# KhaoulaAguech/pl-fem-vectoriel

Hardware: AMD Instinct MI355X
Metric: eigenmodes/sec (assembly+solve), 7-core P2 mesh, 10 modes; |Δn_eff| vs ref (higher is better)
Workload: dtype f64

## Files before the change

### include/plfem.h

```cpp
#ifndef PLFEM_H
#define PLFEM_H

#include <stdint.h>

#ifdef __cplusplus
extern "C" {
#endif

#define PLFEM_OK 0
#define PLFEM_EINVAL (-1)
#define PLFEM_EMESH (-2)
#define PLFEM_EHIP (-3)
#define PLFEM_ENOCONV (-4)
#define PLFEM_ESTATE (-5)
#define PLFEM_ESINGULAR (-6)
#define PLFEM_ERESIDUAL (-7)
#define PLFEM_EHOST (-8)

typedef struct plfem_symbolic plfem_symbolic;
typedef struct plfem_ctx plfem_ctx;

int plfem_symbolic_create(int32_t nv, int32_t ne, const double* p_host, const int32_t* t_host,
                          int32_t leaf_elems, int32_t nthreads, plfem_symbolic** out,
                          char* err, int32_t errlen);
// ... 15 lines not shown
int plfem_symbolic_get(const plfem_symbolic* sym, const char* name, void* out_host, int64_t nbytes);

int plfem_mesh_edge_count(int32_t nv, int32_t ne, const double* p_host, const int32_t* t_host,
                          int32_t* nedges, char* err, int32_t errlen);
int plfem_mesh_refine(int32_t nv, int32_t ne, const double* p_host, const int32_t* t_host,
                      double* p_out, int32_t* t_out, char* err, int32_t errlen);

int plfem_mesh_refine_marked_count(int32_t nv, int32_t ne, const double* p_host, const int32_t* t_host,
                                   const uint8_t* marked_host, int32_t* nv_out, int32_t* ne_out, char* err, int32_t errlen);
int plfem_mesh_refine_marked(int32_t nv, int32_t ne, const double* p_host, const int32_t* t_host,
                             const uint8_t* marked_host, double* p_out, int32_t* t_out, int32_t* parent_out,
                             char* err, int32_t errlen);

#define PLFEM_MAX_NCV 320
int plfem_workspace_bytes(const plfem_symbolic* sym, int32_t max_ncv, int64_t* bytes);
int plfem_create(const plfem_symbolic* sym, int32_t device, void* hip_stream, int32_t max_ncv,
                 void* workspace_dev, int64_t workspace_bytes, plfem_ctx** out, char* err, int32_t errlen);
void plfem_destroy(plfem_ctx* ctx);
const char* plfem_last_error(const plfem_ctx* ctx);
int plfem_synchronize(plfem_ctx* ctx);

int plfem_assemble_hfield(plfem_ctx* ctx, const double* cores_host, int32_t ncore, double eps_core,
                          double eps_clad, double k0, double alpha_p);

int plfem_assemble_scalar(plfem_ctx* ctx, const double* cores_host, int32_t ncore, double eps_core,
                          double eps_clad, double k0);

int plfem_set_index_profile(plfem_ctx* ctx, const double* layers_host, int32_t nlayer, double eps_bg);

int plfem_set_index_map(plfem_ctx* ctx, const double* eps_host, int32_t nx, int32_t ny, double x0, double y0, double dx,
                        double dy);

int plfem_cmt_coupling(plfem_ctx* ctx, int32_t n, const double* fields_i_dev, const double* fields_j_dev,
                       const double* cores_host, int32_t ncore, double eps_core, double eps_clad,
                       double* raw_host, double* pi_host, double* pj_host, double* eps_mean_host);

enum { PLFEM_BLK_AXX = 0, PLFEM_BLK_AXY, PLFEM_BLK_AYX, PLFEM_BLK_AYY, PLFEM_BLK_MINV,
       PLFEM_BLK_DXX, PLFEM_BLK_DXY, PLFEM_BLK_DYY, PLFEM_BLK_COUNT };
int plfem_block_values_dev(plfem_ctx* ctx, int32_t block, const double** values_dev);
int plfem_block_values_host(plfem_ctx* ctx, int32_t block, double* values_host);

int plfem_spmv(plfem_ctx* ctx, int32_t which, const double* x_dev, double* y_dev);

int plfem_factor(plfem_ctx* ctx, double sigma);
int plfem_solve(plfem_ctx* ctx, const double* rhs_dev, double* x_dev, int32_t refine_steps);

int plfem_lanczos_shift_invert(plfem_ctx* ctx, int32_t k, int32_t ncv, double tol, int32_t maxiter,
                               double sigma, double* evals_host, double* evecs_dev, double* stats_host);

enum { PLFEM_POST_NORM = 0, PLFEM_POST_DIV_ENERGY, PLFEM_POST_CORE_X, PLFEM_POST_CORE_Y,
       PLFEM_POST_ALL_X, PLFEM_POST_ALL_Y, PLFEM_POST_COUNT };
int plfem_postprocess(plfem_ctx* ctx, int32_t k, double* evecs_dev, const double* cores_host,
                      int32_t ncore, double* out_host, double* frac_core_host, double* modes_int_dev);

int plfem_residuals(plfem_ctx* ctx, int32_t k, const double* evals_host, const double* evecs_dev, double* out_host);

enum { PLFEM_SOLVE_NCONV = 0, PLFEM_SOLVE_NOPINV, PLFEM_SOLVE_RESTARTS, PLFEM_SOLVE_MAX_REL_RES, PLFEM_SOLVE_BLOCK_SOLVES,
       PLFEM_SOLVE_RESIDUAL_FIRST, PLFEM_SOLVE_RESIDUAL, PLFEM_SOLVE_REFINED, PLFEM_SOLVE_PERTURBED,
       PLFEM_SOLVE_T_ASSEMBLE_US, PLFEM_SOLVE_T_FACTOR_US, PLFEM_SOLVE_T_LANCZOS_US, PLFEM_SOLVE_T_POST_US,
       PLFEM_SOLVE_T_UPLOAD_US, PLFEM_SOLVE_T_RESIDUAL_US, PLFEM_SOLVE_T_CALL_US, PLFEM_SOLVE_STATS };
int plfem_solve_modes(plfem_ctx* ctx, const double* cores_host, int32_t ncore, double eps_core, double eps_clad,
                      double k0, double alpha_p, double sigma, int32_t k, int32_t ncv, double tol, int32_t maxiter,
                      double residual_tol, double tol_refined, double* evals_host, double* post_host,
                      double* frac_core_host, double* resid_host, double* modes_int_host, double* stats_host);
int plfem_modes_dev(plfem_ctx* ctx, const double** evecs_dev, int32_t* k);

int plfem_set_option(plfem_ctx* ctx, const char* name, double value);

int plfem_timings(plfem_ctx* ctx, double* out_host );

enum { PLFEM_PROF_KFWD = 0, PLFEM_PROF_FWD_SWEEP, PLFEM_PROF_BWD_SWEEP, PLFEM_PROF_SPMV_B, PLFEM_PROF_COUNT };
int plfem_profile_begin(plfem_ctx* ctx, int32_t max_ranges);
int plfem_profile_end(plfem_ctx* ctx, double* out_host );

#define PLFEM_LOC_TOL 1e-10
#define PLFEM_LOC_EPS4 8.881784197001252e-16
typedef struct plfem_locator plfem_locator;
int plfem_locator_bytes(const plfem_symbolic* sym, int64_t* bytes);
int plfem_locator_create(const plfem_symbolic* sym, int32_t device, void* hip_stream, void* mem_dev, int64_t mem_bytes,
                         plfem_locator** out, char* err, int32_t errlen);
void plfem_locator_destroy(plfem_locator* loc);
const char* plfem_locator_last_error(const plfem_locator* loc);
int plfem_stage_modes(plfem_locator* loc, int32_t ncomp, int32_t k, int32_t nrows, const double* src_dev, double* dst_dev);
int plfem_sample_fields(plfem_locator* loc, int32_t ncomp, int32_t k, const double* modes_dev, int32_t indexed,
                        const double* beta_dev, int32_t npts, const double* points_dev, double* out_dev, int32_t* elem_dev);
int plfem_overlap_work_bytes(int32_t ka, int32_t kb, int64_t* bytes);
int plfem_field_overlap(plfem_locator* loc_a, const double* modes_a_dev, int32_t ka, int32_t indexed_a,
                        plfem_locator* loc_b, const double* modes_b_dev, int32_t kb, int32_t indexed_b, int32_t ncomp,
                        const double* cores_host, int32_t ncore, double eps_core, double eps_clad,
                        void* work_dev, int64_t work_bytes, double* out_host);
int plfem_overlap_posed_work_bytes(const plfem_locator* loc_b, int32_t ka, int32_t kb, int32_t nposes, int64_t* bytes);
int plfem_field_overlap_posed(plfem_locator* loc_a, const double* modes_a_dev, int32_t ka, int32_t indexed_a,
                              plfem_locator* loc_b, const double* modes_b_dev, int32_t kb, int32_t indexed_b, int32_t ncomp,
                              const double* cores_host, int32_t ncore, double eps_core, double eps_clad,
                              int32_t nposes, const double* poses_host ,
                              void* work_dev, int64_t work_bytes, double* out_host );
int plfem_gram_work_bytes(int32_t ncomp, int32_t k, int64_t* bytes);
int plfem_mode_grams(plfem_locator* loc, int32_t ncomp, int32_t k, const double* modes_dev, int32_t indexed,
                     const double* cores_host, int32_t ncore, void* work_dev, int64_t work_bytes, double* out_host);

int plfem_profile_gram_work_bytes(int32_t ncomp, int32_t k, int64_t* bytes);
int plfem_profile_grams(plfem_locator* loc, int32_t ncomp, int32_t k, const double* modes_dev, int32_t indexed,
                        const double* layers_host, int32_t nlayer, double eps_bg, void* work_dev, int64_t work_bytes,
                        double* out_host);

int plfem_locator_set_index_map(plfem_locator* loc, const double* eps_host, int32_t nx, int32_t ny, double x0, double y0,
                                double dx, double dy);

int plfem_core_gram_work_bytes(const plfem_locator* loc, int32_t ncomp, int32_t k, int32_t ncore, int64_t* bytes);
int plfem_core_grams(plfem_locator* loc, int32_t ncomp, int32_t k, const double* modes_dev, int32_t indexed,
                     const double* cores_host, int32_t ncore, void* work_dev, int64_t work_bytes,
                     double* out_host   ,
                     int64_t* count_host );

int plfem_moment_gram_work_bytes(int32_t ncomp, int32_t k, int64_t* bytes);
int plfem_moment_grams(plfem_locator* loc, int32_t ncomp, int32_t k, const double* modes_dev, int32_t indexed,
                       const double* cores_host, int32_t ncore, const double origin_host[2], void* work_dev,
                       int64_t work_bytes, double* out_host);

int plfem_quartic_work_bytes(int32_t ncomp, int32_t k, int64_t* bytes);
int plfem_mode_quartic(plfem_locator* loc, int32_t ncomp, int32_t k, const double* modes_dev, int32_t indexed,
                       const double* cores_host, int32_t ncore, double w_core, double w_clad,
                       void* work_dev, int64_t work_bytes, double* out_host);

int plfem_project_work_bytes(int32_t ncomp, int32_t k, int32_t la, int32_t lb, int64_t* bytes);
int plfem_mode_project(plfem_locator* loc, int32_t ncomp, int32_t k, const double* modes_dev, int32_t indexed,
                       int32_t la, const double* xfac_host ,
                       int32_t lb, const double* yfac_host ,
                       void* work_dev, int64_t work_bytes, double* out_host );

int plfem_project_sampled_work_bytes(int32_t ncomp, int32_t k, int32_t nf, int64_t* bytes);
int plfem_mode_project_sampled(plfem_locator* loc, int32_t ncomp, int32_t k, const double* modes_dev, int32_t indexed,
                               int32_t nx, int32_t ny, double x0, double y0, double dx, double dy,
                               int32_t nf, const double* frames_dev ,
                               void* work_dev, int64_t work_bytes, double* out_host );

int plfem_indicator_work_bytes(const plfem_locator* loc, int32_t ncomp, int32_t k, int64_t* bytes);
int plfem_mode_indicators(plfem_locator* loc, int32_t ncomp, int32_t k, const double* modes_dev, int32_t indexed,
                          const double* lambda_host , double k0, double alpha_p,
                          const double* cores_host, int32_t ncore, double eps_core, double eps_clad,
                          const double* layers_host, int32_t nlayer, double eps_bg,
                          void* work_dev, int64_t work_bytes, double* out_host );

#ifdef PLFEM_TEST_HOOKS
int plfem_debug_factor_until(plfem_ctx* ctx, double sigma, int32_t level, int32_t step, int32_t stage);
int plfem_debug_copy(plfem_ctx* ctx, const char* name, int64_t offset, int64_t count, double* out_host);
int plfem_debug_symeig(int32_t n, const double* a_host, int32_t last_rows, double* w_out, double* v_out);
int plfem_debug_symeig_band(int32_t n, int32_t b, const double* a_host, int32_t nsel, double* w_out, double* v_out);
int plfem_debug_set_perturb(plfem_ctx* ctx, double value);
int plfem_debug_set_elements(plfem_ctx* ctx, const double* elem_host );
#define PLFEM_DEBUG_PLAN_FIELDS 10
int plfem_debug_solve_block(plfem_ctx* ctx, const double* rhs_dev, int64_t ldx, double* x_dev, int32_t refine_steps);
int plfem_debug_level_plan(plfem_ctx* ctx, int64_t* out, int64_t cap);
enum { PLFEM_DEBUG_PANEL_DOT = 0, PLFEM_DEBUG_PANEL_AXPY, PLFEM_DEBUG_PANEL_DOT_BLOCK, PLFEM_DEBUG_PANEL_AXPY_BLOCK };
enum { PLFEM_DEBUG_SPMV_B_BLOCK = 0, PLFEM_DEBUG_SPMV_B_BLOCK_IL, PLFEM_DEBUG_SPMV_B_BLOCK_IL_GRAM, PLFEM_DEBUG_SPMV_A_BLOCK };
int plfem_debug_panel(plfem_ctx* ctx, int32_t form, int32_t ncols, const double* Pm, double* W, int64_t ldw, double* H,
                      int32_t ldh, double* hacc, int32_t ldacc, double* wil);
int plfem_debug_scale_store(plfem_ctx* ctx, const double* w, const double* bw, const double* beta2, double* v, double* bv,
                            double* beta_out);
int plfem_debug_first_pass(plfem_ctx* ctx, const double* xl_front, const double* BVm, const double* Vm, int32_t ncols,
                           double* W, int64_t ldw, double* Hout, int32_t ldh);
int plfem_debug_spmv_block(plfem_ctx* ctx, int32_t form, const double* x, double* y, int64_t ld, double* gram_out,
                           int32_t* nparts);
int plfem_debug_chol(plfem_ctx* ctx, const double* G, int32_t ldg, int32_t use_partials, int32_t nchunks, double* Tblk,
                     int32_t ldT, double* Rinv, int32_t* rank_flag);
int plfem_debug_block_scale(plfem_ctx* ctx, const double* W, const double* BW, int64_t ldw, const double* Rinv, double* Vn,
                            double* BVn, int64_t ldv, const double* exp_src, int32_t exp_n, double* exp_dst, int32_t* cnt_dst,
                            int32_t want_front);
int plfem_debug_rotate(plfem_ctx* ctx, const double* V, int32_t m, const double* S, int32_t ldS, int32_t p, double* out);
int plfem_debug_start_field(plfem_ctx* ctx, int32_t nvec, double* out);
#endif

#ifdef __cplusplus
}
#endif
#endif
```

### pl_fem_vectoriel_amd/_native.py

```python
from __future__ import annotations

import ctypes
import time
import os
from typing import Optional

import numpy as np

_HERE = os.path.dirname(os.path.abspath(__file__))
LIB_PATH = os.path.join(_HERE, "libplfem_hip.so")
HOOKS_PATH = os.path.join(_HERE, "libplfem_testhooks.so")

PLFEM_OK = 0
PLFEM_EINVAL, PLFEM_EMESH, PLFEM_EHIP, PLFEM_ENOCONV, PLFEM_ESTATE, PLFEM_ESINGULAR, PLFEM_ERESIDUAL = -1, -2, -3, -4, -5, -6, -7
PLFEM_EHOST = -8
BLOCKS = ("Axx", "Axy", "Ayx", "Ayy", "Minv", "Dxx", "Dxy", "Dyy")
INFO_NAMES = ("nv", "ne", "nedges", "N", "nsolve", "nnz", "levels", "nfronts", "front_doubles", "max_front",
              "solve_entries", "factor_flops", "t_numbering_us", "t_pattern_us", "t_tree_us", "t_fronts_us", "dofs_per_node",
              "arena_doubles")
POST_NAMES = ("norm", "div_energy", "core_x", "core_y", "all_x", "all_y")

EXPORTS = (
    "plfem_symbolic_create", "plfem_symbolic_destroy", "plfem_symbolic_info", "plfem_symbolic_array_bytes",
    "plfem_symbolic_get", "plfem_workspace_bytes", "plfem_create", "plfem_destroy", "plfem_last_error", "plfem_synchronize",
    "plfem_assemble_hfield", "plfem_block_values_dev", "plfem_block_values_host", "plfem_spmv", "plfem_factor",
    "plfem_solve", "plfem_lanczos_shift_invert", "plfem_postprocess", "plfem_timings",
    "plfem_profile_begin", "plfem_profile_end",
    "plfem_mesh_edge_count", "plfem_mesh_refine",
    "plfem_residuals", "plfem_set_option", "plfem_symbolic_create_ex", "plfem_assemble_scalar", "plfem_cmt_coupling",
    "plfem_solve_modes", "plfem_modes_dev",
    "plfem_locator_bytes", "plfem_locator_create", "plfem_locator_destroy", "plfem_locator_last_error", "plfem_stage_modes",
    "plfem_sample_fields", "plfem_overlap_work_bytes", "plfem_field_overlap", "plfem_gram_work_bytes", "plfem_mode_grams",
    "plfem_overlap_posed_work_bytes", "plfem_field_overlap_posed",
    "plfem_quartic_work_bytes", "plfem_mode_quartic", "plfem_project_work_bytes", "plfem_mode_project",
    "plfem_core_gram_work_bytes", "plfem_core_grams", "plfem_moment_gram_work_bytes", "plfem_moment_grams",
    "plfem_set_index_profile", "plfem_profile_gram_work_bytes", "plfem_profile_grams",
    "plfem_project_sampled_work_bytes", "plfem_mode_project_sampled",
    "plfem_indicator_work_bytes", "plfem_mode_indicators", "plfem_mesh_refine_marked_count", "plfem_mesh_refine_marked",
    "plfem_set_index_map", "plfem_locator_set_index_map",
)
SOLVE_STATS = ("nconv", "n_opinv", "restarts", "max_rel_res", "n_block_solves", "true_residual_first", "true_residual", "refined",
               "pivot_perturbations", "assemble_us", "factor_us", "lanczos_us", "post_us", "upload_us", "residual_us", "call_us")
TEST_HOOK_EXPORTS = ("plfem_debug_factor_until", "plfem_debug_copy", "plfem_debug_symeig", "plfem_debug_symeig_band",
                     "plfem_debug_set_perturb", "plfem_debug_solve_block", "plfem_debug_level_plan", "plfem_debug_panel",
                     "plfem_debug_scale_store", "plfem_debug_first_pass", "plfem_debug_spmv_block", "plfem_debug_chol",
                     "plfem_debug_block_scale", "plfem_debug_rotate", "plfem_debug_start_field", "plfem_debug_set_elements")
PANEL_FORMS = ("dot", "axpy", "dot_block", "axpy_block")
SPMV_BLOCK_FORMS = ("b_block", "b_block_il", "b_block_il_gram", "a_block")
BLOCK_P = 4
PLAN_FIELDS = ("count", "fwd_rows", "bwd_rows", "fwd_mixed", "max_s2", "max_m", "fwd_n", "bwd_n", "steps", "max_block_p")
MAX_NCV = 320
PROF_SLOTS = ("k_fwd", "fwd_sweep", "bwd_sweep", "spmv_b")

_ARRAY_DTYPES = {
    "edof": np.int32, "tsorted": np.int32, "edges": np.int32, "doflocs": np.float64, "bmask": np.uint8,
    "interior": np.int32, "int_index": np.int32, "rowptr": np.int32, "colind": np.int32, "slot_row": np.int32,
    "nptr": np.int32, "nadj": np.int32, "nloc": np.uint8, "leaf_of_elem": np.int32, "leaf_elem_ptr": np.int32, "leaf_elems": np.int32, "epos": np.int32, "epos_leaf": np.int32,
    "owner": np.int32, "fs": np.int32, "fb": np.int32, "fs_true": np.int32, "fb_true": np.int32,
    "fnode_ptr": np.int64, "fnodes": np.int32, "cinv0": np.int32, "cinv1": np.int32, "foff": np.int64, "soff": np.int64, "prow": np.int32, "npos": np.int32,
    "loc_grid": np.float64, "loc_cell_ptr": np.int32, "loc_cell_elems": np.int32, "loc_stats": np.float64,
    "elem_nbr": np.int32,
}


from scipy.sparse.linalg import ArpackNoConvergence as _ArpackNoConvergence


def set_index_map_call(entry, handle, index_map):
    if index_map is None:
        return entry(handle, None, 0, 0, 0.0, 0.0, 0.0, 0.0)
    eps, x0, y0, dx, dy = index_map
    eps = np.ascontiguousarray(eps, dtype=np.float64)
    if eps.ndim != 2:
        raise ValueError("the index map must be a (ny, nx) array")
    return entry(handle, eps.ctypes.data_as(ctypes.c_void_p), eps.shape[1], eps.shape[0], float(x0), float(y0), float(dx),
                 float(dy))


class ArpackLikeNoConvergence(_ArpackNoConvergence, RuntimeError):

    def __init__(self, msg, eigenvalues=None, eigenvectors=None, stats=None):
        _ArpackNoConvergence.__init__(self, msg, eigenvalues, eigenvectors)
        self.stats = stats


_lib = None
_hooks = None

SCRATCH_FILL = None


def device_scratch(nbytes: int, tdev):
    import torch
    if SCRATCH_FILL is None:
        return torch.empty(int(nbytes), dtype=torch.uint8, device=tdev)
    buf = torch.empty((int(nbytes) + 7) & ~7, dtype=torch.uint8, device=tdev)
    buf.view(torch.float64).fill_(float(SCRATCH_FILL))
    torch.cuda.current_stream(tdev).synchronize()
    return buf


def device_output(shape, dtype, tdev):
    import torch
    if SCRATCH_FILL is None:
        return torch.empty(shape, dtype=dtype, device=tdev)
    shape = tuple(int(v) for v in (shape if isinstance(shape, (tuple, list)) else (shape,)))
    nbytes = int(np.prod(shape, dtype=np.int64)) * torch.empty((), dtype=dtype).element_size()
    return device_scratch(nbytes, tdev)[:nbytes].view(dtype).view(shape)


def _tune_host_allocator(_force: bool = False) -> None:
    if os.environ.get("PLFEM_MALLOC_TUNE", "0") != "1" and not _force:
        return
    try:
        libc = ctypes.CDLL("libc.so.6")
        libc.mallopt(-3, 32 << 20)
        libc.mallopt(-1, 512 << 20)
    except (OSError, AttributeError):
        pass


def load_library() -> ctypes.CDLL:
    global _lib
    if _lib is not None:
        return _lib
    if not os.path.exists(LIB_PATH):
        raise RuntimeError(
            f"libplfem_hip.so requis: {LIB_PATH} not found — build it with "
            "`python -c 'import __graft_entry__ as g; g.build()'` (hipcc --offload-arch=gfx950). "
            "There is no CPU fallback for the eigenmode path.")
    import torch
    lib = ctypes.CDLL(LIB_PATH)
    _tune_host_allocator()
    c_void_pp = ctypes.POINTER(ctypes.c_void_p)
    lib.plfem_symbolic_create.argtypes = [ctypes.c_int32, ctypes.c_int32, ctypes.c_void_p, ctypes.c_void_p,
                                          ctypes.c_int32, ctypes.c_int32, c_void_pp, ctypes.c_char_p, ctypes.c_int32]
    lib.plfem_symbolic_create_ex.argtypes = [ctypes.c_int32, ctypes.c_int32, ctypes.c_void_p, ctypes.c_void_p, ctypes.c_int32,
                                             ctypes.c_int32, ctypes.c_int32, ctypes.c_int32, c_void_pp, ctypes.c_char_p, ctypes.c_int32]
    lib.plfem_symbolic_destroy.argtypes = [ctypes.c_void_p]
    lib.plfem_symbolic_destroy.restype = None
    lib.plfem_symbolic_info.argtypes = [ctypes.c_void_p, ctypes.c_void_p]
    lib.plfem_symbolic_array_bytes.argtypes = [ctypes.c_void_p, ctypes.c_char_p]
    lib.plfem_symbolic_array_bytes.restype = ctypes.c_int64
    lib.plfem_symbolic_get.argtypes = [ctypes.c_void_p, ctypes.c_char_p, ctypes.c_void_p, ctypes.c_int64]
    lib.plfem_workspace_bytes.argtypes = [ctypes.c_void_p, ctypes.c_int32, ctypes.POINTER(ctypes.c_int64)]
    lib.plfem_create.argtypes = [ctypes.c_void_p, ctypes.c_int32, ctypes.c_void_p, ctypes.c_int32, ctypes.c_void_p,
                                 ctypes.c_int64, c_void_pp, ctypes.c_char_p, ctypes.c_int32]
    lib.plfem_destroy.argtypes = [ctypes.c_void_p]
    lib.plfem_destroy.restype = None
    lib.plfem_last_error.argtypes = [ctypes.c_void_p]
    lib.plfem_last_error.restype = ctypes.c_char_p
    lib.plfem_synchronize.argtypes = [ctypes.c_void_p]
    lib.plfem_assemble_hfield.argtypes = [ctypes.c_void_p, ctypes.c_void_p, ctypes.c_int32, ctypes.c_double,
                                          ctypes.c_double, ctypes.c_double, ctypes.c_double]
    lib.plfem_assemble_scalar.argtypes = [ctypes.c_void_p, ctypes.c_void_p, ctypes.c_int32, ctypes.c_double,
                                          ctypes.c_double, ctypes.c_double]
    lib.plfem_cmt_coupling.argtypes = [ctypes.c_void_p, ctypes.c_int32, ctypes.c_void_p, ctypes.c_void_p, ctypes.c_void_p,
                                       ctypes.c_int32, ctypes.c_double, ctypes.c_double, ctypes.c_void_p, ctypes.c_void_p,
                                       ctypes.c_void_p, ctypes.POINTER(ctypes.c_double)]
    lib.plfem_block_values_dev.argtypes = [ctypes.c_void_p, ctypes.c_int32, c_void_pp]
    lib.plfem_block_values_host.argtypes = [ctypes.c_void_p, ctypes.c_int32, ctypes.c_void_p]
    lib.plfem_spmv.argtypes = [ctypes.c_void_p, ctypes.c_int32, ctypes.c_void_p, ctypes.c_void_p]
    lib.plfem_factor.argtypes = [ctypes.c_void_p, ctypes.c_double]
    lib.plfem_solve.argtypes = [ctypes.c_void_p, ctypes.c_void_p, ctypes.c_void_p, ctypes.c_int32]
    lib.plfem_lanczos_shift_invert.argtypes = [ctypes.c_void_p, ctypes.c_int32, ctypes.c_int32, ctypes.c_double,
                                               ctypes.c_int32, ctypes.c_double, ctypes.c_void_p, ctypes.c_void_p,
                                               ctypes.c_void_p]
    lib.plfem_postprocess.argtypes = [ctypes.c_void_p, ctypes.c_int32, ctypes.c_void_p, ctypes.c_void_p,
                                      ctypes.c_int32, ctypes.c_void_p, ctypes.c_void_p, ctypes.c_void_p]
    lib.plfem_timings.argtypes = [ctypes.c_void_p, ctypes.c_void_p]
    lib.plfem_mesh_edge_count.argtypes = [ctypes.c_int32, ctypes.c_int32, ctypes.c_void_p, ctypes.c_void_p,
                                          ctypes.POINTER(ctypes.c_int32), ctypes.c_char_p, ctypes.c_int32]
    lib.plfem_mesh_refine.argtypes = [ctypes.c_int32, ctypes.c_int32, ctypes.c_void_p, ctypes.c_void_p,
                                      ctypes.c_void_p, ctypes.c_void_p, ctypes.c_char_p, ctypes.c_int32]
    lib.plfem_profile_begin.argtypes = [ctypes.c_void_p, ctypes.c_int32]
    lib.plfem_profile_end.argtypes = [ctypes.c_void_p, ctypes.c_void_p]
    lib.plfem_residuals.argtypes = [ctypes.c_void_p, ctypes.c_int32, ctypes.c_void_p, ctypes.c_void_p, ctypes.c_void_p]
    lib.plfem_set_option.argtypes = [ctypes.c_void_p, ctypes.c_char_p, ctypes.c_double]
    lib.plfem_solve_modes.argtypes = ([ctypes.c_void_p, ctypes.c_void_p, ctypes.c_int32] + [ctypes.c_double] * 5 +
                                      [ctypes.c_int32, ctypes.c_int32, ctypes.c_double, ctypes.c_int32, ctypes.c_double,
                                       ctypes.c_double] + [ctypes.c_void_p] * 6)
    lib.plfem_modes_dev.argtypes = [ctypes.c_void_p, c_void_pp, ctypes.POINTER(ctypes.c_int32)]
    lib.plfem_locator_bytes.argtypes = [ctypes.c_void_p, ctypes.POINTER(ctypes.c_int64)]
    lib.plfem_locator_create.argtypes = [ctypes.c_void_p, ctypes.c_int32, ctypes.c_void_p, ctypes.c_void_p, ctypes.c_int64,
                                         c_void_pp, ctypes.c_char_p, ctypes.c_int32]
    lib.plfem_locator_destroy.argtypes = [ctypes.c_void_p]
    lib.plfem_locator_destroy.restype = None
    lib.plfem_locator_last_error.argtypes = [ctypes.c_void_p]
    lib.plfem_locator_last_error.restype = ctypes.c_char_p
    lib.plfem_stage_modes.argtypes = [ctypes.c_void_p, ctypes.c_int32, ctypes.c_int32, ctypes.c_int32, ctypes.c_void_p,
                                      ctypes.c_void_p]
    lib.plfem_sample_fields.argtypes = [ctypes.c_void_p, ctypes.c_int32, ctypes.c_int32, ctypes.c_void_p, ctypes.c_int32,
                                        ctypes.c_void_p, ctypes.c_int32, ctypes.c_void_p, ctypes.c_void_p, ctypes.c_void_p]
    lib.plfem_overlap_work_bytes.argtypes = [ctypes.c_int32, ctypes.c_int32, ctypes.POINTER(ctypes.c_int64)]
    lib.plfem_field_overlap.argtypes = ([ctypes.c_void_p, ctypes.c_void_p, ctypes.c_int32, ctypes.c_int32] * 2 +
                                        [ctypes.c_int32, ctypes.c_void_p, ctypes.c_int32, ctypes.c_double, ctypes.c_double,
                                         ctypes.c_void_p, ctypes.c_int64, ctypes.c_void_p])
    lib.plfem_overlap_posed_work_bytes.argtypes = [ctypes.c_void_p, ctypes.c_int32, ctypes.c_int32, ctypes.c_int32,
                                                   ctypes.POINTER(ctypes.c_int64)]
    lib.plfem_field_overlap_posed.argtypes = ([ctypes.c_void_p, ctypes.c_void_p, ctypes.c_int32, ctypes.c_int32] * 2 +
                                              [ctypes.c_int32, ctypes.c_void_p, ctypes.c_int32, ctypes.c_double, ctypes.c_double,
                                               ctypes.c_int32, ctypes.c_void_p, ctypes.c_void_p, ctypes.c_int64, ctypes.c_void_p])
    lib.plfem_gram_work_bytes.argtypes = [ctypes.c_int32, ctypes.c_int32, ctypes.POINTER(ctypes.c_int64)]
    lib.plfem_mode_grams.argtypes = [ctypes.c_void_p, ctypes.c_int32, ctypes.c_int32, ctypes.c_void_p, ctypes.c_int32,
                                     ctypes.c_void_p, ctypes.c_int32, ctypes.c_void_p, ctypes.c_int64, ctypes.c_void_p]
    lib.plfem_core_gram_work_bytes.argtypes = [ctypes.c_void_p, ctypes.c_int32, ctypes.c_int32, ctypes.c_int32,
                                               ctypes.POINTER(ctypes.c_int64)]
    lib.plfem_core_grams.argtypes = [ctypes.c_void_p, ctypes.c_int32, ctypes.c_int32, ctypes.c_void_p, ctypes.c_int32,
                                     ctypes.c_void_p, ctypes.c_int32, ctypes.c_void_p, ctypes.c_int64, ctypes.c_void_p,
                                     ctypes.c_void_p]
    lib.plfem_moment_gram_work_bytes.argtypes = [ctypes.c_int32, ctypes.c_int32, ctypes.POINTER(ctypes.c_int64)]
    lib.plfem_moment_grams.argtypes = [ctypes.c_void_p, ctypes.c_int32, ctypes.c_int32, ctypes.c_void_p, ctypes.c_int32,
                                       ctypes.c_void_p, ctypes.c_int32, ctypes.c_void_p, ctypes.c_void_p, ctypes.c_int64,
                                       ctypes.c_void_p]
    lib.plfem_set_index_profile.argtypes = [ctypes.c_void_p, ctypes.c_void_p, ctypes.c_int32, ctypes.c_double]
    lib.plfem_set_index_map.argtypes = [ctypes.c_void_p, ctypes.c_void_p, ctypes.c_int32, ctypes.c_int32] + [ctypes.c_double] * 4
    lib.plfem_locator_set_index_map.argtypes = lib.plfem_set_index_map.argtypes
    lib.plfem_profile_gram_work_bytes.argtypes = [ctypes.c_int32, ctypes.c_int32, ctypes.POINTER(ctypes.c_int64)]
    lib.plfem_profile_grams.argtypes = [ctypes.c_void_p, ctypes.c_int32, ctypes.c_int32, ctypes.c_void_p, ctypes.c_int32,
                                        ctypes.c_void_p, ctypes.c_int32, ctypes.c_double, ctypes.c_void_p, ctypes.c_int64,
                                        ctypes.c_void_p]
    lib.plfem_quartic_work_bytes.argtypes = [ctypes.c_int32, ctypes.c_int32, ctypes.POINTER(ctypes.c_int64)]
    lib.plfem_mode_quartic.argtypes = [ctypes.c_void_p, ctypes.c_int32, ctypes.c_int32, ctypes.c_void_p, ctypes.c_int32,
                                       ctypes.c_void_p, ctypes.c_int32, ctypes.c_double, ctypes.c_double, ctypes.c_void_p,
                                       ctypes.c_int64, ctypes.c_void_p]
    lib.plfem_project_work_bytes.argtypes = [ctypes.c_int32] * 4 + [ctypes.POINTER(ctypes.c_int64)]
    lib.plfem_mode_project.argtypes = [ctypes.c_void_p, ctypes.c_int32, ctypes.c_int32, ctypes.c_void_p, ctypes.c_int32,
                                       ctypes.c_int32, ctypes.c_void_p, ctypes.c_int32, ctypes.c_void_p, ctypes.c_void_p,
                                       ctypes.c_int64, ctypes.c_void_p]
    lib.plfem_project_sampled_work_bytes.argtypes = [ctypes.c_int32] * 3 + [ctypes.POINTER(ctypes.c_int64)]
    lib.plfem_mode_project_sampled.argtypes = [ctypes.c_void_p, ctypes.c_int32, ctypes.c_int32, ctypes.c_void_p, ctypes.c_int32,
                                               ctypes.c_int32, ctypes.c_int32, ctypes.c_double, ctypes.c_double, ctypes.c_double,
                                               ctypes.c_double, ctypes.c_int32, ctypes.c_void_p, ctypes.c_void_p, ctypes.c_int64,
                                               ctypes.c_void_p]
    lib.plfem_indicator_work_bytes.argtypes = [ctypes.c_void_p, ctypes.c_int32, ctypes.c_int32, ctypes.POINTER(ctypes.c_int64)]
    lib.plfem_mode_indicators.argtypes = [ctypes.c_void_p, ctypes.c_int32, ctypes.c_int32, ctypes.c_void_p, ctypes.c_int32,
                                          ctypes.c_void_p, ctypes.c_double, ctypes.c_double, ctypes.c_void_p, ctypes.c_int32,
                                          ctypes.c_double, ctypes.c_double, ctypes.c_void_p, ctypes.c_int32, ctypes.c_double,
                                          ctypes.c_void_p, ctypes.c_int64, ctypes.c_void_p]
    lib.plfem_mesh_refine_marked_count.argtypes = [ctypes.c_int32, ctypes.c_int32, ctypes.c_void_p, ctypes.c_void_p,
                                                   ctypes.c_void_p, ctypes.POINTER(ctypes.c_int32),
                                                   ctypes.POINTER(ctypes.c_int32), ctypes.c_char_p, ctypes.c_int32]
    lib.plfem_mesh_refine_marked.argtypes = [ctypes.c_int32, ctypes.c_int32, ctypes.c_void_p, ctypes.c_void_p, ctypes.c_void_p,
                                             ctypes.c_void_p, ctypes.c_void_p, ctypes.c_void_p, ctypes.c_char_p, ctypes.c_int32]
    _lib = lib
    return lib


def _ptr(a: np.ndarray):
    return a.ctypes.data_as(ctypes.c_void_p)


def mesh_refine(p, t):
    lib = load_library()
    p = np.ascontiguousarray(np.asarray(p, dtype=np.float64))
    t = np.ascontiguousarray(np.asarray(t, dtype=np.int32))
    if p.ndim != 2 or p.shape[0] != 2 or t.ndim != 2 or t.shape[0] != 3:
        raise ValueError("mesh.p must be (2, nv) and mesh.t (3, ne)")
    err = ctypes.create_string_buffer(512)
    nedges = ctypes.c_int32(0)
    rc = lib.plfem_mesh_edge_count(p.shape[1], t.shape[1], _ptr(p), _ptr(t), ctypes.byref(nedges), err, 512)
    if rc != PLFEM_OK:
        raise ValueError(f"plfem_mesh_edge_count failed ({rc}): {err.value.decode()}")
    p2 = np.empty((2, p.shape[1] + nedges.value), dtype=np.float64)
    t2 = np.empty((3, 4 * t.shape[1]), dtype=np.int32)
    rc = lib.plfem_mesh_refine(p.shape[1], t.shape[1], _ptr(p), _ptr(t), _ptr(p2), _ptr(t2), err, 512)
    if rc != PLFEM_OK:
        raise ValueError(f"plfem_mesh_refine failed ({rc}): {err.value.decode()}")
    return p2, t2


def mesh_refine_marked(p, t, marked):
    lib = load_library()
    p = np.ascontiguousarray(np.asarray(p, dtype=np.float64))
    t = np.ascontiguousarray(np.asarray(t, dtype=np.int32))
    if p.ndim != 2 or p.shape[0] != 2 or t.ndim != 2 or t.shape[0] != 3:
        raise ValueError("mesh.p must be (2, nv) and mesh.t (3, ne)")
    try:
        mk = np.asarray(marked)
        if mk.dtype.kind not in "biu":
            raise TypeError
    except (TypeError, ValueError):
        raise ValueError("marked must be an array of one flag (bool or integer) per element") from None
    if mk.shape != (t.shape[1],):
        raise ValueError(f"marked must have one flag per element ({t.shape[1]}), got shape {mk.shape}")
    mk = np.ascontiguousarray(mk != 0, dtype=np.uint8)
    err = ctypes.create_string_buffer(512)
    nv2, ne2 = ctypes.c_int32(0), ctypes.c_int32(0)
    rc = lib.plfem_mesh_refine_marked_count(p.shape[1], t.shape[1], _ptr(p), _ptr(t), _ptr(mk), ctypes.byref(nv2),
                                            ctypes.byref(ne2), err, 512)
    if rc != PLFEM_OK:
        raise ValueError(f"plfem_mesh_refine_marked_count failed ({rc}): {err.value.decode()}")
    p2 = np.empty((2, nv2.value), dtype=np.float64)
    t2 = np.empty((3, ne2.value), dtype=np.int32)
    parent = np.empty(ne2.value, dtype=np.int32)
    rc = lib.plfem_mesh_refine_marked(p.shape[1], t.shape[1], _ptr(p), _ptr(t), _ptr(mk), _ptr(p2), _ptr(t2), _ptr(parent),
                                      err, 512)
    if rc != PLFEM_OK:
        raise ValueError(f"plfem_mesh_refine_marked failed ({rc}): {err.value.decode()}")
    return p2, t2, parent


def load_test_hooks() -> ctypes.CDLL:
    global _hooks
    if _hooks is not None:
        return _hooks
    load_library()
    if not os.path.exists(HOOKS_PATH):
        raise RuntimeError(f"{HOOKS_PATH} not found -- build it with `python -c 'import __graft_entry__ as g; g.build()'`")
    h = ctypes.CDLL(HOOKS_PATH)
    h.plfem_debug_factor_until.argtypes = [ctypes.c_void_p, ctypes.c_double, ctypes.c_int32, ctypes.c_int32, ctypes.c_int32]
    h.plfem_debug_copy.argtypes = [ctypes.c_void_p, ctypes.c_char_p, ctypes.c_int64, ctypes.c_int64, ctypes.c_void_p]
    h.plfem_debug_set_perturb.argtypes = [ctypes.c_void_p, ctypes.c_double]
    h.plfem_debug_set_elements.argtypes = [ctypes.c_void_p, ctypes.c_void_p]
    h.plfem_debug_solve_block.argtypes = [ctypes.c_void_p, ctypes.c_void_p, ctypes.c_int64, ctypes.c_void_p, ctypes.c_int32]
    h.plfem_debug_level_plan.argtypes = [ctypes.c_void_p, ctypes.c_void_p, ctypes.c_int64]
    h.plfem_debug_symeig.argtypes = [ctypes.c_int32, ctypes.c_void_p, ctypes.c_int32, ctypes.c_void_p, ctypes.c_void_p]
    h.plfem_debug_symeig_band.argtypes = [ctypes.c_int32, ctypes.c_int32, ctypes.c_void_p, ctypes.c_int32,
                                          ctypes.c_void_p, ctypes.c_void_p]
    vp, i32, i64 = ctypes.c_void_p, ctypes.c_int32, ctypes.c_int64
    h.plfem_debug_panel.argtypes = [vp, i32, i32, vp, vp, i64, vp, i32, vp, i32, vp]
    h.plfem_debug_scale_store.argtypes = [vp, vp, vp, vp, vp, vp, vp]
    h.plfem_debug_first_pass.argtypes = [vp, vp, vp, vp, i32, vp, i64, vp, i32]
    h.plfem_debug_spmv_block.argtypes = [vp, i32, vp, vp, i64, vp, vp]
    h.plfem_debug_chol.argtypes = [vp, vp, i32, i32, i32, vp, i32, vp, vp]
    h.plfem_debug_block_scale.argtypes = [vp, vp, vp, i64, vp, vp, vp, i64, vp, i32, vp, vp, i32]
    h.plfem_debug_rotate.argtypes = [vp, vp, i32, vp, i32, i32, vp]
    h.plfem_debug_start_field.argtypes = [vp, i32, vp]
    _hooks = h
    return h


def debug_symeig(a, last_rows: int = -1):
    lib = load_test_hooks()
    a = np.ascontiguousarray(np.asarray(a, dtype=np.float64))
    n = a.shape[0]
    if a.shape != (n, n):
        raise ValueError("square matrix expected")
    w = np.empty(n, dtype=np.float64)
    v = np.empty((n, n if last_rows < 0 else last_rows), dtype=np.float64)
    rc = lib.plfem_debug_symeig(n, _ptr(a), int(last_rows), _ptr(w), _ptr(v))
    if rc != PLFEM_OK:
        raise ValueError(f"plfem_debug_symeig failed ({rc})")
    return w, v


def debug_symeig_band(a, b: int, nsel: int):
    lib = load_test_hooks()
    a = np.ascontiguousarray(np.asarray(a, dtype=np.float64))
    n = a.shape[0]
    if a.shape != (n, n):
        raise ValueError("square matrix expected")
    w = np.empty(n, dtype=np.float64)
    v = np.empty((n, n), dtype=np.float64)
    rc = lib.plfem_debug_symeig_band(n, int(b), _ptr(a), int(nsel), _ptr(w), _ptr(v))
    if rc != PLFEM_OK:
        raise ValueError(f"plfem_debug_symeig_band failed ({rc})")
    return w, v


def default_host_threads() -> int:
    ncpu = os.cpu_count() or 1
    if ncpu < 64:
        return max(1, min(ncpu, 8))
    try:
        local_world = max(1, int(os.environ.get("LOCAL_WORLD_SIZE", "1")))
    except ValueError:
        local_world = 1
    return max(2, min(24, (ncpu // 2) // local_world))


class Symbolic:

    def __init__(self, p, t, leaf_elems: int = 0, nthreads: int = 0, dofs_per_node: int = 2, dirichlet: bool = True):
        lib = load_library()
        p = np.ascontiguousarray(np.asarray(p, dtype=np.float64))
        t = np.ascontiguousarray(np.asarray(t, dtype=np.int32))
        if p.ndim != 2 or p.shape[0] != 2 or t.ndim != 2 or t.shape[0] != 3:
            raise ValueError("mesh.p must be (2, nv) and mesh.t (3, ne)")
        h = ctypes.c_void_p()
        err = ctypes.create_string_buffer(512)
        if nthreads <= 0:
            nthreads = int(os.environ.get("PLFEM_HOST_THREADS", default_host_threads()))
        if leaf_elems <= 0:
            leaf_elems = int(os.environ.get("PLFEM_LEAF_ELEMS", 0))
        rc = lib.plfem_symbolic_create_ex(p.shape[1], t.shape[1], _ptr(p), _ptr(t), int(leaf_elems), int(nthreads),
                                          int(dofs_per_node), 1 if dirichlet else 0, ctypes.byref(h), err, 512)
        if rc != PLFEM_OK:
            raise ValueError(f"plfem_symbolic_create failed ({rc}): {err.value.decode()}")
        self._h = h
        self._lib = lib
        info = np.zeros(32, dtype=np.int64)
        lib.plfem_symbolic_info(h, _ptr(info))
        self.info = {k: int(info[i]) for i, k in enumerate(INFO_NAMES)}
        for k in ("nv", "ne", "nedges", "N", "nsolve", "nnz"):
            setattr(self, k, self.info[k])
        self.dofs_per_node = self.info["dofs_per_node"]

    def array(self, name: str) -> np.ndarray:
        nb = self._lib.plfem_symbolic_array_bytes(self._h, name.encode())
        if nb < 0:
            raise KeyError(name)
        out = np.empty(nb // np.dtype(_ARRAY_DTYPES[name]).itemsize, dtype=_ARRAY_DTYPES[name])
        rc = self._lib.plfem_symbolic_get(self._h, name.encode(), _ptr(out), ctypes.c_int64(nb))
        if rc != PLFEM_OK:
            raise RuntimeError(f"plfem_symbolic_get({name}) failed: {rc}")
        return out

    def close(self):
        if getattr(self, "_h", None):
            self._lib.plfem_symbolic_destroy(self._h)
            self._h = None

    def __del__(self):
        try:
            self.close()
        except Exception:
            pass


class Context:

    def __init__(self, sym: Symbolic, device: Optional[int] = None, max_ncv: int = 65, use_torch_stream: bool = True):
        import torch

        lib = load_library()
        if not torch.cuda.is_available():
            raise RuntimeError("no HIP device visible: the eigenmode path has no CPU fallback")
        if device is None:
            device = torch.cuda.current_device()
        self.torch = torch
        self.device = int(device)
        self.tdev = torch.device("cuda", self.device)
        self.sym = sym
        self._lib = lib
        stream = torch.cuda.current_stream(self.tdev).cuda_stream if use_torch_stream else 0
        h = ctypes.c_void_p()
        err = ctypes.create_string_buffer(512)
        need = ctypes.c_int64(0)
        rc = lib.plfem_workspace_bytes(sym._h, int(max_ncv), ctypes.byref(need))
        if rc != PLFEM_OK:
            raise ValueError(f"plfem_workspace_bytes failed ({rc})")
        t0 = time.perf_counter()
        self.workspace = device_scratch(int(need.value) + 256, self.tdev)
        self.t_workspace = time.perf_counter() - t0
        base = self.workspace.data_ptr()
        aligned = (base + 255) & ~255
        rc = lib.plfem_create(sym._h, self.device, ctypes.c_void_p(stream), int(max_ncv), ctypes.c_void_p(aligned),
                              ctypes.c_int64(int(need.value)), ctypes.byref(h), err, 512)
        if rc in (PLFEM_EINVAL, PLFEM_EMESH):
            raise ValueError(f"plfem_create: {err.value.decode()}")
        if rc != PLFEM_OK:
            raise RuntimeError(f"plfem_create failed ({rc}): {err.value.decode()}")
        self._h = h
        self.max_ncv = int(max_ncv)
        self.N = sym.N
        self.dpn = sym.dofs_per_node
        self.n2 = self.dpn * sym.N

    def _check(self, rc, what):
        if rc == PLFEM_OK:
            return
        msg = self._lib.plfem_last_error(self._h).decode()
        if rc in (PLFEM_EINVAL, PLFEM_EMESH):
            raise ValueError(f"{what}: {msg}")
        raise RuntimeError(f"{what} failed ({rc}): {msg}")

    def _cores(self, cores):
        c = np.ascontiguousarray(np.asarray(cores, dtype=np.float64).reshape(-1, 3))
        return c, c.shape[0]

    def empty(self, *shape):
        return device_output(shape, self.torch.float64, self.tdev)

    def set_index_profile(self, profile=None):
        if profile is None:
            self._check(self._lib.plfem_set_index_profile(self._h, None, 0, 0.0), "plfem_set_index_profile")
            self.set_index_map(None)
            return
        t = np.ascontiguousarray(np.asarray(profile.table(), dtype=np.float64).reshape(-1, 8))
        index_map = getattr(profile, "index_map", None)
        if t.shape[0] == 0 and index_map is None:
            raise ValueError("plfem_set_index_profile: the profile has no layers")
# ... 41 lines not shown
    def factor(self, sigma: float):
        self._check(self._lib.plfem_factor(self._h, float(sigma)), "plfem_factor")

    def solve(self, rhs, refine_steps: int = 0):
        x = self.empty(self.n2)
        self._check(self._lib.plfem_solve(self._h, ctypes.c_void_p(rhs.data_ptr()), ctypes.c_void_p(x.data_ptr()),
                                          int(refine_steps)), "plfem_solve")
        return x

    def lanczos(self, k, ncv, tol, maxiter, sigma):
        evals = np.empty(k, dtype=np.float64)
        evecs = self.empty(k, self.n2)
        stats = np.zeros(8, dtype=np.float64)
        rc = self._lib.plfem_lanczos_shift_invert(self._h, int(k), int(ncv), float(tol), int(maxiter), float(sigma),
                                                  _ptr(evals), ctypes.c_void_p(evecs.data_ptr()), _ptr(stats))
        st = {"nconv": int(stats[0]), "n_opinv": int(stats[1]), "restarts": int(stats[2]), "max_rel_res": float(stats[3]),
              "n_block_solves": int(stats[4])}
        if rc == PLFEM_ENOCONV:
            raise ArpackLikeNoConvergence(self._lib.plfem_last_error(self._h).decode(), evals, evecs, st)
        self._check(rc, "plfem_lanczos_shift_invert")
        return evals, evecs, st

    def solve_modes(self, cores, eps_core, eps_clad, k0, alpha_p, sigma, k, ncv, tol, maxiter, residual_tol, tol_refined,
                    modes_host=None):
        c, n = self._cores(cores)
        evals = np.empty(k, dtype=np.float64)
        post = np.zeros((k, len(POST_NAMES)), dtype=np.float64)
        resid = np.zeros(k, dtype=np.float64)
        stats = np.zeros(len(SOLVE_STATS), dtype=np.float64)
        frac = ctypes.c_double(0.0)
        if modes_host is not None and (tuple(modes_host.shape) != (k, self.dpn * self.sym.nsolve) or not modes_host.is_contiguous()
                                       or modes_host.dtype != self.torch.float64 or modes_host.device.type != "cpu"):
            raise ValueError("modes_host must be a contiguous float64 CPU tensor of shape (k, dofs_per_node * nsolve)")
        rc = self._lib.plfem_solve_modes(self._h, _ptr(c), n, float(eps_core), float(eps_clad), float(k0), float(alpha_p),
                                         float(sigma), int(k), int(ncv), float(tol), int(maxiter), float(residual_tol),
                                         float(tol_refined), _ptr(evals), _ptr(post), ctypes.cast(ctypes.byref(frac), ctypes.c_void_p),
                                         _ptr(resid), ctypes.c_void_p(modes_host.data_ptr()) if modes_host is not None else None,
                                         _ptr(stats))
        st = {name: (float(stats[i]) if name.endswith("_us") or "res" in name else int(stats[i])) for i, name in enumerate(SOLVE_STATS)}
        st["refined"] = bool(st["refined"])
        if rc == PLFEM_ENOCONV:
            raise ArpackLikeNoConvergence(self._lib.plfem_last_error(self._h).decode(), evals, self.modes_dev(), st)
        self._check(rc, "plfem_solve_modes")
        return evals, post, float(frac.value), resid, st

    def modes_dev(self):
        ptr = ctypes.c_void_p()
        k = ctypes.c_int32(0)
        self._check(self._lib.plfem_modes_dev(self._h, ctypes.byref(ptr), ctypes.byref(k)), "plfem_modes_dev")

        class _View:
            __cuda_array_interface__ = {"shape": (int(k.value), int(self.n2)), "typestr": "<f8", "data": (int(ptr.value), False),
                                        "version": 2, "strides": None}
        return self.torch.as_tensor(_View(), device=self.tdev).clone()

    def postprocess(self, evecs, cores, want_interior: bool = True):
        k = evecs.shape[0]
        c, n = self._cores(cores)
        out = np.zeros((k, len(POST_NAMES)), dtype=np.float64)
        frac = ctypes.c_double(0.0)
        modes_int = self.empty(k, self.dpn * self.sym.nsolve) if want_interior else None
        self._check(self._lib.plfem_postprocess(self._h, int(k), ctypes.c_void_p(evecs.data_ptr()), _ptr(c), n,
                                                _ptr(out), ctypes.byref(frac),
                                                ctypes.c_void_p(modes_int.data_ptr()) if want_interior else None),
                    "plfem_postprocess")
        return out, float(frac.value), modes_int

    def timings(self):
        t = np.zeros(8, dtype=np.float64)
        self._check(self._lib.plfem_timings(self._h, _ptr(t)), "plfem_timings")
        return {"assemble_us": t[0], "factor_us": t[1], "lanczos_us": t[2], "post_us": t[3], "upload_us": t[4],
                "pivot_perturbations": int(t[5])}

    def debug_factor_until(self, sigma, level, step, stage):
        self._check(load_test_hooks().plfem_debug_factor_until(self._h, float(sigma), int(level), int(step), int(stage)),
                    "plfem_debug_factor_until")

    def debug_copy(self, name: str, offset: int, count: int) -> np.ndarray:
        out = np.empty(int(count), dtype=np.float64)
        self._check(load_test_hooks().plfem_debug_copy(self._h, name.encode(), ctypes.c_int64(int(offset)),
                                                       ctypes.c_int64(int(count)), _ptr(out)), "plfem_debug_copy")
        return out

    def debug_set_perturb(self, value: float):
        self._check(load_test_hooks().plfem_debug_set_perturb(self._h, float(value)), "plfem_debug_set_perturb")

    def debug_set_elements(self, elem: np.ndarray):
        elem = np.ascontiguousarray(elem, dtype=np.float64)
        if elem.size != self.sym.ne * 8 * 36:
            raise ValueError("debug_set_elements: need ne x 8 x 36 doubles")
        self._check(load_test_hooks().plfem_debug_set_elements(self._h, _ptr(elem)), "plfem_debug_set_elements")

    def debug_solve_block(self, rhs, x, ldx: int, refine_steps: int = 0):
        self._check(load_test_hooks().plfem_debug_solve_block(self._h, ctypes.c_void_p(rhs.data_ptr()), ctypes.c_int64(int(ldx)),
                                                              ctypes.c_void_p(x.data_ptr()), int(refine_steps)),
                    "plfem_debug_solve_block")

    @staticmethod
    def _dev(t, offset: int = 0):
        return None if t is None else ctypes.c_void_p(t.data_ptr() + 8 * int(offset))

    def debug_panel(self, form: str, ncols: int, Pm, W, ldw: int, H, ldh: int, hacc=None, ldacc: int = 0, wil=None):
        d = self._dev
        self._check(load_test_hooks().plfem_debug_panel(self._h, PANEL_FORMS.index(form), int(ncols), d(Pm), d(W), int(ldw), d(H),
                                                        int(ldh), d(hacc), int(ldacc), d(wil)), "plfem_debug_panel")

    def debug_scale_store(self, w, bw, beta2, v, bv, beta_out=None):
        d = self._dev
        self._check(load_test_hooks().plfem_debug_scale_store(self._h, d(w), d(bw), d(beta2), d(v), d(bv), d(beta_out)),
                    "plfem_debug_scale_store")

    def debug_first_pass(self, xl_front, BVm, Vm, ncols: int, W, ldw: int, Hout, ldh: int):
        d = self._dev
        self._check(load_test_hooks().plfem_debug_first_pass(self._h, d(xl_front), d(BVm), d(Vm), int(ncols), d(W), int(ldw),
                                                             d(Hout), int(ldh)), "plfem_debug_first_pass")

    def debug_spmv_block(self, form: str, x, y, ld: int, gram_out=None) -> int:
        nparts = ctypes.c_int32(0)
        d = self._dev
        self._check(load_test_hooks().plfem_debug_spmv_block(self._h, SPMV_BLOCK_FORMS.index(form), d(x), d(y), int(ld),
                                                             d(gram_out), ctypes.byref(nparts)), "plfem_debug_spmv_block")
        return int(nparts.value)

    def debug_chol(self, G, ldg: int, use_partials: bool, nchunks: int, Tblk, ldT: int, Rinv, Tblk_offset: int = 0) -> int:
        flag = ctypes.c_int32(0)
        d = self._dev
        self._check(load_test_hooks().plfem_debug_chol(self._h, d(G), int(ldg), 1 if use_partials else 0, int(nchunks),
                                                       d(Tblk, Tblk_offset), int(ldT), d(Rinv), ctypes.byref(flag)),
                    "plfem_debug_chol")
        return int(flag.value)

    def debug_block_scale(self, W, BW, ldw: int, Rinv, Vn, BVn, ldv: int, exp_src=None, exp_n: int = 0, exp_dst=None,
                          cnt_dst=None, want_front: bool = False):
        d = self._dev
        self._check(load_test_hooks().plfem_debug_block_scale(self._h, d(W), d(BW), int(ldw), d(Rinv), d(Vn), d(BVn), int(ldv),
                                                              d(exp_src), int(exp_n), d(exp_dst), d(cnt_dst),
                                                              1 if want_front else 0), "plfem_debug_block_scale")

    def debug_rotate(self, V, m: int, S, ldS: int, p: int, out):
        d = self._dev
        self._check(load_test_hooks().plfem_debug_rotate(self._h, d(V), int(m), d(S), int(ldS), int(p), d(out)),
                    "plfem_debug_rotate")

    def debug_start_field(self, nvec: int, out):
        self._check(load_test_hooks().plfem_debug_start_field(self._h, int(nvec), self._dev(out)), "plfem_debug_start_field")

    def debug_level_plan(self):
        nl = self.sym.info["levels"] + 1
        out = np.zeros(len(PLAN_FIELDS) * nl, dtype=np.int64)
        self._check(load_test_hooks().plfem_debug_level_plan(self._h, _ptr(out), ctypes.c_int64(out.size)),
                    "plfem_debug_level_plan")
        return [dict(zip(PLAN_FIELDS, (int(v) for v in row))) for row in out.reshape(nl, len(PLAN_FIELDS))]

    def profile_begin(self, max_launches: int = 4096):
        self._check(self._lib.plfem_profile_begin(self._h, int(max_launches)), "plfem_profile_begin")

    def profile_end(self):
        out = np.zeros((len(PROF_SLOTS), 3), dtype=np.float64)
        self._check(self._lib.plfem_profile_end(self._h, _ptr(out)), "plfem_profile_end")
        res = {"launches": int(out[0, 0]), "total_us": float(out[0, 1]), "bytes": float(out[0, 2])}
        res["slots"] = {name: {"ranges": int(out[i, 0]), "total_us": float(out[i, 1]), "bytes": float(out[i, 2])}
                        for i, name in enumerate(PROF_SLOTS)}
        return res

    def residuals(self, evals, evecs) -> np.ndarray:
        lam = np.ascontiguousarray(np.asarray(evals, dtype=np.float64))
        out = np.zeros(len(lam), dtype=np.float64)
        self._check(self._lib.plfem_residuals(self._h, len(lam), _ptr(lam), ctypes.c_void_p(evecs.data_ptr()), _ptr(out)),
                    "plfem_residuals")
        return out

    def set_option(self, name: str, value: float):
        self._check(self._lib.plfem_set_option(self._h, name.encode(), float(value)), "plfem_set_option")

    def synchronize(self):
        self._check(self._lib.plfem_synchronize(self._h), "plfem_synchronize")

    def close(self):
        if getattr(self, "_h", None):
            self._lib.plfem_destroy(self._h)
            self._h = None
            self.workspace = None

    def __del__(self):
        try:
            self.close()
        except Exception:
            pass
```

### pl_fem_vectoriel_amd/csrc/api_debug.hip

```cpp
#include <algorithm>
#include <cmath>
#include <cstring>
#include <numeric>
#include <string>
#include <vector>

#ifndef PLFEM_TEST_HOOKS
#define PLFEM_TEST_HOOKS 1
#endif
#include "device.h"

namespace {
void perturb_root_pivots(plfem_ctx* c) {
  if (c->test_perturb != 0.0)
    plfem::launch_axpby(c, (int64_t)2 * c->dpn * c->S->fs[0], 1.0 + c->test_perturb, c->d_delta, 0.0, c->d_delta,
                        c->d_delta);
}
}

extern "C" int plfem_debug_set_perturb(plfem_ctx* c, double value) try {
  if (!c) return PLFEM_EINVAL;
  c->test_perturb = value;
  c->test_post_factor = value != 0.0 ? perturb_root_pivots : nullptr;
  c->factored = false;
  return PLFEM_OK;
} catch (...) { return host_failure(c); }

extern "C" int plfem_debug_factor_until(plfem_ctx* c, double sigma, int32_t level, int32_t step, int32_t stage) try {
  if (!c) return PLFEM_EINVAL;
  if (!c->assembled) { c->err = "debug factor before assemble"; return PLFEM_ESTATE; }
  TRY(wait_for_upload(c));
  plfem::launch_factor(c, sigma, level, step, stage);
  HIP_TRY(c, hipStreamSynchronize(c->stream));
  return check_launch(c, "debug factor");
} catch (...) { return host_failure(c); }

extern "C" int plfem_debug_copy(plfem_ctx* c, const char* name, int64_t offset, int64_t count, double* out_host) try {
  if (!c || !name || !out_host || offset < 0 || count < 0) return PLFEM_EINVAL;
  std::string n(name);
  const double* src = nullptr;
  if (n == "front") src = c->d_front;
  else if (n == "schur") src = c->d_schur;
  else if (n == "fvec") src = c->d_fvec;
  else if (n == "wbuf") src = c->d_wbuf;
  else if (n == "rbuf") src = c->d_rbuf;
  else if (n == "dinv") src = c->d_dinv;
  else if (n == "delta") src = c->d_delta;
  else if (n == "fvec2") src = c->d_fvec2;
  else if (n == "xl") src = c->d_xl;
  else if (n == "elem") src = c->d_elem;
  else if (n == "V") src = c->d_V;
  else if (n == "BV") src = c->d_BV;
  else if (n == "Hcols") src = c->d_Hcols;
  else if (n == "counters") {
    if (offset + count > 4) return PLFEM_EINVAL;
    int32_t tmp[4];
    HIP_TRY(c, hipStreamSynchronize(c->stream));
    HIP_TRY(c, hipMemcpy(tmp, c->d_counters, sizeof(tmp), hipMemcpyDeviceToHost));
    for (int64_t q = 0; q < count; ++q) out_host[q] = (double)tmp[offset + q];
    return PLFEM_OK;
  }
  else if (n == "colind" || n == "slot_row") {
    if (offset + count > c->nnz) return PLFEM_EINVAL;
    std::vector<int32_t> tmp((size_t)count);
    HIP_TRY(c, hipStreamSynchronize(c->stream));
    HIP_TRY(c, hipMemcpy(tmp.data(), (n == "colind" ? c->d_colind : c->d_slot_row) + offset, sizeof(int32_t) * count, hipMemcpyDeviceToHost));
    for (int64_t q = 0; q < count; ++q) out_host[q] = (double)tmp[q];
    return PLFEM_OK;
  }
  else return PLFEM_EINVAL;
  HIP_TRY(c, hipStreamSynchronize(c->stream));
  HIP_TRY(c, hipMemcpy(out_host, src + offset, sizeof(double) * count, hipMemcpyDeviceToHost));
  return PLFEM_OK;
} catch (...) { return host_failure(c); }

extern "C" int plfem_debug_set_elements(plfem_ctx* c, const double* elem_host) try {
  if (!c || !elem_host) return PLFEM_EINVAL;
  HIP_TRY(c, hipSetDevice(c->device));
  TRY(wait_for_upload(c));
  HIP_TRY(c, hipStreamSynchronize(c->stream));
  HIP_TRY(c, hipMemcpy(c->d_elem, elem_host, sizeof(double) * (size_t)c->ne * plfem::ELEM_STRIDE, hipMemcpyHostToDevice));
  plfem::launch_csr_gather(c);
  HIP_TRY(c, hipStreamSynchronize(c->stream));
  TRY(check_launch(c, "debug set elements"));
  c->assembled = true;
  c->factored = false;
  return PLFEM_OK;
} catch (...) { return host_failure(c); }

extern "C" int plfem_debug_solve_block(plfem_ctx* c, const double* rhs_dev, int64_t ldx, double* x_dev, int32_t refine_steps) try {
  constexpr int P = plfem::BLOCK_P;
  if (!c || !rhs_dev || !x_dev || refine_steps < 0) return PLFEM_EINVAL;
  if (!c->factored) { c->err = "debug block solve before plfem_factor"; return PLFEM_ESTATE; }
  if (c->max_block_p < P) { c->err = "debug block solve: the LDS budget of this tree allows one right-hand side per sweep"; return PLFEM_EINVAL; }
  if (ldx < c->n2) { c->err = "debug block solve: ldx < n2"; return PLFEM_EINVAL; }
  const int64_t scratch = (int64_t)c->n2 * plfem::basis_cols(c->max_ncv);
  if (refine_steps > 0 && 3 * P * ldx > scratch) { c->err = "debug block solve: ldx too large for the refinement scratch"; return PLFEM_EINVAL; }
  HIP_TRY(c, hipSetDevice(c->device));
  plfem::solve_refined(c, P, rhs_dev, x_dev, ldx, false, refine_steps, c->d_V2, c->d_V2 + (size_t)P * ldx,
                       c->d_V2 + (size_t)2 * P * ldx);
  HIP_TRY(c, hipStreamSynchronize(c->stream));
  return check_launch(c, "debug block solve");
} catch (...) { return host_failure(c); }

extern "C" int plfem_debug_level_plan(plfem_ctx* c, int64_t* out, int64_t cap) try {
  if (!c || !out) return PLFEM_EINVAL;
  const plfem::LaunchPlan& plan = *c->plan;
  const int nl = (int)plan.levels.size();
  if (cap < (int64_t)PLFEM_DEBUG_PLAN_FIELDS * nl) { c->err = "debug level plan: cap too small"; return PLFEM_EINVAL; }
  for (int l = 0; l < nl; ++l) {
    const plfem::LevelInfo& li = plan.levels[l];
    const int next = l + 1 < nl ? plan.levels[l + 1].step0 : (int)plan.upd_n.size();
    const int64_t rec[PLFEM_DEBUG_PLAN_FIELDS] = {li.count, li.fwd_rows, li.bwd_rows, li.fwd_mixed ? 1 : 0, li.max_s2, li.max_m,
                                                  li.fwd_n, li.bwd_n, next - li.step0, c->max_block_p};
    std::copy(rec, rec + PLFEM_DEBUG_PLAN_FIELDS, out + (int64_t)PLFEM_DEBUG_PLAN_FIELDS * l);
  }
  return PLFEM_OK;
} catch (...) { return host_failure(c); }

namespace {
int lanczos_hook_done(plfem_ctx* c, const char* what) {
  HIP_TRY(c, hipStreamSynchronize(c->stream));
  return check_launch(c, what);
}
}

extern "C" int plfem_debug_panel(plfem_ctx* c, int32_t form, int32_t ncols, const double* Pm, double* W, int64_t ldw, double* H,
                                 int32_t ldh, double* hacc, int32_t ldacc, double* wil) try {
  constexpr int P = plfem::BLOCK_P;
  if (!c || !H || !Pm || !W || form < PLFEM_DEBUG_PANEL_DOT || form > PLFEM_DEBUG_PANEL_AXPY_BLOCK) return PLFEM_EINVAL;
  if (ncols < 1 || ncols > c->max_ncv + P) { c->err = "debug panel: need 1 <= ncols <= max_ncv + BLOCK_P"; return PLFEM_EINVAL; }
  const bool block = form == PLFEM_DEBUG_PANEL_DOT_BLOCK || form == PLFEM_DEBUG_PANEL_AXPY_BLOCK;
  if (block && (ldw < c->n2 || ldh < ncols || (hacc && ldacc < ncols))) { c->err = "debug panel: leading dimension too small"; return PLFEM_EINVAL; }
  HIP_TRY(c, hipSetDevice(c->device));
  switch (form) {
    case PLFEM_DEBUG_PANEL_DOT: plfem::launch_panel_dot(c, 1, Pm, ncols, W, ldw, H, ldh, hacc, ldacc); break;
    case PLFEM_DEBUG_PANEL_AXPY: plfem::launch_panel_axpy(c, 1, Pm, ncols, H, ldh, W, ldw); break;
    case PLFEM_DEBUG_PANEL_DOT_BLOCK: plfem::launch_panel_dot(c, P, Pm, ncols, W, ldw, H, ldh, hacc, ldacc); break;
    default: plfem::launch_panel_axpy(c, P, Pm, ncols, H, ldh, W, ldw, wil); break;
  }
  return lanczos_hook_done(c, "debug panel");
} catch (...) { return host_failure(c); }

extern "C" int plfem_debug_scale_store(plfem_ctx* c, const double* w, const double* bw, const double* beta2, double* v, double* bv,
                                       double* beta_out) try {
  if (!c || !w || !bw || !beta2 || !v || !bv) return PLFEM_EINVAL;
  HIP_TRY(c, hipSetDevice(c->device));
  plfem::launch_scale_store(c, w, bw, beta2, v, bv, beta_out);
  return lanczos_hook_done(c, "debug scale store");
} catch (...) { return host_failure(c); }

extern "C" int plfem_debug_first_pass(plfem_ctx* c, const double* xl_front, const double* BVm, const double* Vm, int32_t ncols,
                                      double* W, int64_t ldw, double* Hout, int32_t ldh) try {
  if (!c || !xl_front || !BVm || !Vm || !W || !Hout) return PLFEM_EINVAL;
  if (ncols < 1 || ncols > plfem::FIRST_COLS || ldw < c->n2 || ldh < ncols) { c->err = "debug first pass: need 1 <= ncols <= FIRST_COLS, ldw >= n2, ldh >= ncols"; return PLFEM_EINVAL; }
  HIP_TRY(c, hipSetDevice(c->device));
  HIP_TRY(c, hipMemcpyAsync(c->d_xl, xl_front, sizeof(double) * 2 * c->fnodes_total * plfem::BLOCK_P, hipMemcpyDeviceToDevice, c->stream));
  plfem::launch_first_pass_block(c, BVm, Vm, ncols, W, ldw, Hout, ldh);
  return lanczos_hook_done(c, "debug first pass");
} catch (...) { return host_failure(c); }

extern "C" int plfem_debug_spmv_block(plfem_ctx* c, int32_t form, const double* x, double* y, int64_t ld, double* gram_out,
                                      int32_t* nparts) try {
  constexpr int P = plfem::BLOCK_P;
  if (!c || !x || !y || form < PLFEM_DEBUG_SPMV_B_BLOCK || form > PLFEM_DEBUG_SPMV_A_BLOCK) return PLFEM_EINVAL;
  if (!c->assembled) { c->err = "debug block spmv before assemble"; return PLFEM_ESTATE; }
  if (ld < c->n2) { c->err = "debug block spmv: ld < n2"; return PLFEM_EINVAL; }
  HIP_TRY(c, hipSetDevice(c->device));
  int np = 0;
  switch (form) {
    case PLFEM_DEBUG_SPMV_B_BLOCK: plfem::launch_spmv(c, 1, P, x, y, ld); break;
    case PLFEM_DEBUG_SPMV_B_BLOCK_IL: plfem::launch_spmv_b_block_il(c, x, y, ld); break;
    case PLFEM_DEBUG_SPMV_B_BLOCK_IL_GRAM:
      np = plfem::launch_spmv_b_block_il(c, x, y, ld, c->d_partial);
      if (gram_out) HIP_TRY(c, hipMemcpyAsync(gram_out, c->d_partial, sizeof(double) * P * P * np, hipMemcpyDeviceToDevice, c->stream));
      break;
    default: plfem::launch_spmv(c, 0, P, x, y, ld); break;
  }
  if (nparts) *nparts = np;
  return lanczos_hook_done(c, "debug block spmv");
} catch (...) { return host_failure(c); }

extern "C" int plfem_debug_chol(plfem_ctx* c, const double* G, int32_t ldg, int32_t use_partials, int32_t nchunks, double* Tblk,
                                int32_t ldT, double* Rinv, int32_t* rank_flag) try {
  constexpr int P = plfem::BLOCK_P;
  if (!c || !Tblk || !Rinv || ldT < P) return PLFEM_EINVAL;
  HIP_TRY(c, hipSetDevice(c->device));
  if (use_partials) {
    if (nchunks < 1 || (size_t)P * P * nchunks > c->partial_doubles) { c->err = "debug chol: nchunks out of range"; return PLFEM_EINVAL; }
    if (G) HIP_TRY(c, hipMemcpyAsync(c->d_partial, G, sizeof(double) * P * P * nchunks, hipMemcpyDeviceToDevice, c->stream));
  } else if (!G || ldg < P) {
    return PLFEM_EINVAL;
  }
  HIP_TRY(c, hipMemsetAsync(c->d_counters + 2, 0, sizeof(int32_t), c->stream));
  if (use_partials) plfem::launch_chol_from_partials(c, nchunks, Tblk, ldT, Rinv);
  else plfem::launch_chol_block(c, G, ldg, Tblk, ldT, Rinv);
  int32_t flag = 0;
  HIP_TRY(c, hipMemcpyAsync(&flag, c->d_counters + 2, sizeof(int32_t), hipMemcpyDeviceToHost, c->stream));
  HIP_TRY(c, hipMemsetAsync(c->d_counters + 2, 0, sizeof(int32_t), c->stream));
  TRY(lanczos_hook_done(c, "debug chol"));
  if (rank_flag) *rank_flag = flag;
  return PLFEM_OK;
} catch (...) { return host_failure(c); }

extern "C" int plfem_debug_block_scale(plfem_ctx* c, const double* W, const double* BW, int64_t ldw, const double* Rinv, double* Vn,
                                       double* BVn, int64_t ldv, const double* exp_src, int32_t exp_n, double* exp_dst,
                                       int32_t* cnt_dst, int32_t want_front) try {
  if (!c || !W || !BW || !Rinv || !Vn || !BVn || exp_n < 0) return PLFEM_EINVAL;
  if (ldw < c->n2 || ldv < c->n2) { c->err = "debug block scale: leading dimension < n2"; return PLFEM_EINVAL; }
  if (exp_dst && (!exp_src || !cnt_dst)) { c->err = "debug block scale: an export needs exp_src and cnt_dst"; return PLFEM_EINVAL; }
  HIP_TRY(c, hipSetDevice(c->device));
  plfem::launch_block_scale(c, W, BW, ldw, Rinv, Vn, BVn, ldv, exp_src, exp_dst ? exp_n : 0, exp_dst, cnt_dst,
                            want_front ? c->d_fvec : nullptr);
  return lanczos_hook_done(c, "debug block scale");
} catch (...) { return host_failure(c); }

extern "C" int plfem_debug_rotate(plfem_ctx* c, const double* V, int32_t m, const double* S, int32_t ldS, int32_t p, double* out) try {
  if (!c || !V || !S || !out) return PLFEM_EINVAL;
  if (m < 1 || m > PLFEM_MAX_NCV + plfem::BLOCK_P || p < 1 || ldS < m) { c->err = "debug rotate: need 1 <= m <= PLFEM_MAX_NCV + BLOCK_P, p >= 1, ldS >= m"; return PLFEM_EINVAL; }
  HIP_TRY(c, hipSetDevice(c->device));
  plfem::launch_rotate(c, V, m, S, ldS, p, out);
  return lanczos_hook_done(c, "debug rotate");
} catch (...) { return host_failure(c); }

extern "C" int plfem_debug_start_field(plfem_ctx* c, int32_t nvec, double* out) try {
  if (!c || !out || nvec < 1 || nvec > plfem::BLOCK_P) return PLFEM_EINVAL;
  HIP_TRY(c, hipSetDevice(c->device));
  plfem::launch_start_field(c, nvec, out);
  return lanczos_hook_done(c, "debug start field");
} catch (...) { return host_failure(c); }
```

### pl_fem_vectoriel_amd/csrc/api_debug_host.cpp

```cpp
#include <algorithm>
#include <cmath>
#include <numeric>
#include <vector>

#define PLFEM_TEST_HOOKS 1
#include "../../include/plfem.h"
#include "host_eig.h"
#include "internal.h"

extern "C" int plfem_debug_symeig(int32_t n, const double* a_host, int32_t last_rows, double* w_out, double* v_out) try {
  if (n < 1 || n > 4096 || !a_host || !w_out || !v_out || last_rows > n) return PLFEM_EINVAL;
  std::vector<double> A(a_host, a_host + (size_t)n * n), V, w;
  const bool ok = last_rows < 0 ? plfem::sym_eig(n, A, V, w) : plfem::sym_eig_last_rows(n, last_rows, A, V, w);
  std::copy(w.begin(), w.end(), w_out);
  std::copy(V.begin(), V.end(), v_out);
  return ok ? PLFEM_OK : PLFEM_ENOCONV;
} catch (...) { return host_failure(nullptr, 0); }

extern "C" int plfem_debug_symeig_band(int32_t n, int32_t b, const double* a_host, int32_t nsel, double* w_out, double* v_out) try {
  if (n < 1 || n > 4096 || b < 0 || !a_host || !w_out || !v_out || nsel < 0 || nsel > n) return PLFEM_EINVAL;
  std::vector<double> w;
  bool ok = plfem::sym_band_eigenvalues(n, b, a_host, n, w);
  std::vector<int> order(n);
  std::iota(order.begin(), order.end(), 0);
  std::sort(order.begin(), order.end(), [&](int x, int y) { return std::fabs(w[x]) > std::fabs(w[y]); });
  order.resize(nsel);
  std::fill(v_out, v_out + (size_t)n * n, 0.0);
  ok = plfem::sym_band_eigenvectors(n, b, a_host, n, w, order, v_out, n) && ok;
  std::copy(w.begin(), w.end(), w_out);
  return ok ? PLFEM_OK : PLFEM_ENOCONV;
} catch (...) { return host_failure(nullptr, 0); }
```

### pl_fem_vectoriel_amd/csrc/api_device.hip

```cpp
#include <algorithm>
#include <atomic>
#include <memory>
#include <cmath>
#include <cstdio>
#include <cstdlib>
#include <cstring>
#include <chrono>
#include <mutex>
#include <numeric>
#include <thread>
#include <vector>

#include "device.h"
#include "host_eig.h"
#include "p2_element.h"

using plfem::Symbolic;

namespace {
template <class T>
T& process_wide() {
  static T* t = new T();
  return *t;
}
// ... 64 lines not shown
    auto& cache = pc.blocks;
    int best = -1;
    for (int i = 0; i < (int)cache.size(); ++i)
      if (cache[i].bytes >= bytes && (best < 0 || cache[i].bytes < cache[best].bytes)) best = i;
    if (best >= 0) {
      *out = cache[best].p;
      *got = cache[best].bytes;
      cache.erase(cache.begin() + best);
      return hipSuccess;
    }
  }
  *got = bytes;
  return hipHostMalloc((void**)out, bytes, hipHostMallocMapped | hipHostMallocCoherent | hipHostMallocPortable);
}

void pinned_release(double* p, size_t bytes) noexcept {
  try {
    auto& pc = process_wide<PinnedCache>();
    std::lock_guard<std::mutex> lk(pc.m);
    if (pc.blocks.size() < 8) { pc.blocks.push_back({p, bytes}); return; }
  } catch (const std::exception&) {
  }
  (void)hipHostFree(p);
}
}

namespace {

inline size_t align_up(size_t x) { return (x + 255) & ~(size_t)255; }

template <class T>
int dalloc(plfem_ctx* c, T** dst, size_t count) {
  size_t bytes = align_up(std::max<size_t>(count, 1) * sizeof(T));
  if (c->slab) {
    if (c->slab_off + bytes > c->slab_bytes) { c->err = "workspace too small"; return PLFEM_EINVAL; }
    *dst = reinterpret_cast<T*>(c->slab + c->slab_off);
  }
  c->slab_off += bytes;
  return PLFEM_OK;
}

struct UploadItem { size_t off; const void* src; size_t bytes; };

template <class T, class A>
int upload(plfem_ctx* c, std::vector<UploadItem>& items, T** dst, const std::vector<T, A>& src) {
  const size_t off = c->slab_off;
  int rc = dalloc(c, dst, src.size());
  if (rc != PLFEM_OK) return rc;
  if (c->slab && !src.empty()) items.push_back({off, src.data(), src.size() * sizeof(T)});
  return PLFEM_OK;
}

int flush_uploads(plfem_ctx* c, const std::vector<UploadItem>& items, size_t span, char* staging, size_t mesh_items) {
  size_t total = 0;
  for (const auto& it : items) total += it.bytes;
  const int nthreads = total > (4u << 20) ? 8 : 1;
  const int npieces = total > (2u << 20) ? 4 : 1;
  std::vector<size_t> first(1, 0);
  if (mesh_items > 0 && mesh_items < items.size()) first.push_back(mesh_items);
  {
    size_t acc = 0, rest = 0;
    for (size_t q = first.back(); q < items.size(); ++q) rest += items[q].bytes;
    const size_t q0 = first.back(), base = first.size();
    for (size_t q = q0; q < items.size(); ++q) {
      if ((int)first.size() < npieces && acc >= rest * (first.size() - base + 1) / (npieces - base + 1) && q > first.back()) first.push_back(q);
      acc += items[q].bytes;
    }
    first.push_back(items.size());
  }
  const bool split = c->copy_stream != nullptr && mesh_items > 0 && mesh_items < items.size();
  const size_t npc = first.size() - 1;
  std::unique_ptr<std::atomic<int>[]> done(new std::atomic<int>[npc]);
  for (size_t pc = 0; pc < npc; ++pc) done[pc].store(0, std::memory_order_relaxed);
  hipError_t herr = hipSuccess;
  plfem::host_parallel(nthreads, [&](int t, int nt) {
    for (size_t pc = 0; pc < npc; ++pc) {
      size_t bytes = 0;
      for (size_t q = first[pc]; q < first[pc + 1]; ++q) bytes += items[q].bytes;
      const size_t lo = bytes * t / nt, hi = bytes * (t + 1) / nt;
      size_t pos = 0;
      for (size_t q = first[pc]; q < first[pc + 1] && pos < hi; ++q) {
        const size_t b0 = std::max(lo, pos), b1 = std::min(hi, pos + items[q].bytes);
        if (b0 < b1) std::memcpy(staging + items[q].off + (b0 - pos), (const char*)items[q].src + (b0 - pos), b1 - b0);
        pos += items[q].bytes;
      }
      done[pc].fetch_add(1, std::memory_order_release);
      if (t != 0) continue;
      for (int spins = 0; done[pc].load(std::memory_order_acquire) < nt; ++spins) plfem::cpu_relax(spins);
      const size_t q0 = first[pc], q1 = first[pc + 1];
      if (q0 == q1 || herr != hipSuccess) continue;
      const size_t plo = items[q0].off, phi = q1 < items.size() ? items[q1].off : span;
      herr = hipMemcpyAsync(c->slab + plo, staging + plo, phi - plo, hipMemcpyHostToDevice, (split && pc > 0) ? c->copy_stream : c->stream);
    }
  });
  if (herr == hipSuccess && split) {
    herr = hipEventRecord(c->ev_upload, c->copy_stream);
    c->upload_pending = true;
  }
  if (herr != hipSuccess) {
    c->err = std::string("hipMemcpyAsync (index upload): ") + hipGetErrorString(herr);
    return PLFEM_EHIP;
  }
  return PLFEM_OK;
}

void free_all(plfem_ctx* c) {
  if (c->copy_stream) (void)hipStreamSynchronize(c->copy_stream);
  if (c->own_slab && c->slab) (void)hipFree(c->slab);
  plfem::free_index_map(c->map);
  if (c->h_pinned) pinned_release(c->h_pinned, c->h_pinned_bytes);
  if (c->h_staging) {
    (void)hipStreamSynchronize(c->stream);
    pinned_release(c->h_staging, c->h_staging_bytes);
  }
  for (auto& pr : c->ev)
    for (auto& e : pr) ctx_event_release(c->device, EV_TIMING, e);
  for (auto& e : c->ev_step) ctx_event_release(c->device, EV_NO_TIMING, e);
  process_wide<EventPool>().give_all(c->device, EV_PROFILE, c->prof_ev);
  if (c->copy_stream) {
    (void)hipStreamSynchronize(c->copy_stream);
    process_wide<StreamPool>().give(c->device, 0, c->copy_stream, SIZE_MAX);
    c->copy_stream = nullptr;
  }
  ctx_event_release(c->device, EV_NO_TIMING, c->ev_copy);
  ctx_event_release(c->device, EV_NO_TIMING, c->ev_upload);
}

static double now_ms() { return std::chrono::duration<double, std::milli>(std::chrono::steady_clock::now().time_since_epoch()).count(); }

struct Placement {
  std::vector<UploadItem> items;
  size_t upload_span = 0, mesh_items = 0;
};

int place_buffers(plfem_ctx* c, int max_ncv, Placement& pl) {
  const Symbolic& S = *c->S;
  const plfem::LaunchPlan& P = *c->plan;
  auto& items = pl.items;
  c->slab_off = 0;
  items.clear();
  TRY(upload(c, items, &c->d_edof, S.edof));
  c->d_tsorted = c->d_edof;
  TRY(upload(c, items, &c->d_rowptr, S.rowptr));
  TRY(upload(c, items, &c->d_nptr, S.nptr));
  TRY(upload(c, items, &c->d_nadj, S.nadj));
  TRY(upload(c, items, &c->d_nloc, S.nloc));
  TRY(upload(c, items, &c->d_interior, S.interior));
  TRY(upload(c, items, &c->d_bmask, S.bmask));
  TRY(upload(c, items, &c->d_doflocs, S.doflocs));
  pl.mesh_items = items.size();
  TRY(upload(c, items, &c->d_blk, P.jobs));
  TRY(upload(c, items, reinterpret_cast<plfem::Tile**>(&c->d_tiles), P.tiles));
  TRY(upload(c, items, &c->d_forder, P.forder));
  TRY(upload(c, items, &c->d_frec, P.frec));
  TRY(upload(c, items, &c->d_fs2, P.fs2));
  TRY(upload(c, items, &c->d_fm, P.fm));
  TRY(upload(c, items, &c->d_fnode_ptr, S.fnode_ptr));
  TRY(upload(c, items, &c->d_foff, S.foff));
  TRY(upload(c, items, &c->d_soff, S.soff));
  TRY(upload(c, items, &c->d_fnodes, S.fnodes));
  TRY(upload(c, items, &c->d_cinv0, S.cinv0));
  TRY(upload(c, items, &c->d_cinv1, S.cinv1));
  TRY(upload(c, items, &c->d_epos, S.epos));
  TRY(upload(c, items, &c->d_leaf_elem_ptr, S.leaf_elem_ptr));
  TRY(upload(c, items, &c->d_leaf_elems, S.leaf_elems));
  TRY(upload(c, items, &c->d_npos, S.npos));
  TRY(upload(c, items, &c->d_prow, S.prow));
  pl.upload_span = c->slab_off;
  TRY(dalloc(c, &c->d_colind, (size_t)c->nnz));
  TRY(dalloc(c, &c->d_slot_row, (size_t)c->nnz));
  TRY(dalloc(c, &c->d_cores, plfem::MAX_CORES * 3));
  TRY(dalloc(c, &c->d_elem, (size_t)S.ne * plfem::ELEM_STRIDE));
  for (auto& p : c->d_vals) TRY(dalloc(c, &p, (size_t)c->nnz));
  TRY(dalloc(c, &c->d_front, (size_t)S.foff[S.nfronts]));
  c->arena_doubles = (S.arena_doubles + 31) & ~(int64_t)31;
  const int64_t fnodes_total = c->fnodes_total = S.fnode_ptr[S.nfronts];
  TRY(dalloc(c, &c->d_fvec, (size_t)2 * fnodes_total * plfem::BLOCK_P));
  const size_t union_start = c->slab_off;
  TRY(dalloc(c, &c->d_schur, (size_t)2 * c->arena_doubles));
  TRY(dalloc(c, &c->d_wbuf, (size_t)6 * P.level_nodes_max * plfem::NB));
  TRY(dalloc(c, &c->d_rbuf, (size_t)6 * P.level_nodes_max * plfem::NB));
  const size_t factor_end = c->slab_off;
  const size_t n2 = (size_t)c->n2, nc1 = (size_t)plfem::basis_cols(max_ncv), ncp = (size_t)plfem::proj_cols(max_ncv);
  c->slab_off = union_start;
  TRY(dalloc(c, &c->d_V, n2 * nc1));
  TRY(dalloc(c, &c->d_BV, n2 * nc1));
  TRY(dalloc(c, &c->d_V2, n2 * nc1));
  TRY(dalloc(c, &c->d_BV2, n2 * nc1));
  c->slab_off = std::max(c->slab_off, factor_end);
  TRY(dalloc(c, &c->d_dinv, (size_t)2 * S.nfronts * plfem::NB * plfem::NB));
  TRY(dalloc(c, &c->d_delta, (size_t)4 * fnodes_total));
  TRY(dalloc(c, &c->d_fvec2, (size_t)2 * fnodes_total * plfem::BLOCK_P));
  TRY(dalloc(c, &c->d_u0, (size_t)2 * fnodes_total * plfem::BLOCK_P));
  TRY(dalloc(c, &c->d_u1, (size_t)2 * fnodes_total * plfem::BLOCK_P));
  TRY(dalloc(c, &c->d_xl, (size_t)2 * fnodes_total * plfem::BLOCK_P));
  TRY(dalloc(c, &c->d_counters, 4));
  TRY(dalloc(c, &c->d_w, n2 * plfem::BLOCK_P));
  TRY(dalloc(c, &c->d_bw, n2 * plfem::BLOCK_P));
  TRY(dalloc(c, &c->d_hblk, ncp * plfem::BLOCK_P));
  TRY(dalloc(c, &c->d_G, 64));
  TRY(dalloc(c, &c->d_Rinv, 64));
  TRY(dalloc(c, &c->d_t1, n2 * plfem::BLOCK_P));
  TRY(dalloc(c, &c->d_t2, n2 * plfem::BLOCK_P));
  TRY(dalloc(c, &c->d_h, ncp));
  TRY(dalloc(c, &c->d_hacc, ncp));
  c->partial_doubles = std::max({plfem::panel_dot_partial_doubles(c->n2, (int)ncp), plfem::gram_partial_doubles(S.N),
                                 plfem::first_pass_partial_doubles(c->n2)});
  TRY(dalloc(c, &c->d_partial, c->partial_doubles));
  TRY(dalloc(c, &c->d_scal, 16));
  TRY(dalloc(c, &c->d_S, nc1 * nc1));
  TRY(dalloc(c, &c->d_Hcols, (nc1 + 1) * (nc1 + 1)));
  TRY(dalloc(c, &c->d_coremask, (size_t)S.N));
  c->post_doubles = std::max(plfem::post_sum_doubles(S.N, (int)nc1), plfem::resid_sum_doubles(S.N, (int)nc1)) + 16;
  TRY(dalloc(c, &c->d_post, 2 * c->post_doubles));
  TRY(dalloc(c, &c->d_layers, (size_t)plfem::MAX_LAYERS * plfem::LAYER_DOUBLES));
  return PLFEM_OK;
}

int create_impl(plfem_ctx* c, const plfem_symbolic* sym, int device, void* stream, int max_ncv, void* workspace,
                int64_t workspace_bytes, bool size_only) {
  const Symbolic& S = sym->S;
  c->S = &S;
  c->device = device;
  c->stream = (hipStream_t)stream;
  if (!size_only) {
    HIP_TRY(c, hipSetDevice(device));
    for (auto& pr : c->ev)
      for (auto& e : pr) HIP_TRY(c, ctx_event_acquire(device, EV_TIMING, &e));
    for (auto& e : c->ev_step) HIP_TRY(c, ctx_event_acquire(device, EV_NO_TIMING, &e));
    HIP_TRY(c, ctx_event_acquire(device, EV_NO_TIMING, &c->ev_upload));
    HIP_TRY(c, copy_stream_acquire(device, &c->copy_stream));
    HIP_TRY(c, phase_begin(c, plfem::PH_UPLOAD));
  }
  c->nv = S.nv; c->ne = S.ne; c->N = S.N; c->nnz = S.rowptr.empty() ? 0 : (int)S.rowptr[S.N]; c->nsolve = S.nsolve;
  c->L = S.L; c->nfronts = S.nfronts; c->dpn = S.dpn; c->sh = S.dpn - 1; c->n2 = S.dpn * (int64_t)S.N; c->max_ncv = max_ncv;
  if (!S.plan.built) { c->err = "plfem_create: the analysis carries no launch plan"; return PLFEM_ESTATE; }
  c->plan = &S.plan;
  if (!size_only) {
    int lim = 0;
    HIP_TRY(c, hipDeviceGetAttribute(&lim, hipDeviceAttributeMaxSharedMemoryPerBlock, device));
    const int worst = c->plan->worst_m;
    if (plfem::sweep_lds(plfem::BLOCK_P, worst) <= (size_t)lim) c->max_block_p = plfem::BLOCK_P;
    else if (plfem::sweep_lds(1, worst) <= (size_t)lim) c->max_block_p = 1;
    else {
      c->err = "plfem_create: largest front has " + std::to_string(worst) + " DOFs; the solve sweeps stage 8 (m + 1) bytes of it in LDS, "
               "which exceeds this device's " + std::to_string(lim) + " bytes per workgroup (use a smaller leaf size / a coarser mesh)";
      return PLFEM_EINVAL;
    }
  }
  const bool ctx_trace = getenv("PLFEM_CTX_TRACE") != nullptr;
  const double tt1 = now_ms();
  Placement pl;
  TRY(place_buffers(c, max_ncv, pl));
  const size_t need = c->slab_off;
  c->workspace_need = (int64_t)need;
  if (size_only) return PLFEM_OK;
  if (workspace) {
    if (workspace_bytes < (int64_t)need) { c->err = "plfem_create: workspace smaller than plfem_workspace_bytes"; return PLFEM_EINVAL; }
    if ((uintptr_t)workspace & 255) { c->err = "plfem_create: workspace must be 256-byte aligned"; return PLFEM_EINVAL; }
    c->slab = reinterpret_cast<char*>(workspace);
  } else {
    HIP_TRY(c, hipMalloc((void**)&c->slab, need));
    c->own_slab = true;
  }
  c->slab_bytes = need;
  const double tt2 = now_ms();
  TRY(place_buffers(c, max_ncv, pl));
  double* staging = nullptr;
  size_t staging_bytes = 0;
  HIP_TRY(c, pinned_acquire(pl.upload_span, &staging, &staging_bytes));
  c->h_staging = staging;
  c->h_staging_bytes = staging_bytes;
  TRY(flush_uploads(c, pl.items, pl.upload_span, reinterpret_cast<char*>(staging), pl.mesh_items));
  const double tt3 = now_ms();
  HIP_TRY(c, hipMemsetAsync(c->d_counters, 0, 4 * sizeof(int32_t), c->stream));
  HIP_TRY(c, hipMemsetAsync(c->d_fvec, 0, sizeof(double) * 2 * c->fnodes_total * plfem::BLOCK_P, c->stream));
  plfem::launch_pattern_fill(c);
  TRY(check_launch(c, "pattern fill"));
  {
    const size_t nc1p = (size_t)max_ncv + 2 + plfem::BLOCK_P;
    HIP_TRY(c, pinned_acquire(sizeof(double) * (plfem::PIN_PROJ + nc1p * nc1p + 2 * nc1p * plfem::BLOCK_P), &c->h_pinned, &c->h_pinned_bytes));
    c->h_slots = c->h_pinned + plfem::PIN_PROJ + nc1p * nc1p;
  }
  HIP_TRY(c, phase_end(c, plfem::PH_UPLOAD));
  const double tt4 = now_ms();
  if (ctx_trace) fprintf(stderr, "[ctx] size pass %.3f  upload pass %.3f  pinned+launch %.3f  sync %.3f ms\n", tt2 - tt1, tt3 - tt2, tt4 - tt3, now_ms() - tt4);
  return PLFEM_OK;
}

int upload_cores(plfem_ctx* c, const double* cores_host, int ncore) {
  if (ncore < 0 || ncore > plfem::MAX_CORES || (ncore > 0 && !cores_host)) {
    c->err = "ncore must be in [0, 64]";
    return PLFEM_EINVAL;
  }
  if (ncore > 0) {
    std::memcpy(c->h_pinned + plfem::PIN_CORES, cores_host, sizeof(double) * 3 * ncore);
    HIP_TRY(c, hipMemcpyAsync(c->d_cores, c->h_pinned + plfem::PIN_CORES, sizeof(double) * 3 * ncore, hipMemcpyHostToDevice, c->stream));
  }
  return PLFEM_OK;
}

}

extern "C" int plfem_create(const plfem_symbolic* sym, int32_t device, void* hip_stream, int32_t max_ncv,
                            void* workspace_dev, int64_t workspace_bytes, plfem_ctx** out, char* err,
                            int32_t errlen) try {
  if (!out) return PLFEM_EINVAL;
  *out = nullptr;
  if (!sym) return write_err(err, errlen, "plfem_create: null symbolic handle", PLFEM_EINVAL);
  if (max_ncv < 3 || max_ncv > PLFEM_MAX_NCV)
    return write_err(err, errlen, "plfem_create: max_ncv must be in [3, " + std::to_string(PLFEM_MAX_NCV) + "]", PLFEM_EINVAL);
  int ndev = 0;
  if (hipGetDeviceCount(&ndev) != hipSuccess || ndev < 1)
    return write_err(err, errlen, "plfem_create: no HIP device available (this library has no CPU fallback)", PLFEM_EHIP);
  if (device < 0 || device >= ndev) return write_err(err, errlen, "plfem_create: device index out of range", PLFEM_EINVAL);
  struct FreeCtx {
    void operator()(plfem_ctx* c) const { free_all(c); delete c; }
  };
  std::unique_ptr<plfem_ctx, FreeCtx> c(new plfem_ctx());
  const int rc = create_impl(c.get(), sym, device, hip_stream, max_ncv, workspace_dev, workspace_bytes, false);
  if (rc != PLFEM_OK) return write_err(err, errlen, c->err, rc);
  *out = c.release();
  return PLFEM_OK;
} catch (...) { return host_failure(err, errlen); }

extern "C" int plfem_workspace_bytes(const plfem_symbolic* sym, int32_t max_ncv, int64_t* bytes) try {
  if (!sym || !bytes || max_ncv < 3 || max_ncv > PLFEM_MAX_NCV) return PLFEM_EINVAL;
  plfem_ctx tmp;
  int rc = create_impl(&tmp, sym, 0, nullptr, max_ncv, nullptr, 0, true);
  *bytes = tmp.workspace_need;
  return rc;
} catch (...) { return host_failure(nullptr, 0); }

extern "C" void plfem_destroy(plfem_ctx* ctx) {
  if (!ctx) return;
  (void)hipSetDevice(ctx->device);
  (void)hipStreamSynchronize(ctx->stream);
  free_all(ctx);
  delete ctx;
}

extern "C" const char* plfem_last_error(const plfem_ctx* ctx) { return ctx ? ctx->err.c_str() : "null context"; }

extern "C" int plfem_synchronize(plfem_ctx* ctx) try {
  if (!ctx) return PLFEM_EINVAL;
  HIP_TRY(ctx, hipStreamSynchronize(ctx->stream));
  return PLFEM_OK;
} catch (...) { return host_failure(ctx); }

namespace {
template <class ElementMatrices>
int assemble(plfem_ctx* c, const double* cores_host, int ncore, double eps_core, double eps_clad, const char* what,
             ElementMatrices element_matrices) {
  const bool profile = c->nlayer > 0 || c->map.set();
  if (!profile && (!(eps_core > 0) || !(eps_clad > 0))) { c->err = "permittivities must be positive"; return PLFEM_EINVAL; }
  if (profile && !(c->eps_bg > 0)) {
    c->err = std::string(what) + ": an index map is set without a background permittivity (plfem_set_index_profile(ctx, NULL, 0, eps_bg))";
    return PLFEM_EINVAL;
  }
  HIP_TRY(c, hipSetDevice(c->device));
  TRY(upload_cores(c, cores_host, ncore));
  HIP_TRY(c, phase_begin(c, plfem::PH_ASSEMBLE));
  element_matrices();
  plfem::launch_csr_gather(c);
  HIP_TRY(c, phase_end(c, plfem::PH_ASSEMBLE));
  TRY(check_launch(c, what));
  c->assembled = true;
  c->factored = false;
  return PLFEM_OK;
}
}

extern "C" int plfem_set_index_profile(plfem_ctx* c, const double* layers_host, int32_t nlayer, double eps_bg) try {
  if (!c) return PLFEM_EINVAL;
  if (nlayer == 0) {
    c->nlayer = 0;
    c->eps_bg = (std::isfinite(eps_bg) && eps_bg > 0.0) ? eps_bg : 0.0;
    return PLFEM_OK;
  }
  if (const char* bad = plfem::profile_table_error(layers_host, nlayer, eps_bg)) {
    c->err = std::string("plfem_set_index_profile: ") + bad;
    return PLFEM_EINVAL;
  }
  HIP_TRY(c, hipSetDevice(c->device));
  const size_t bytes = sizeof(double) * plfem::LAYER_DOUBLES * nlayer;
  double* pin = c->h_pinned + plfem::PIN_LAYERS;
  std::memcpy(pin, layers_host, bytes);
  HIP_TRY(c, hipMemcpyAsync(c->d_layers, pin, bytes, hipMemcpyHostToDevice, c->stream));
  HIP_TRY(c, hipStreamSynchronize(c->stream));
  c->nlayer = nlayer;
// ... 670 lines not shown
```

### pl_fem_vectoriel_amd/csrc/device.h

```cpp
#pragma once
#include <hip/hip_runtime.h>

#include <cmath>
#include <cstdint>
#include <functional>
#include <string>
#include <type_traits>
#include <vector>

#include "../../include/plfem.h"
#include "internal.h"
#include "plan.h"

namespace plfem {

constexpr size_t PIN_POST = 0;
constexpr size_t PIN_RESID = 2048;
constexpr size_t PIN_CORE_QP = 4000;
constexpr size_t PIN_COUNTERS = 4096;
constexpr int PIN_COUNTERS_N = 2 * 4;
constexpr size_t PIN_CORES = 6144;
constexpr size_t PIN_LAYERS = 6400;
constexpr size_t PIN_PROJ = 8192;
static_assert(PIN_POST + 5 * PLFEM_MAX_NCV <= PIN_RESID, "pinned layout: post-processing sums");
static_assert(PIN_RESID + 3 * PLFEM_MAX_NCV <= PIN_CORE_QP, "pinned layout: residual check");
static_assert(PIN_CORE_QP + 1 <= PIN_COUNTERS, "pinned layout: core-point counter");
static_assert(PIN_COUNTERS + PIN_COUNTERS_N * sizeof(int32_t) / sizeof(double) <= PIN_CORES, "pinned layout: counters");
static_assert(PIN_CORES + 3 * MAX_CORES <= PIN_LAYERS, "pinned layout: core table");
static_assert(PIN_LAYERS + LAYER_DOUBLES * MAX_LAYERS <= PIN_PROJ, "pinned layout: layer table");

enum Phase { PH_ASSEMBLE, PH_FACTOR, PH_LANCZOS, PH_POST, PH_UPLOAD, PH_RESIDUAL, PH_COUNT };
static_assert(PLFEM_SOLVE_T_ASSEMBLE_US + PH_RESIDUAL == PLFEM_SOLVE_T_RESIDUAL_US, "phases in PLFEM_SOLVE_T_* order");

}

#define HIP_TRY(owner, call)                                                                 \
  do {                                                                                       \
    hipError_t e__ = (call);                                                                 \
    if (e__ != hipSuccess) {                                                                 \
      (owner)->err = std::string(#call) + ": " + hipGetErrorString(e__);                     \
      return PLFEM_EHIP;                                                                     \
    }                                                                                        \
  } while (0)

#define TRY(x)                         \
  do {                                 \
    int rc__ = (x);                    \
    if (rc__ != PLFEM_OK) return rc__; \
  } while (0)

namespace plfem {
struct IndexMap {
  double* d = nullptr;
  size_t cap = 0;
  int nx = 0, ny = 0;
  double x0 = 0, y0 = 0, inv_dx = 0, inv_dy = 0;
  bool set() const { return nx > 0; }
};
struct IndexMapHeader {
  double x0, y0, inv_dx, inv_dy;
  int nx, ny;
};
static_assert(sizeof(IndexMapHeader) <= MAP_HEADER * sizeof(double), "the grid fits the map buffer's header");
}

struct plfem_ctx {
  const plfem::Symbolic* S = nullptr;
  const plfem::LaunchPlan* plan = nullptr;
  int device = 0;
  hipStream_t stream = nullptr;
  std::string err;
  int nv = 0, ne = 0, N = 0, nnz = 0, nsolve = 0, L = 0, nfronts = 0, max_ncv = 0;
  int dpn = 2, sh = 1;
  int64_t fnodes_total = 0;
  int64_t n2 = 0;
  int32_t* d_forder = nullptr;
  plfem::FrontRec* d_frec = nullptr;
  int2* d_tiles = nullptr;
  plfem::SweepJob* d_blk = nullptr;
  int32_t *d_tsorted = nullptr, *d_edof = nullptr, *d_rowptr = nullptr, *d_colind = nullptr;
  int32_t *d_slot_row = nullptr, *d_nptr = nullptr, *d_nadj = nullptr, *d_interior = nullptr;
  uint8_t* d_nloc = nullptr;
  uint8_t* d_bmask = nullptr;
  double* d_doflocs = nullptr;
  int32_t *d_fs2 = nullptr, *d_fm = nullptr;
  int64_t *d_fnode_ptr = nullptr, *d_foff = nullptr;
  int32_t *d_fnodes = nullptr, *d_cinv0 = nullptr, *d_cinv1 = nullptr;
  int32_t *d_epos = nullptr, *d_leaf_elem_ptr = nullptr, *d_leaf_elems = nullptr;
  double* d_cores = nullptr;
  double* d_layers = nullptr;
  int nlayer = 0;
  double eps_bg = 0.0;
  plfem::IndexMap map;
  double* d_elem = nullptr;
  double* d_vals[PLFEM_BLK_COUNT] = {nullptr};
  double* d_front = nullptr;
  double* d_schur = nullptr;
  int64_t arena_doubles = 0;
  int64_t* d_soff = nullptr;
  double* d_fvec = nullptr;
  double *d_u0 = nullptr, *d_u1 = nullptr;
  double* d_xl = nullptr;
  int32_t* d_npos = nullptr;
  int32_t* d_prow = nullptr;
  double *d_wbuf = nullptr, *d_rbuf = nullptr;
  double* d_dinv = nullptr;
  double* d_delta = nullptr;
  double* d_fvec2 = nullptr;
  int32_t* d_counters = nullptr;
  double *d_V = nullptr, *d_BV = nullptr, *d_V2 = nullptr, *d_BV2 = nullptr;
  double *d_w = nullptr, *d_bw = nullptr, *d_t1 = nullptr, *d_t2 = nullptr;
  double *d_hblk = nullptr, *d_G = nullptr, *d_Rinv = nullptr;
  double *d_h = nullptr, *d_hacc = nullptr, *d_partial = nullptr, *d_scal = nullptr, *d_S = nullptr;
  double* d_Hcols = nullptr;
  uint8_t* d_coremask = nullptr;
  double* d_post = nullptr;
  size_t post_doubles = 0;
  size_t partial_doubles = 0;
  double* h_pinned = nullptr;
  size_t h_pinned_bytes = 0;
  double* h_staging = nullptr;
  size_t h_staging_bytes = 0;
  double* h_slots = nullptr;
  char* slab = nullptr;
  size_t slab_off = 0, slab_bytes = 0;
  bool own_slab = false;
  int64_t workspace_need = 0;
  bool assembled = false, factored = false;
  hipEvent_t ev_step[2] = {nullptr, nullptr};
  bool defer_sync = false;
  hipStream_t copy_stream = nullptr;
  hipEvent_t ev_copy = nullptr;
  hipEvent_t ev_upload = nullptr;
  bool upload_pending = false;
  bool prof_on = false;
  unsigned prof_toggle = 0;
  int prof_n = 0, prof_max = 0;
  std::vector<hipEvent_t> prof_ev;
  std::vector<int> prof_slot;
  std::vector<double> prof_rbytes;
  int refine_steps = 0;
  void (*test_post_factor)(plfem_ctx*) = nullptr;
  double test_perturb = 0.0;
  int max_block_p = plfem::BLOCK_P;
  double sigma = 0.0;
  hipEvent_t ev[plfem::PH_COUNT][2] = {};
  bool ev_used[plfem::PH_COUNT] = {};
  double* modes_dev = nullptr;
  int modes_k = 0;
};

namespace {
template <class Owner>
int check_launch(Owner* owner, const char* what) {
  const hipError_t e = hipGetLastError();
  if (e == hipSuccess) return PLFEM_OK;
  owner->err = std::string(what) + ": " + hipGetErrorString(e);
  return PLFEM_EHIP;
}

int wait_for_upload(plfem_ctx* c) {
  if (!c->upload_pending) return PLFEM_OK;
  HIP_TRY(c, hipStreamWaitEvent(c->stream, c->ev_upload, 0));
  c->upload_pending = false;
  return PLFEM_OK;
}

hipError_t phase_begin(plfem_ctx* c, plfem::Phase ph) { return hipEventRecord(c->ev[ph][0], c->stream); }
hipError_t phase_end(plfem_ctx* c, plfem::Phase ph) {
  const hipError_t e = hipEventRecord(c->ev[ph][1], c->stream);
  if (e == hipSuccess) c->ev_used[ph] = true;
  return e;
}
double phase_us(const plfem_ctx* c, plfem::Phase ph) {
  float ms = 0;
  return (c->ev_used[ph] && hipEventElapsedTime(&ms, c->ev[ph][0], c->ev[ph][1]) == hipSuccess) ? ms * 1e3 : 0.0;
}
}

namespace plfem {

inline int prof_open(plfem_ctx* c, int slot, double bytes) {
  if (!c->prof_on || c->prof_n >= c->prof_max) return -1;
  while ((int)c->prof_ev.size() < 2 * (c->prof_n + 1)) {
    hipEvent_t e;
    if (hipEventCreate(&e) != hipSuccess) return -1;
    c->prof_ev.push_back(e);
  }
  const int id = c->prof_n++;
  c->prof_slot.push_back(slot);
  c->prof_rbytes.push_back(bytes);
  (void)hipEventRecord(c->prof_ev[2 * id], c->stream);
  return id;
}
inline void prof_close(plfem_ctx* c, int id) {
  if (id >= 0) (void)hipEventRecord(c->prof_ev[2 * id + 1], c->stream);
}

template <int V, int... Rest, class F>
inline void with_constant(int v, F&& f) {
  if constexpr (sizeof...(Rest) == 0) f(std::integral_constant<int, V>());
  else if (v == V) f(std::integral_constant<int, V>());
  else with_constant<Rest...>(v, f);
}

template <int V, bool DESC = false>
__device__ __forceinline__ int multi_reduce_index(int lane) {
  int idx = 0;
#pragma unroll
  for (int h = V / 2, s = 0; h >= 1; h >>= 1, ++s) idx += ((DESC ? lane >> (5 - s) : lane >> s) & 1) ? h : 0;
  return idx;
}

template <int H, int BIT, bool DESC, int V>
__device__ __forceinline__ void multi_reduce_step(double (&a)[V], int lane) {
  if constexpr (H >= 1) {
    const bool up = (lane & BIT) != 0;
#pragma unroll
    for (int k = 0; k < H; ++k) {
      const double send = up ? a[k] : a[k + H];
      const double keep = up ? a[k + H] : a[k];
      a[k] = keep + __shfl_xor(send, BIT);
    }
    multi_reduce_step<H / 2, DESC ? BIT / 2 : 2 * BIT, DESC>(a, lane);
  }
}

template <int V, bool DESC = false>
__device__ __forceinline__ void multi_reduce(double (&a)[V], int lane) {
  multi_reduce_step<V / 2, DESC ? 32 : 1, DESC>(a, lane);
  if constexpr (DESC) {
#pragma unroll
    for (int off = 32 / V; off >= 1; off >>= 1) a[0] += __shfl_xor(a[0], off);
  } else {
#pragma unroll
    for (int off = V; off < 64; off <<= 1) a[0] += __shfl_xor(a[0], off);
  }
}

inline int ceil_div(int64_t a, int64_t b) { return (int)((a + b - 1) / b); }
inline int basis_cols(int max_ncv) { return max_ncv + 1 + BLOCK_P; }
inline int proj_cols(int max_ncv) { return basis_cols(max_ncv) + 8; }

inline const char* profile_table_error(const double* layers, int nlayer, double eps_bg) {
  if (nlayer < 0 || nlayer > MAX_LAYERS) return "nlayer must be in [0, 64]";
  if (nlayer > 0 && !layers) return "null layer table";
  if (!std::isfinite(eps_bg) || !(eps_bg > 0.0)) return "the background permittivity must be finite and positive";
  for (int l = 0; l < nlayer; ++l) {
    const double* p = layers + LAYER_DOUBLES * l;
    for (int j = 0; j < LAYER_DOUBLES; ++j)
      if (!std::isfinite(p[j])) return "every layer entry must be finite";
    if (p[2] < 0.0) return "r_in must be >= 0";
    if (!(p[3] > p[2])) return "r_out must be > r_in";
    if (!(p[4] > 0.0) || !(p[5] > 0.0)) return "permittivities must be positive";
    if (p[6] < 0.0) return "g must be >= 0";
  }
  return nullptr;
}

inline const char* index_map_error(const double* eps, int nx, int ny, double x0, double y0, double dx, double dy) {
  if (nx < 2 || ny < 2 || nx > MAP_NMAX || ny > MAP_NMAX || (int64_t)nx * ny > MAP_SAMPLES)
    return "nx and ny must be in [2, 8192] with nx ny <= 2^24 (a null map with nx = ny = 0 clears)";
  if (!eps) return "null map";
  if (!std::isfinite(x0) || !std::isfinite(y0)) return "the origin must be finite";
  if (!std::isfinite(dx) || !std::isfinite(dy) || !(dx > 0.0) || !(dy > 0.0) || !std::isfinite(1.0 / dx) ||
      !std::isfinite(1.0 / dy))
    return "the steps must be finite and positive, with finite inverses";
  for (int64_t i = 0, n = (int64_t)nx * ny; i < n; ++i)
    if (!std::isfinite(eps[i]) || !(eps[i] > 0.0)) return "every permittivity must be finite and positive";
  return nullptr;
}

template <class Owner>
int set_index_map(Owner* o, const char* entry, const double* eps, int nx, int ny, double x0, double y0, double dx, double dy) {
  IndexMap& m = o->map;
  const bool clear = !eps && nx == 0 && ny == 0;
  if (!clear) {
    if (const char* bad = index_map_error(eps, nx, ny, x0, y0, dx, dy)) {
      o->err = std::string(entry) + ": " + bad;
      return PLFEM_EINVAL;
    }
  }
  if (clear && !m.d) return PLFEM_OK;
  HIP_TRY(o, hipSetDevice(o->device));
  const size_t n = clear ? 0 : (size_t)nx * ny;
  if (clear || m.cap < n) {
    HIP_TRY(o, hipStreamSynchronize(o->stream));
    double* old = m.d;
    m = IndexMap();
    if (old) HIP_TRY(o, hipFree(old));
    if (clear) return PLFEM_OK;
    HIP_TRY(o, hipMalloc((void**)&m.d, sizeof(double) * (MAP_HEADER + n)));
    m.cap = n;
  }
  m.nx = 0;
  const IndexMapHeader head{x0, y0, 1.0 / dx, 1.0 / dy, nx, ny};
// ... 60 lines not shown
```

### pl_fem_vectoriel_amd/csrc/kernels_front.hip

```cpp
#include <algorithm>

#include <type_traits>

#include "device.h"

namespace plfem {
namespace {

typedef double v4d __attribute__((ext_vector_type(4)));

__device__ __forceinline__ double* schur_of(int f, const int64_t* __restrict__ soff, double* __restrict__ schur, int64_t arena) {
  const int level = 31 - __clz(f + 1);
  return schur + (level & 1) * arena + soff[f];
}

template <int sh>
__global__ __launch_bounds__(256) void k_leaf_assemble(
    int first_front, int ne, double sigma, const int32_t* __restrict__ fs2, const int32_t* __restrict__ fm,
    const int64_t* __restrict__ foff, const int64_t* __restrict__ soff,
    const int64_t* __restrict__ fnode_ptr, const int32_t* __restrict__ fnodes,
    const int32_t* __restrict__ leaf_elem_ptr, const int32_t* __restrict__ leaf_elems,
    const int32_t* __restrict__ epos, const double* __restrict__ elem, double* __restrict__ front,
    double* __restrict__ schur, int64_t arena) {
  const int lf = blockIdx.x;
// ... 137 lines not shown
    const double r2 = fast_rcp(d2);
    const double l0 = past_first ? y0 * r1 : 0.0;
    const double l1 = past_second ? fma(-l0, b, y1) * r2 : 0.0;
#pragma unroll
    for (int cc = 0; cc < 4; ++cc) v[cc] = fma(-l1, fma(-g, ra[cc], rb[cc]), fma(-l0, ra[cc], v[cc]));
    d0 = r1;
    d1 = r2;
    od = 0.0;
    asm volatile("" ::: "memory");
  } else {
    double dt = det;
    if (__builtin_expect(!(fabs(dt) >= thr * s), 0)) {
      dt = (dt < 0.0) ? -rep * s : rep * s;
      nper += 1;
    }
    const double rd = fast_rcp(dt);
    const double x11 = c * rd, x12 = -b * rd, x22 = a * rd;
    const double l0 = past_second ? fma(y0, x11, y1 * x12) : 0.0;
    const double l1 = past_second ? fma(y0, x12, y1 * x22) : 0.0;
#pragma unroll
    for (int cc = 0; cc < 4; ++cc) v[cc] = fma(-l1, rb[cc], fma(-l0, ra[cc], v[cc]));
    d0 = x11;
    d1 = x22;
    od = x12;
    asm volatile("" ::: "memory");
  }
}

struct PivotLds {
  double row[2][2][NB];
  double col[2][2][NB];
  double rmax[NB];
};

__device__ __forceinline__ void ldl_pivot_block(const double* src, int64_t ld, int nbk, int tid,
                                                double (*tile)[NB + 1], double* __restrict__ sDd, double* __restrict__ sDo,
                                                PivotLds& S, int32_t* __restrict__ counters) {
  static_assert(NB == 32, "thread map of ldl_pivot_block");
  const int i = tid & 31, cg = tid >> 5;
  double v[4];
  double rmax = 0.0;
#pragma unroll
  for (int cc = 0; cc < 4; ++cc) {
    const int c = 4 * cg + cc;
    v[cc] = (i < nbk && c < nbk) ? src[(int64_t)c * ld + i] : (i == c ? 1.0 : 0.0);
    rmax = fmax(rmax, fabs(v[cc]));
  }
  __syncthreads();
  tile[cg][i] = rmax;
  __syncthreads();
  if (tid < NB) {
    double r = 0.0;
#pragma unroll
    for (int g = 0; g < 8; ++g) r = fmax(r, fmax(tile[g][tid], tile[g][tid ^ 1]));
    S.rmax[tid] = r;
  }
  double dd = 1.0, od = 0.0;
  int nper = 0;
#pragma unroll
  for (int q = 0; q < NB / 2; ++q) {
    const int k = 2 * q, cgk = k >> 2, pc = k & 3, buf = q & 1;
    if (k >= nbk) break;
    if (cg == cgk) {
      S.col[buf][0][i] = v[pc];
      S.col[buf][1][i] = v[pc + 1];
      v[pc] = (i == k) ? 1.0 : 0.0;
      v[pc + 1] = (i == k + 1) ? 1.0 : 0.0;
    }
    if ((i | 1) == k + 1) {
#pragma unroll
      for (int cc = 0; cc < 4; ++cc) S.row[buf][i & 1][4 * cg + cc] = v[cc];
    }
    __syncthreads();
    const double a = S.col[buf][0][k], b = S.col[buf][0][k + 1], c = S.col[buf][1][k + 1];
    const double thr = fmax(1e-13 * S.rmax[k], 1e-300), rep = fmax(1e-8 * S.rmax[k], 1e-300);
    const double y0 = (i > k) ? S.col[buf][0][i] : 0.0, y1 = (i > k + 1) ? S.col[buf][1][i] : 0.0;
    double ra[4], rb[4];
#pragma unroll
    for (int cc = 0; cc < 4; ++cc) {
      const int cidx = 4 * cg + cc;
      const bool behind = cidx > k + 1;
      ra[cc] = behind ? S.col[buf][0][cidx] : S.row[buf][0][cidx];
      rb[cc] = behind ? S.col[buf][1][cidx] : S.row[buf][1][cidx];
    }
    double d0, d1, o01;
    pair_step(a, b, c, thr, rep, i > k, i > k + 1, y0, y1, ra, rb, v, d0, d1, o01, nper);
    if ((i | 1) == k + 1) {
      dd = (i == k) ? d0 : d1;
      od = o01;
    }
  }
  __syncthreads();
#pragma unroll
  for (int cc = 0; cc < 4; ++cc) {
    const int c = 4 * cg + cc;
    tile[i][c] = (c <= i) ? v[cc] : 0.0;
  }
  if (tid < NB) {
    sDd[i] = dd;
    sDo[i] = od;
  }
  if (tid == 0 && nper > 0 && counters) atomicAdd(&counters[0], nper);
}

__device__ __forceinline__ void store_pivot_results(int f, int k0, int nbk, int64_t np,
                                                    double* __restrict__ dinv, double* __restrict__ delta,
                                                    double (*tile)[NB + 1], const double* __restrict__ sDd,
                                                    const double* __restrict__ sDo) {
  double* D = dinv + (int64_t)f * NB * NB;
  for (int e = threadIdx.x; e < NB * NB; e += 256) D[e] = tile[e & (NB - 1)][e >> 5];
  if ((int)threadIdx.x < nbk)
    reinterpret_cast<double2*>(delta)[2 * np + k0 + threadIdx.x] = make_double2(sDd[threadIdx.x], sDo[threadIdx.x]);
}

struct PanelOperands {
  double xa0[NB / 4], xa1[NB / 4], rdd[2][4], rdo[2][4];
  __device__ __forceinline__ void load(const double (*tile)[NB + 1], const double* sDd, const double* sDo, int nbk, int lr, int lk) {
#pragma unroll
    for (int kk = 0; kk < NB / 4; ++kk) {
      xa0[kk] = tile[lr][4 * kk + lk];
      xa1[kk] = tile[16 + lr][4 * kk + lk];
    }
#pragma unroll
    for (int tc = 0; tc < 2; ++tc)
#pragma unroll
      for (int r = 0; r < 4; ++r) {
        const int c = 16 * tc + lk + 4 * r;
        rdd[tc][r] = (c < nbk) ? sDd[c] : 0.0;
        rdo[tc][r] = (c < nbk) ? sDo[c] : 0.0;
      }
  }
  __device__ __forceinline__ void rows(const double (&b)[NB / 4], int nbk, int kcol, int64_t m, int i, int lk,
                                       double* __restrict__ W, double* __restrict__ Y, double* __restrict__ F) const {
    v4d y0 = (v4d){0.0, 0.0, 0.0, 0.0}, y1 = (v4d){0.0, 0.0, 0.0, 0.0};
#pragma unroll
    for (int kk = 0; kk < NB / 4; ++kk) {
      y0 = __builtin_amdgcn_mfma_f64_16x16x4f64(xa0[kk], b[kk], y0, 0, 0, 0);
      y1 = __builtin_amdgcn_mfma_f64_16x16x4f64(xa1[kk], b[kk], y1, 0, 0, 0);
    }
#pragma unroll
    for (int tc = 0; tc < 2; ++tc)
#pragma unroll
      for (int r = 0; r < 4; ++r) {
        const int c = 16 * tc + lk + 4 * r;
        const double y = tc == 0 ? y0[r] : y1[r];
        const double w = fma(y, rdd[tc][r], lane_xor16(y, lk & 1) * rdo[tc][r]);
        W[(int64_t)c * m + i] = w;
        Y[(int64_t)c * m + i] = y;
        if (c < nbk) F[(int64_t)(kcol + c) * m + i] = w;
      }
  }
};

__global__ __launch_bounds__(256) void k_ldl_first_panel(const FrontRec* __restrict__ frec, double* __restrict__ front,
                                                         double* __restrict__ dinv, double* __restrict__ delta,
                                                         double* __restrict__ wbuf, double* __restrict__ rbuf,
                                                         int32_t* __restrict__ counters) {
  const FrontRec R = frec[blockIdx.x];
  const int f = R.f;
  const int s2 = R.s2;
  const int nbk = min(NB, s2);
  const int m = R.m;
  double* F = front + R.foff;
  const int wave = threadIdx.x >> 6, lane = threadIdx.x & 63;
  const int bx = blockIdx.y;
  const int n_pan = gridDim.y;
  const int t0 = nbk;
  if (bx > 0 && t0 + bx * 64 >= m) return;
  __shared__ __attribute__((aligned(16))) PivotLds piv;
  __shared__ double tile[NB][NB + 1];
  __shared__ double sDd[NB], sDo[NB];
  const int lr = lane & 15, lk = lane >> 4;
  double b[NB / 4];
  {
    const int ibase = t0 + bx * 64 + 16 * wave;
#pragma unroll
    for (int kk = 0; kk < NB / 4; ++kk) {
      const int jx = 4 * kk + lk;
      b[kk] = (ibase < m && jx < nbk) ? F[(int64_t)jx * m + ibase + lr] : 0.0;
    }
  }
  ldl_pivot_block(F, m, nbk, threadIdx.x, tile, sDd, sDo, piv, bx == 0 ? counters : nullptr);
  __syncthreads();
  if (bx == 0) store_pivot_results(f, 0, nbk, R.np, dinv, delta, tile, sDd, sDo);
  double* W = wbuf + 2 * R.np * NB;
  double* Y = rbuf + 2 * R.np * NB;
  PanelOperands po;
  po.load(tile, sDd, sDo, nbk, lr, lk);
  for (int ch = bx; t0 + ch * 64 < m; ch += n_pan) {
    const int ibase = t0 + ch * 64 + 16 * wave;
    if (ibase >= m) break;
    const int i = ibase + lr;
    if (ch != bx) {
#pragma unroll
      for (int kk = 0; kk < NB / 4; ++kk) {
        const int jx = 4 * kk + lk;
        b[kk] = (jx < nbk) ? F[(int64_t)jx * m + i] : 0.0;
      }
    }
    po.rows(b, nbk, 0, m, i, lk, W, Y, F);
  }
}

__device__ __forceinline__ void ldl_invrow_block(int f, int bx, int kb, const int32_t* __restrict__ fs2,
                                                 const int32_t* __restrict__ fm, const int64_t* __restrict__ foff,
                                                 double* __restrict__ front, const double* __restrict__ dinv,
                                                 double* __restrict__ part ) {
  const int s2 = fs2[f];
  const int k0 = kb * NB;
  if (k0 >= s2 || k0 == 0) return;
  const int wave = threadIdx.x >> 6, lane = threadIdx.x & 63;
  const int c0 = bx * 16;
  if (c0 >= k0) return;
  const int nbk = min(NB, s2 - k0);
  const int m = fm[f];
  double* F = front + foff[f];
  const double* D = dinv + (int64_t)f * NB * NB;
  const int lr = lane & 15, lk = lane >> 4;
  const int c = c0 + lr;
  v4d t0 = (v4d){0.0, 0.0, 0.0, 0.0}, t1 = (v4d){0.0, 0.0, 0.0, 0.0};
  auto groups = [&](int j0, auto G_) {
    constexpr int G = decltype(G_)::value;
    double a0[4 * G], a1[4 * G], b[4 * G];
#pragma unroll
    for (int t = 0; t < 4 * G; ++t) {
      const int j = j0 + 4 * t + lk;
      a0[t] = F[(int64_t)j * m + k0 + lr];
      a1[t] = (nbk > 16) ? F[(int64_t)j * m + k0 + 16 + lr] : 0.0;
      b[t] = (j >= c) ? F[(int64_t)j * m + c] : 0.0;
    }
#pragma unroll
    for (int t = 0; t < 4 * G; ++t) {
      t0 = __builtin_amdgcn_mfma_f64_16x16x4f64(a0[t], b[t], t0, 0, 0, 0);
      t1 = __builtin_amdgcn_mfma_f64_16x16x4f64(a1[t], b[t], t1, 0, 0, 0);
    }
  };
  const int ngroups = (k0 - c0) / 16;
  int j0 = c0 + 16 * (wave * ngroups / 4);
  const int j_end = c0 + 16 * ((wave + 1) * ngroups / 4);
  for (; j0 + 16 < j_end; j0 += 32) groups(j0, std::integral_constant<int, 2>());
  if (j0 < j_end) groups(j0, std::integral_constant<int, 1>());
  if (wave > 0) {
#pragma unroll
    for (int r = 0; r < 4; ++r) {
      part[((wave - 1) * 8 + r) * 64 + lane] = t0[r];
      part[((wave - 1) * 8 + 4 + r) * 64 + lane] = t1[r];
    }
  }
  __syncthreads();
  if (wave > 0) return;
#pragma unroll
  for (int w = 0; w < 3; ++w)
#pragma unroll
    for (int r = 0; r < 4; ++r) {
      t0[r] += part[(w * 8 + r) * 64 + lane];
      t1[r] += part[(w * 8 + 4 + r) * 64 + lane];
    }
  v4d x0 = (v4d){0.0, 0.0, 0.0, 0.0}, x1 = (v4d){0.0, 0.0, 0.0, 0.0};
#pragma unroll
  for (int kk = 0; kk < 8; ++kk) {
    const int q = 4 * kk + lk;
    const double a0 = -D[(int64_t)q * NB + lr];
    const double a1 = -D[(int64_t)q * NB + 16 + lr];
    const double b = kk < 4 ? t0[kk & 3] : t1[kk & 3];
    x0 = __builtin_amdgcn_mfma_f64_16x16x4f64(a0, b, x0, 0, 0, 0);
    x1 = __builtin_amdgcn_mfma_f64_16x16x4f64(a1, b, x1, 0, 0, 0);
  }
#pragma unroll
  for (int r = 0; r < 4; ++r) {
    const int r0 = lk + 4 * r, r1 = 16 + lk + 4 * r;
    if (r0 < nbk) F[(int64_t)(k0 + r0) * m + c] = x0[r];
    if (r1 < nbk) F[(int64_t)(k0 + r1) * m + c] = x1[r];
  }
}

template <int MODE>
__device__ __forceinline__ void ldl_update_tile(const int2 job, int kb, const int32_t* __restrict__ fs2,
                                                const int32_t* __restrict__ fm, const int64_t* __restrict__ foff,
                                                const int64_t* __restrict__ soff, const int64_t* __restrict__ fnode_ptr,
                                                double* __restrict__ front, double* __restrict__ schur, int64_t arena,
                                                const double* __restrict__ wbuf, const double* __restrict__ rbuf,
                                                const double* __restrict__ wbuf_prev, const double* __restrict__ rbuf_prev) {
  const int f = job.x;
  const int s2 = fs2[f];
  const int k0 = kb * NB;
  if (k0 >= s2) return;
  const int m = fm[f];
  const int nbk = min(NB, s2 - k0);
  const int t0 = k0 + nbk;
  const int wave = threadIdx.x >> 6, lane = threadIdx.x & 63;
  const int i0 = t0 + ((job.y & 0xffff) * 2 + (wave & 1)) * 32;
  const int j0 = t0 + ((job.y >> 16) * 2 + (wave >> 1)) * 32;
  if (i0 >= m || j0 >= m) return;
  if (i0 < j0) return;
  const int ncol = (t0 < s2 && j0 == t0) ? min(NB, s2 - t0) : 0;
  if ((MODE == 0 && t0 < s2) || ncol == NB) return;
  double* F = front + foff[f];
  double* S = schur_of(f, soff, schur, arena);
  const int b2 = m - s2;
  const int lr = lane & 15, lk = lane >> 4;
  const bool iv1 = i0 + 16 < m, jv1 = j0 + 16 < m;
  auto quad_ok = [&](int tj, int ti) { return (tj == 0 || jv1) && (ti == 0 || iv1) && !(j0 + 16 * tj >= s2 && i0 + 16 * ti < s2); };
  auto addr = [&](int tj, int ti, int r) -> double* {
    const int j = j0 + 16 * tj + lk + 4 * r, i = i0 + 16 * ti + lr;
    return j0 + 16 * tj < s2 ? F + (int64_t)j * m + i : S + (int64_t)(j - s2) * b2 + (i - s2);
  };
  double fv[2][2][4];
#pragma unroll
  for (int tj = 0; tj < 2; ++tj)
#pragma unroll
    for (int ti = 0; ti < 2; ++ti)
#pragma unroll
      for (int r = 0; r < 4; ++r) fv[tj][ti][r] = quad_ok(tj, ti) ? *addr(tj, ti, r) : 0.0;
  v4d acc[2][2];
#pragma unroll
  for (int tj = 0; tj < 2; ++tj)
#pragma unroll
    for (int ti = 0; ti < 2; ++ti) acc[tj][ti] = (v4d){0.0, 0.0, 0.0, 0.0};
#pragma unroll
  for (int pass = 0; pass <= MODE; ++pass) {
    const double* W = (pass == 0 ? wbuf : wbuf_prev) + 2 * fnode_ptr[f] * NB;
    const double* Y = (pass == 0 ? rbuf : rbuf_prev) + 2 * fnode_ptr[f] * NB;
    double a0[NB / 4], a1[NB / 4], b0[NB / 4], b1[NB / 4];
#pragma unroll
    for (int it = 0; it < NB / 4; ++it) {
      const int64_t col = (int64_t)(4 * it + lk) * m;
      a0[it] = Y[col + j0 + lr];
      a1[it] = jv1 ? Y[col + j0 + 16 + lr] : 0.0;
      b0[it] = W[col + i0 + lr];
      b1[it] = iv1 ? W[col + i0 + 16 + lr] : 0.0;
    }
#pragma unroll
    for (int it = 0; it < NB / 4; ++it) {
      acc[0][0] = __builtin_amdgcn_mfma_f64_16x16x4f64(a0[it], b0[it], acc[0][0], 0, 0, 0);
      acc[0][1] = __builtin_amdgcn_mfma_f64_16x16x4f64(a0[it], b1[it], acc[0][1], 0, 0, 0);
      acc[1][0] = __builtin_amdgcn_mfma_f64_16x16x4f64(a1[it], b0[it], acc[1][0], 0, 0, 0);
      acc[1][1] = __builtin_amdgcn_mfma_f64_16x16x4f64(a1[it], b1[it], acc[1][1], 0, 0, 0);
    }
  }
#pragma unroll
  for (int tj = 0; tj < 2; ++tj) {
#pragma unroll
    for (int ti = 0; ti < 2; ++ti) {
      if (!quad_ok(tj, ti)) continue;
      if (16 * tj < ncol) continue;
#pragma unroll
      for (int r = 0; r < 4; ++r) *addr(tj, ti, r) = fv[tj][ti][r] - acc[tj][ti][r];
    }
  }
}

template <int MODE>
__device__ __forceinline__ void ldl_column_block(const FrontRec& R, int bx, int n_pan, int kb, double* __restrict__ front,
                                                 double* __restrict__ dinv_next, double* __restrict__ delta,
                                                 const double* __restrict__ wbuf, const double* __restrict__ rbuf,
                                                 const double* __restrict__ wbuf_prev, const double* __restrict__ rbuf_prev,
                                                 double* __restrict__ wbuf_next, double* __restrict__ rbuf_next,
                                                 int32_t* __restrict__ counters) {
  const int f = R.f, s2 = R.s2;
  const int k0 = kb * NB;
  const int t0 = k0 + NB;
  if (t0 >= s2) return;
  const int nbn = min(NB, s2 - t0);
  const int m = R.m;
  const int t1 = t0 + nbn;
  if (bx > 0 && t1 + bx * 64 >= m) return;
  double* F = front + R.foff;
  __shared__ __attribute__((aligned(16))) PivotLds piv;
  __shared__ double tile[NB][NB + 1];
  __shared__ double sDd[NB], sDo[NB];
  const int wave = threadIdx.x >> 6, lane = threadIdx.x & 63;
  const int lr = lane & 15, lk = lane >> 4;
  const int64_t pbase = 2 * R.np * NB;
  const bool full = nbn > 16;
  const int qi = wave & 1, qj = wave >> 1;
  const bool quad_on = 16 * qi < nbn && 16 * qj < nbn;
  auto strip = [&](int ibase, double (&bq)[NB / 4], auto QUAD_, int m, int64_t pbase) {
    constexpr bool QUAD = decltype(QUAD_)::value;
    const bool rows_on = ibase < m;
    const int i = (rows_on ? ibase : t0) + lr;
    double fv[2][4], qv[4];
#pragma unroll
    for (int tj = 0; tj < 2; ++tj)
#pragma unroll
      for (int r = 0; r < 4; ++r) fv[tj][r] = (tj == 0 || full) ? F[(int64_t)(t0 + 16 * tj + lk + 4 * r) * m + i] : 0.0;
    if (QUAD) {
#pragma unroll
      for (int r = 0; r < 4; ++r) qv[r] = quad_on ? F[(int64_t)(t0 + 16 * qj + lk + 4 * r) * m + (t0 + 16 * qi + lr)] : 0.0;
    }
    v4d acc[2] = {(v4d){0.0, 0.0, 0.0, 0.0}, (v4d){0.0, 0.0, 0.0, 0.0}};
    v4d qacc = (v4d){0.0, 0.0, 0.0, 0.0};
#pragma unroll
    for (int pass = 0; pass <= MODE; ++pass) {
      const double* W = (pass == 0 ? wbuf : wbuf_prev) + pbase;
      const double* Y = (pass == 0 ? rbuf : rbuf_prev) + pbase;
      double ya[2][NB / 4], b[NB / 4], qb[NB / 4];
#pragma unroll
      for (int it = 0; it < NB / 4; ++it) {
        const int64_t col = (int64_t)(4 * it + lk) * m;
        ya[0][it] = Y[col + t0 + lr];
        ya[1][it] = full ? Y[col + t0 + 16 + lr] : 0.0;
        b[it] = W[col + i];
        if (QUAD) qb[it] = W[col + t0 + 16 * qi + lr];
      }
#pragma unroll
      for (int it = 0; it < NB / 4; ++it) {
        acc[0] = __builtin_amdgcn_mfma_f64_16x16x4f64(ya[0][it], b[it], acc[0], 0, 0, 0);
        acc[1] = __builtin_amdgcn_mfma_f64_16x16x4f64(ya[1][it], b[it], acc[1], 0, 0, 0);
        if (QUAD) qacc = __builtin_amdgcn_mfma_f64_16x16x4f64(qj == 0 ? ya[0][it] : ya[1][it], qb[it], qacc, 0, 0, 0);
      }
    }
#pragma unroll
    for (int tj = 0; tj < 2; ++tj)
#pragma unroll
      for (int r = 0; r < 4; ++r) bq[r + 4 * tj] = (tj == 0 || full) ? fv[tj][r] - acc[tj][r] : 0.0;
    if (QUAD && quad_on) {
#pragma unroll
      for (int r = 0; r < 4; ++r) tile[16 * qj + lk + 4 * r][16 * qi + lr] = qv[r] - qacc[r];
    }
  };
  double bq[NB / 4];
  const int ibase0 = t1 + bx * 64 + 16 * wave;
  strip(ibase0, bq, std::true_type(), m, pbase);
  __syncthreads();
  ldl_pivot_block(&tile[0][0], NB + 1, nbn, threadIdx.x, tile, sDd, sDo, piv, bx == 0 ? counters : nullptr);
  __syncthreads();
  if (bx == 0) store_pivot_results(f, t0, nbn, R.np, dinv_next, delta, tile, sDd, sDo);
  double* Wn = wbuf_next + pbase;
  double* Yn = rbuf_next + pbase;
  if (ibase0 >= m) return;
  {
    PanelOperands po;
    po.load(tile, sDd, sDo, nbn, lr, lk);
    po.rows(bq, nbn, t0, m, ibase0 + lr, lk, Wn, Yn, F);
  }
  for (int ibase = ibase0 + n_pan * 64; ibase < m; ibase += n_pan * 64) {
    int ml = m;
    int64_t pl = pbase;
    asm volatile("" : "+s"(ml), "+s"(pl) : : "memory");
    strip(ibase, bq, std::false_type(), ml, pl);
    asm volatile("" ::: "memory");
    PanelOperands po;
    po.load(tile, sDd, sDo, nbn, lr, lk);
    po.rows(bq, nbn, t0, ml, ibase + lr, lk, wbuf_next + pl, rbuf_next + pl, F);
  }
}

template <int MODE>
__global__ __launch_bounds__(256) __attribute__((amdgpu_waves_per_eu(3, 3))) void k_ldl_update(
    int un, int n_inv, int n_look, int n_pan, const int2* __restrict__ tiles, const int32_t* __restrict__ forder,
    const FrontRec* __restrict__ frec, int kb,
    const int32_t* __restrict__ fs2, const int32_t* __restrict__ fm, const int64_t* __restrict__ foff,
    const int64_t* __restrict__ soff, const int64_t* __restrict__ fnode_ptr, double* __restrict__ front,
    double* __restrict__ schur, int64_t arena, const double* __restrict__ dinv, double* __restrict__ dinv_next,
    double* __restrict__ delta, const double* __restrict__ wbuf, const double* __restrict__ rbuf,
    const double* __restrict__ wbuf_prev, const double* __restrict__ rbuf_prev, double* __restrict__ wbuf_next,
    double* __restrict__ rbuf_next, int32_t* __restrict__ counters) {
  int bid = blockIdx.x;
  if (bid < n_look * n_pan) {
    const FrontRec R = frec[bid / n_pan];
    ldl_column_block<MODE>(R, bid % n_pan, n_pan, kb, front, dinv_next, delta, wbuf, rbuf, wbuf_prev, rbuf_prev, wbuf_next,
                           rbuf_next, counters);
    return;
  }
  bid -= n_look * n_pan;
  if (bid < un) {
    ldl_update_tile<MODE>(tiles[bid], kb, fs2, fm, foff, soff, fnode_ptr, front, schur, arena, wbuf, rbuf, wbuf_prev, rbuf_prev);
    return;
  }
  bid -= un;
  const int f = forder[bid / (n_inv + 1)];
  const int sub = bid % (n_inv + 1);
  if (sub < n_inv) {
    __shared__ double part[3 * 8 * 64];
    ldl_invrow_block(f, sub, kb, fs2, fm, foff, front, dinv, part);
    return;
  }
  const int s2 = fs2[f];
  const int k0 = kb * NB;
  if (k0 >= s2) return;
  const int nbk = min(NB, s2 - k0);
  const int m = fm[f];
  double* F = front + foff[f];
  const double* D = dinv + (int64_t)f * NB * NB;
  for (int q = threadIdx.x; q < NB * NB; q += 256) {
    const int i = q & (NB - 1), c = q >> 5;
    if (i < nbk && c < nbk) F[(int64_t)(k0 + c) * m + (k0 + i)] = (i >= c) ? D[i + c * NB] : D[c + i * NB];
  }
}

__device__ __forceinline__ void mirror_x_block(const int2 job, const int32_t* __restrict__ fs2, const int32_t* __restrict__ fm,
                                               const int64_t* __restrict__ foff, double* __restrict__ front,
                                               double (*tile)[33]) {
  const int f = job.x, k0 = job.y * NB;
  const int m = fm[f], s2 = fs2[f];
  const int nbk = min(NB, s2 - k0);
  double* F = front + foff[f];
  const int tx = threadIdx.x & 31, ty = threadIdx.x >> 5;
  for (int c0 = 0; c0 < k0; c0 += 32) {
    for (int yy = ty; yy < 32; yy += 8)
      tile[yy][tx] = (yy < nbk) ? F[(int64_t)(k0 + yy) * m + c0 + tx] : 0.0;
    __syncthreads();
    for (int yy = ty; yy < 32; yy += 8)
      if (tx < nbk) F[(int64_t)(c0 + yy) * m + k0 + tx] = tile[tx][yy];
    __syncthreads();
  }
}

__global__ __launch_bounds__(256) void k_form_z_mirror(const int2* __restrict__ jobs, int nz, const int32_t* __restrict__ fs2,
                                                       const int32_t* __restrict__ fm, const int64_t* __restrict__ foff,
                                                       double* __restrict__ front) {
  __shared__ double lds[4][32][33];
  const int2 job = jobs[blockIdx.x];
  if ((int)blockIdx.x >= nz) {
    mirror_x_block(job, fs2, fm, foff, front, lds[0]);
    return;
  }
  const int f = job.x;
  const int m = fm[f], s2 = fs2[f];
  const int b2 = m - s2;
  const int wave = threadIdx.x >> 6, lane = threadIdx.x & 63;
  const int b0 = (job.y * 2 + (wave & 1)) * 32;
  const bool rows_on = b0 < b2;
  double* F = front + foff[f];
  double* FZ = F + (int64_t)m * s2;
  const int lr = lane & 15, lk = lane >> 4;
  const bool bv1 = b0 + 16 < b2;
  double (*tile)[33] = lds[wave];
  for (int cstep = 0; cstep < s2; cstep += 64) {
    const int c0 = cstep + 32 * (wave >> 1);
    const bool on = rows_on && c0 < s2;
    const bool cv1 = c0 + 16 < s2;
    v4d acc[2][2];
    for (int tb = 0; tb < 2; ++tb)
      for (int tc = 0; tc < 2; ++tc) acc[tb][tc] = (v4d){0.0, 0.0, 0.0, 0.0};
    if (on) {
      const int cA = c0 + lr, cB = c0 + 16 + lr;
      for (int j0 = c0; j0 < s2; j0 += 16) {
        double a0[4], a1[4], x0[4], x1[4];
#pragma unroll
        for (int t = 0; t < 4; ++t) {
          const int j = j0 + 4 * t + lk;
          a0[t] = F[(int64_t)j * m + s2 + b0 + lr];
          a1[t] = bv1 ? F[(int64_t)j * m + s2 + b0 + 16 + lr] : 0.0;
          x0[t] = (j >= cA) ? F[(int64_t)j * m + cA] : 0.0;
          x1[t] = (cv1 && j >= cB) ? F[(int64_t)j * m + cB] : 0.0;
        }
#pragma unroll
        for (int t = 0; t < 4; ++t) {
          acc[0][0] = __builtin_amdgcn_mfma_f64_16x16x4f64(a0[t], x0[t], acc[0][0], 0, 0, 0);
          acc[0][1] = __builtin_amdgcn_mfma_f64_16x16x4f64(a0[t], x1[t], acc[0][1], 0, 0, 0);
          acc[1][0] = __builtin_amdgcn_mfma_f64_16x16x4f64(a1[t], x0[t], acc[1][0], 0, 0, 0);
          acc[1][1] = __builtin_amdgcn_mfma_f64_16x16x4f64(a1[t], x1[t], acc[1][1], 0, 0, 0);
        }
      }
      for (int tb = 0; tb < 2; ++tb)
        for (int tc = 0; tc < 2; ++tc)
#pragma unroll
          for (int r = 0; r < 4; ++r) {
            const int bb = 16 * tb + lk + 4 * r, cc = 16 * tc + lr;
            tile[cc][bb] = acc[tb][tc][r];
            if ((tb == 0 || bv1) && (tc == 0 || cv1)) FZ[(int64_t)(b0 + bb) * s2 + (c0 + cc)] = acc[tb][tc][r];
          }
    }
    __syncthreads();
    if (on) {
      const int bb = lane & 31;
#pragma unroll 4
      for (int cc = lane >> 5; cc < 32; cc += 2)
        if (b0 + bb < b2 && c0 + cc < s2) F[(int64_t)(c0 + cc) * m + s2 + b0 + bb] = tile[cc][bb];
    }
  }
}

}

void launch_factor(plfem_ctx* c, double sigma, int stop_level, int stop_step, int stop_stage) {
  hipStream_t st = c->stream;
  const LaunchPlan& plan = *c->plan;
  (void)hipMemsetAsync(c->d_counters, 0, 4 * sizeof(int32_t), st);
  for (int lev = c->L; lev >= 0; --lev) {
    const LevelInfo& li = plan.levels[lev];
    if (lev == c->L) {
      const int64_t lo = c->S->foff[li.first], hi = c->S->foff[li.first + li.count];
      (void)hipMemsetAsync(c->d_front + lo, 0, sizeof(double) * (size_t)(hi - lo), st);
      int64_t sch = 0;
      for (int f = li.first; f < li.first + li.count; ++f) {
        const int64_t b2 = (int64_t)c->dpn * c->S->fb[f];
        sch = std::max(sch, c->S->soff[f] + b2 * b2);
      }
      (void)hipMemsetAsync(c->d_schur + (size_t)(lev & 1) * c->arena_doubles, 0, sizeof(double) * (size_t)sch, st);
      with_constant<0, 1>(c->sh, [&](auto sh) {
        hipLaunchKernelGGL(k_leaf_assemble<decltype(sh)::value>, dim3(li.count), dim3(256), 0, st, li.first, c->ne, sigma, c->d_fs2,
                           c->d_fm, c->d_foff, c->d_soff, c->d_fnode_ptr, c->d_fnodes, c->d_leaf_elem_ptr, c->d_leaf_elems, c->d_epos,
                           c->d_elem, c->d_front, c->d_schur, c->arena_doubles);
      });
    } else if (li.gather_n > 0) {
      with_constant<0, 1>(c->sh, [&](auto sh) {
        hipLaunchKernelGGL(k_front_gather<decltype(sh)::value>, dim3(li.gather_n), dim3(256), 0, st, c->d_tiles + li.gather_off,
                           c->d_fs2, c->d_fm, c->d_foff, c->d_soff, c->d_fnode_ptr, c->d_fnodes, c->d_cinv0, c->d_cinv1, c->d_front,
                           c->d_schur, c->arena_doubles);
      });
    }
    if (lev == stop_level && stop_stage == 0) return;
    const int steps = (li.max_s2 + NB - 1) / NB;
    const int32_t* ford = c->d_forder + li.first;
    const FrontRec* frec = c->d_frec + li.first;
    const int* hs2 = plan.forder_s2.data() + li.first;
    const int* hpm = plan.forder_maxm.data() + li.first;
    for (int kb = 0; kb < steps; ++kb) {
      const bool stop_here = (lev == stop_level && kb == stop_step);
      const int k0 = kb * NB;
      int nact = 0;
      {
        int lo = 0, hi = li.count;
        while (lo < hi) { int mid = (lo + hi) / 2; if (hs2[mid] > k0) lo = mid + 1; else hi = mid; }
        nact = lo;
      }
      if (nact == 0) break;
      const size_t third = (size_t)2 * plan.level_nodes_max * NB;
      const int64_t base = 2 * c->S->fnode_ptr[li.first] * NB;
      double* wb0 = c->d_wbuf - base;
      double* rb0 = c->d_rbuf - base;
      double* wb = wb0 + (kb % 3) * third;
      double* rb = rb0 + (kb % 3) * third;
      double* wb_prev = wb0 + ((kb + 2) % 3) * third;
      double* rb_prev = rb0 + ((kb + 2) % 3) * third;
      double* wb_next = wb0 + ((kb + 1) % 3) * third;
      double* rb_next = rb0 + ((kb + 1) % 3) * third;
      double* dinv_cur = c->d_dinv + (size_t)(kb & 1) * c->nfronts * NB * NB;
      double* dinv_nxt = c->d_dinv + (size_t)((kb + 1) & 1) * c->nfronts * NB * NB;
      auto panel_wgs = [&](int rows_below, int cap) {
        int n = std::max(1, rows_below > 0 ? (rows_below + 63) / 64 : 0);
        return li.count > 64 ? std::min(n, cap) : n;
      };
      if (kb == 0) {
        const int n_pan0 = panel_wgs(hpm[nact - 1] - 16, 2);
        hipLaunchKernelGGL(k_ldl_first_panel, dim3(nact, n_pan0), dim3(256), 0, st, frec, c->d_front, dinv_cur, c->d_delta, wb, rb,
                           c->d_counters);
      }
      if (stop_here && stop_stage >= 1 && stop_stage <= 2) return;
      const int un = plan.upd_n[li.step0 + kb];
      const int n_inv = kb > 0 ? (k0 + 15) / 16 : 0;
      const int2* ut = c->d_tiles + plan.upd_off[li.step0 + kb];
      int n_look = 0;
      {
        int lo = 0, hi = nact;
        while (lo < hi) { int mid = (lo + hi) / 2; if (hs2[mid] > k0 + NB) lo = mid + 1; else hi = mid; }
        n_look = lo;
      }
      const int cap = li.count >= 1024 ? 1 : 4;
      const int n_pan = n_look > 0 ? panel_wgs(hpm[n_look - 1] - (k0 + NB) - 16, cap) : 1;
      const unsigned gridB = (unsigned)(n_look * n_pan + un + nact * (n_inv + 1));
      with_constant<0, 1>(kb & 1, [&](auto mode) {
        hipLaunchKernelGGL(k_ldl_update<decltype(mode)::value>, dim3(gridB), dim3(256), 0, st, un, n_inv, n_look, n_pan, ut, ford,
                           frec, kb, c->d_fs2, c->d_fm, c->d_foff, c->d_soff, c->d_fnode_ptr, c->d_front, c->d_schur, c->arena_doubles,
                           dinv_cur, dinv_nxt, c->d_delta, wb, rb, mode ? wb_prev : wb, mode ? rb_prev : rb, wb_next, rb_next,
                           c->d_counters);
      });
      if (stop_here && (stop_stage == 3 || stop_stage == 4)) return;
    }
    if (stop_level >= 0 && li.formz_n + li.mirrorx_n > 0)
      hipLaunchKernelGGL(k_form_z_mirror, dim3(li.formz_n + li.mirrorx_n), dim3(256), 0, st, c->d_tiles + li.formz_off, li.formz_n,
                         c->d_fs2, c->d_fm, c->d_foff, c->d_front);
    if (lev == stop_level && stop_stage == 5) return;
  }
  if (stop_level < 0 && plan.formz_all_n + plan.mirrorx_all_n > 0)
    hipLaunchKernelGGL(k_form_z_mirror, dim3(plan.formz_all_n + plan.mirrorx_all_n), dim3(256), 0, st, c->d_tiles + plan.formz_all_off,
                       plan.formz_all_n, c->d_fs2, c->d_fm, c->d_foff, c->d_front);
}

}
```

### pl_fem_vectoriel_amd/csrc/plan.cpp

```cpp
#include "plan.h"

#include <algorithm>
#include <functional>

#include "symbolic.h"

namespace plfem {

void build_launch_plan(const Symbolic& S, LaunchPlan& P, const PlanTasks& par) {
  auto run = [&](int ntasks, const std::function<void(int)>& f) {
    if (par) par(ntasks, f);
    else for (int q = 0; q < ntasks; ++q) f(q);
  };
  const int nf = S.nfronts, L = S.L, dpn = S.dpn;
  P.fs2.resize(nf);
  P.fm.resize(nf);
  std::vector<int32_t>& fs2 = P.fs2;
  std::vector<int32_t>& fm = P.fm;
  P.levels.assign(L + 1, LevelInfo());
  P.forder.resize(nf);
  std::vector<int32_t>& forder = P.forder;
  P.forder_s2.assign(nf, 0);
  P.forder_maxm.assign(nf, 0);
  auto cdiv = [](int a, int b) { return (a + b - 1) / b; };
  auto gen_jobs = [&](int lev, bool fwd, SweepJob* out) -> int64_t {
    const LevelInfo& li = P.levels[lev];
    const int32_t* o = forder.data() + li.first;
    int64_t n = 0;
    auto put = [&](int f, int rb) {
      if (out) out[n] = SweepJob{f, rb, fm[f], fs2[f], S.fnode_ptr[f], f > 0 ? S.fnode_ptr[(f - 1) >> 1] : 0, S.foff[f], 0};
      ++n;
    };
    for (int q = 0; q < li.count; ++q) {
      const int f = o[q];
      if (fwd) {
        if (li.fwd_rows == 64 && fs2[f] > MIX_BIG_S2)
          for (int t = 0; t * 16 < fm[f]; ++t) put(f, t | SWEEP_ROW_JOB_FLAG);
        else
          for (int t = 0; t * li.fwd_rows < fm[f]; ++t) put(f, t);
      } else {
        const int rows = std::max(fs2[f], lev < L ? 1 : 0);
        for (int t = 0; t * li.bwd_rows < rows; ++t) put(f, t);
      }
    }
    return n;
  };
  auto lower = [](int f, int nt, Tile* out, int64_t& pos) {
    if (out)
      for (int ty = 0; ty < nt; ++ty)
        for (int tx = ty; tx < nt; ++tx) out[pos++] = Tile{f, tx | (ty << 16)};
    else
      pos += (int64_t)nt * (nt + 1) / 2;
  };
  auto gen_gather = [&](int lev, Tile* out) -> int64_t {
    const LevelInfo& li = P.levels[lev];
    const int32_t* o = forder.data() + li.first;
    int64_t pos = 0;
    if (lev < L)
      for (int q = 0; q < li.count; ++q) lower(o[q], cdiv(fm[o[q]], 64), out, pos);
    return pos;
  };
  auto gen_update = [&](int lev, int kb, Tile* out) -> int64_t {
    const LevelInfo& li = P.levels[lev];
    const int32_t* o = forder.data() + li.first;
    const int k0 = kb * NB;
    int64_t pos = 0;
    for (int q = 0; q < li.count && fs2[o[q]] > k0; ++q) {
      const int f = o[q];
      const int t0 = k0 + std::min(NB, fs2[f] - k0);
      if (!((kb & 1) == 0 && t0 < fs2[f])) lower(f, cdiv(fm[f] - t0, 64), out, pos);
    }
    return pos;
  };
  auto gen_formz = [&](int lev, Tile* out) -> int64_t {
    const LevelInfo& li = P.levels[lev];
    const int32_t* o = forder.data() + li.first;
    int64_t pos = 0;
    for (int q = 0; q < li.count; ++q) {
      const int f = o[q];
      if (fs2[f] == 0) continue;
      for (int tb = 0; tb < cdiv(fm[f] - fs2[f], 64); ++tb) {
        if (out) out[pos] = Tile{f, tb};
        ++pos;
      }
    }
    return pos;
  };
  auto gen_mirrorx = [&](int lev, Tile* out) -> int64_t {
    const LevelInfo& li = P.levels[lev];
    const int32_t* o = forder.data() + li.first;
    int64_t pos = 0;
    for (int q = 0; q < li.count; ++q)
      for (int kb = cdiv(fs2[o[q]], NB) - 1; kb >= 1; --kb) {
        if (out) out[pos] = Tile{o[q], kb};
        ++pos;
      }
    return pos;
  };
  struct Counts { int64_t fwd = 0, bwd = 0, gather = 0, formz = 0, mirrorx = 0; std::vector<int64_t> upd; };
  std::vector<Counts> cnt(L + 1);
  run(L + 1, [&](int lev) {
    LevelInfo& li = P.levels[lev];
    li.first = (1 << lev) - 1;
    li.count = 1 << lev;
    for (int f = li.first; f < li.first + li.count; ++f) {
      fs2[f] = dpn * S.fs[f];
      fm[f] = dpn * (S.fs[f] + S.fb[f]);
      li.max_m = std::max(li.max_m, fm[f]);
      li.max_s2 = std::max(li.max_s2, fs2[f]);
      li.max_b2 = std::max(li.max_b2, fm[f] - fs2[f]);
      li.sweep_bytes += 8.0 * ((double)fs2[f] * fm[f] - 0.5 * (double)fs2[f] * fs2[f] + fm[f] + fs2[f]);
      li.sweep_vec_doubles += fm[f] + fs2[f];
    }
    int32_t* o = forder.data() + li.first;
    const int nb = li.max_s2 / 16 + 2;
    std::vector<int32_t> bucket(nb, 0);
    for (int f = li.first; f < li.first + li.count; ++f) bucket[nb - 2 - fs2[f] / 16 + 1]++;
    for (int b = 1; b < nb; ++b) bucket[b] += bucket[b - 1];
    for (int f = li.first; f < li.first + li.count; ++f) o[bucket[nb - 2 - fs2[f] / 16]++] = f;
    int mx = 0;
    for (int q = 0; q < li.count; ++q) {
      mx = std::max(mx, fm[o[q]]);
      P.forder_s2[li.first + q] = fs2[o[q]];
      P.forder_maxm[li.first + q] = mx;
    }
    li.fwd_rows = fwd_block_rows(li.count);
    li.bwd_rows = bwd_block_rows(li.count, lev == L);
    for (int q = 0; q < li.count; ++q)
      if (li.fwd_rows == 64 && fs2[o[q]] > MIX_BIG_S2) li.fwd_mixed = true;
    Counts& c = cnt[lev];
    c.fwd = gen_jobs(lev, true, nullptr);
    c.bwd = gen_jobs(lev, false, nullptr);
    c.gather = gen_gather(lev, nullptr);
    const int steps = (li.max_s2 + NB - 1) / NB;
    c.upd.resize(steps);
    for (int kb = 0; kb < steps; ++kb) c.upd[kb] = gen_update(lev, kb, nullptr);
    c.formz = gen_formz(lev, nullptr);
    c.mirrorx = gen_mirrorx(lev, nullptr);
  });
  P.worst_m = 0;
  struct Fill { int kind, lev, kb; int64_t off; };
  std::vector<Fill> fills;
  int64_t njobs = 0, pos = 0;
  P.upd_off.clear();
  P.upd_n.clear();
  for (int lev = 0; lev <= L; ++lev) {
    LevelInfo& li = P.levels[lev];
    const Counts& c = cnt[lev];
    P.worst_m = std::max(P.worst_m, li.max_m);
    li.fwd_off = njobs; li.fwd_n = (int)c.fwd;
    fills.push_back({0, lev, 0, njobs});
    njobs += c.fwd;
    li.bwd_off = njobs; li.bwd_n = (int)c.bwd;
    fills.push_back({1, lev, 0, njobs});
    njobs += c.bwd;
    li.gather_off = pos; li.gather_n = (int)c.gather;
    if (c.gather) fills.push_back({2, lev, 0, pos});
    pos += c.gather;
    li.step0 = (int)P.upd_n.size();
    for (int kb = 0; kb < (int)c.upd.size(); ++kb) {
      P.upd_off.push_back(pos);
      P.upd_n.push_back((int)c.upd[kb]);
      if (c.upd[kb]) fills.push_back({3, lev, kb, pos});
      pos += c.upd[kb];
    }
    li.formz_off = pos; li.formz_n = (int)c.formz;
    if (c.formz) fills.push_back({4, lev, 0, pos});
    pos += c.formz;
    li.mirrorx_off = pos; li.mirrorx_n = (int)c.mirrorx;
    if (c.mirrorx) fills.push_back({5, lev, 0, pos});
    pos += c.mirrorx;
  }
  P.formz_all_off = pos;
  for (int lev = 0; lev <= L; ++lev) {
    if (cnt[lev].formz) fills.push_back({6, lev, 0, pos});
    pos += cnt[lev].formz;
  }
  P.formz_all_n = (int)(pos - P.formz_all_off);
  P.mirrorx_all_off = pos;
  for (int lev = 0; lev <= L; ++lev) {
    if (cnt[lev].mirrorx) fills.push_back({7, lev, 0, pos});
    pos += cnt[lev].mirrorx;
  }
  P.mirrorx_all_n = (int)(pos - P.mirrorx_all_off);
  for (int lev = 0; lev <= L; ++lev) fills.push_back({8, lev, 0, 0});
  P.jobs.resize((size_t)njobs);
  P.tiles.resize((size_t)pos);
  P.frec.resize(nf);
  std::stable_sort(fills.begin(), fills.end(), [&](const Fill& a, const Fill& b) { return a.lev > b.lev; });
  run((int)fills.size(), [&](int t) {
    const Fill& F = fills[t];
    switch (F.kind) {
      case 0: gen_jobs(F.lev, true, P.jobs.data() + F.off); break;
      case 1: gen_jobs(F.lev, false, P.jobs.data() + F.off); break;
      case 2: gen_gather(F.lev, P.tiles.data() + F.off); break;
      case 3: gen_update(F.lev, F.kb, P.tiles.data() + F.off); break;
      case 4: case 6: gen_formz(F.lev, P.tiles.data() + F.off); break;
      case 5: case 7: gen_mirrorx(F.lev, P.tiles.data() + F.off); break;
      default: {
        const LevelInfo& li = P.levels[F.lev];
        for (int q = li.first; q < li.first + li.count; ++q) {
          const int f = forder[q];
          P.frec[q] = FrontRec{f, fm[f], fs2[f], 0, S.foff[f], S.fnode_ptr[f]};
        }
      }
    }
  });
  int64_t level_nodes = 0;
  for (int lev = 0; lev <= L; ++lev) {
    const int first = (1 << lev) - 1, last = std::min(nf, (1 << (lev + 1)) - 1);
    level_nodes = std::max(level_nodes, S.fnode_ptr[last] - S.fnode_ptr[first]);
  }
  P.level_nodes_max = level_nodes;
  P.built = true;
}

}
```

### pl_fem_vectoriel_amd/csrc/plan.h

```cpp
#pragma once
#include <cstdint>
#include <functional>
#include <memory>
#include <utility>
#include <vector>

namespace plfem {

template <class T>
struct default_init_allocator : std::allocator<T> {
  template <class U>
  struct rebind { using other = default_init_allocator<U>; };
  using std::allocator<T>::allocator;
  template <class U>
  void construct(U* ptr) noexcept { ::new (static_cast<void*>(ptr)) U; }
  template <class U, class... Args>
  void construct(U* ptr, Args&&... args) { ::new (static_cast<void*>(ptr)) U(std::forward<Args>(args)...); }
};

constexpr int NB = 32;
constexpr int PANEL_CHUNK = 1024;
constexpr int FIRST_ROWS = 1024;
constexpr int FIRST_THREADS = 256;
constexpr int FIRST_COLS = 8;
constexpr int SPMV_WG_ROWS = 32;
constexpr int POST_ROWS = 256;
constexpr int POST_SUMS = 5;
constexpr int RESID_SUMS = 2;
constexpr int ROW_FORM_MAX_FRONTS = 32;
constexpr int MIX_BIG_S2 = 192;
constexpr int SWEEP_ROW_JOB_FLAG = 1 << 30;
struct alignas(16) SweepJob {
  int32_t f, rb;
  int32_t m, s2;
  int64_t np, npp;
  int64_t foff;
  int64_t reserved;
};
static_assert(sizeof(SweepJob) == 48, "SweepJob layout");
struct alignas(16) FrontRec {
  int32_t f, m, s2, reserved;
  int64_t foff, np;
};
static_assert(sizeof(FrontRec) == 32, "FrontRec layout");
inline int fwd_block_rows(int count) { return count <= 8 ? 8 : count <= ROW_FORM_MAX_FRONTS ? 16 : 64; }
inline int bwd_block_rows(int count, bool leaf) { return leaf ? 64 : count <= ROW_FORM_MAX_FRONTS ? 8 : 16; }
constexpr int BLOCK_P = 4;
constexpr int MAX_CORES = 64;
constexpr int MAP_NMAX = 8192;
constexpr int64_t MAP_SAMPLES = 1 << 24;
constexpr int MAP_HEADER = 8;
constexpr int MAX_LAYERS = 64;
constexpr int LAYER_DOUBLES = 8;
constexpr int ELEM_FORMS = 8;
constexpr int ELEM_STRIDE = ELEM_FORMS * 36;

struct LevelInfo {
  int first = 0;
  int count = 0;
  int max_m = 0;
  int max_s2 = 0;
  int max_b2 = 0;
  int64_t gather_off = 0, formz_off = 0, mirrorx_off = 0;
  int gather_n = 0, formz_n = 0, mirrorx_n = 0, step0 = 0;
  int fwd_rows = 0, bwd_rows = 0;
  bool fwd_mixed = false;
  int64_t fwd_off = 0, bwd_off = 0;
  int fwd_n = 0, bwd_n = 0;
  double sweep_bytes = 0;
  double sweep_vec_doubles = 0;
};

struct Tile { int32_t x, y; };
static_assert(sizeof(Tile) == 8, "Tile layout");

struct Symbolic;
struct LaunchPlan {
  bool built = false;
  std::vector<int32_t> fs2, fm;
  std::vector<int32_t> forder;
  std::vector<int32_t> forder_s2, forder_maxm;
  std::vector<FrontRec, default_init_allocator<FrontRec>> frec;
  std::vector<LevelInfo> levels;
  std::vector<SweepJob, default_init_allocator<SweepJob>> jobs;
  std::vector<Tile, default_init_allocator<Tile>> tiles;
  std::vector<int64_t> upd_off;
  std::vector<int32_t> upd_n;
  int64_t formz_all_off = 0, mirrorx_all_off = 0;
  int32_t formz_all_n = 0, mirrorx_all_n = 0;
  int64_t level_nodes_max = 0;
  int32_t worst_m = 0;
};
using PlanTasks = std::function<void(int ntasks, const std::function<void(int)>& f)>;
void build_launch_plan(const Symbolic& S, LaunchPlan& P, const PlanTasks& par = {});

}
```

Measured before the change: 517.3.

## Precompute per-front column-panel job lists with per-front workgroup counts

Replaces the uniform 2D grid of panel workgroups (nact x n_pan, with n_pan sized by the largest front and capped) with a precomputed flat list of column jobs. Each job carries its own bx and n_pan, sized per front from its remaining rows under a workgroup budget that shrinks when many update tiles are co-launched. The host-side binary searches per step move into the symbolic plan. The aim is to stop idle or early-exiting workgroups on small fronts and to give big fronts more panel parallelism, at the cost of a larger plan and the budget heuristic.

```diff
diff --git a/include/plfem.h b/include/plfem.h
--- a/include/plfem.h
+++ b/include/plfem.h
@@ -191,6 +191,11 @@
 #define PLFEM_DEBUG_PLAN_FIELDS 10
 int plfem_debug_solve_block(plfem_ctx* ctx, const double* rhs_dev, int64_t ldx, double* x_dev, int32_t refine_steps);
 int plfem_debug_level_plan(plfem_ctx* ctx, int64_t* out, int64_t cap);
+#define PLFEM_DEBUG_COLUMN_FIELDS 9
+int plfem_debug_column_policy(const int32_t* chunks, int32_t n, int64_t budget, int32_t* w);
+int plfem_debug_column_lists(plfem_ctx* ctx, int64_t* out, int64_t cap, int64_t* count);
+int plfem_debug_symbolic_column_lists(const plfem_symbolic* sym, int64_t budget, int64_t* out, int64_t cap, int64_t* count);
+int plfem_debug_set_column_budget(plfem_ctx* ctx, int64_t budget);
 enum { PLFEM_DEBUG_PANEL_DOT = 0, PLFEM_DEBUG_PANEL_AXPY, PLFEM_DEBUG_PANEL_DOT_BLOCK, PLFEM_DEBUG_PANEL_AXPY_BLOCK };
 enum { PLFEM_DEBUG_SPMV_B_BLOCK = 0, PLFEM_DEBUG_SPMV_B_BLOCK_IL, PLFEM_DEBUG_SPMV_B_BLOCK_IL_GRAM, PLFEM_DEBUG_SPMV_A_BLOCK };
 int plfem_debug_panel(plfem_ctx* ctx, int32_t form, int32_t ncols, const double* Pm, double* W, int64_t ldw, double* H,
diff --git a/pl_fem_vectoriel_amd/_native.py b/pl_fem_vectoriel_amd/_native.py
--- a/pl_fem_vectoriel_amd/_native.py
+++ b/pl_fem_vectoriel_amd/_native.py
@@ -44,11 +44,14 @@
 TEST_HOOK_EXPORTS = ("plfem_debug_factor_until", "plfem_debug_copy", "plfem_debug_symeig", "plfem_debug_symeig_band",
                      "plfem_debug_set_perturb", "plfem_debug_solve_block", "plfem_debug_level_plan", "plfem_debug_panel",
                      "plfem_debug_scale_store", "plfem_debug_first_pass", "plfem_debug_spmv_block", "plfem_debug_chol",
-                     "plfem_debug_block_scale", "plfem_debug_rotate", "plfem_debug_start_field", "plfem_debug_set_elements")
+                     "plfem_debug_block_scale", "plfem_debug_rotate", "plfem_debug_start_field", "plfem_debug_set_elements",
+                     "plfem_debug_column_policy", "plfem_debug_column_lists", "plfem_debug_symbolic_column_lists",
+                     "plfem_debug_set_column_budget")
 PANEL_FORMS = ("dot", "axpy", "dot_block", "axpy_block")
 SPMV_BLOCK_FORMS = ("b_block", "b_block_il", "b_block_il_gram", "a_block")
 BLOCK_P = 4
 PLAN_FIELDS = ("count", "fwd_rows", "bwd_rows", "fwd_mixed", "max_s2", "max_m", "fwd_n", "bwd_n", "steps", "max_block_p")
+COLUMN_FIELDS = ("level", "kb", "nact", "n_list", "f", "m", "s2", "bx", "n_pan")
 MAX_NCV = 320
 PROF_SLOTS = ("k_fwd", "fwd_sweep", "bwd_sweep", "spmv_b")
 
@@ -327,8 +330,37 @@
     h.plfem_debug_block_scale.argtypes = [vp, vp, vp, i64, vp, vp, vp, i64, vp, i32, vp, vp, i32]
     h.plfem_debug_rotate.argtypes = [vp, vp, i32, vp, i32, i32, vp]
     h.plfem_debug_start_field.argtypes = [vp, i32, vp]
+    h.plfem_debug_column_policy.argtypes = [vp, i32, i64, vp]
+    h.plfem_debug_column_lists.argtypes = [vp, vp, i64, vp]
+    h.plfem_debug_symbolic_column_lists.argtypes = [vp, i64, vp, i64, vp]
+    h.plfem_debug_set_column_budget.argtypes = [vp, i64]
     _hooks = h
     return h
+
+
+def debug_column_policy(chunks, budget: int) -> np.ndarray:
+    chunks = np.ascontiguousarray(chunks, dtype=np.int32)
+    w = np.zeros(chunks.size, dtype=np.int32)
+    rc = load_test_hooks().plfem_debug_column_policy(_ptr(chunks), int(chunks.size), ctypes.c_int64(int(budget)), _ptr(w))
+    if rc != PLFEM_OK:
+        raise ValueError(f"plfem_debug_column_policy failed ({rc})")
+    return w
+
+
+def _column_records(call) -> np.ndarray:
+    count = ctypes.c_int64(0)
+    call(None, 0, ctypes.byref(count))
+    out = np.zeros((count.value, len(COLUMN_FIELDS)), dtype=np.int64)
+    rc = call(_ptr(out), ctypes.c_int64(out.size), ctypes.byref(count))
+    if rc != PLFEM_OK:
+        raise ValueError(f"column list hook failed ({rc})")
+    return out
+
+
+def debug_symbolic_column_lists(sym, budget: int = -1) -> np.ndarray:
+    h = load_test_hooks()
+    return _column_records(lambda out, cap, count: h.plfem_debug_symbolic_column_lists(sym._h, ctypes.c_int64(int(budget)),
+                                                                                        out, cap, count))
 
 
 def debug_symeig(a, last_rows: int = -1):
@@ -676,6 +708,14 @@
                     "plfem_debug_level_plan")
         return [dict(zip(PLAN_FIELDS, (int(v) for v in row))) for row in out.reshape(nl, len(PLAN_FIELDS))]
 
+    def debug_column_lists(self) -> np.ndarray:
+        h = load_test_hooks()
+        return _column_records(lambda out, cap, count: h.plfem_debug_column_lists(self._h, out, cap, count))
+
+    def debug_set_column_budget(self, budget: int):
+        self._check(load_test_hooks().plfem_debug_set_column_budget(self._h, ctypes.c_int64(int(budget))),
+                    "plfem_debug_set_column_budget")
+
     def profile_begin(self, max_launches: int = 4096):
         self._check(self._lib.plfem_profile_begin(self._h, int(max_launches)), "plfem_profile_begin")
 
diff --git a/pl_fem_vectoriel_amd/csrc/api_debug.hip b/pl_fem_vectoriel_amd/csrc/api_debug.hip
--- a/pl_fem_vectoriel_amd/csrc/api_debug.hip
+++ b/pl_fem_vectoriel_amd/csrc/api_debug.hip
@@ -1,6 +1,7 @@
 #include <algorithm>
 #include <cmath>
 #include <cstring>
+#include <memory>
 #include <numeric>
 #include <string>
 #include <vector>
@@ -118,6 +119,42 @@
   return PLFEM_OK;
 } catch (...) { return host_failure(c); }
 
+namespace plfem {
+int debug_column_records(const LaunchPlan& P, const ColumnLists& C, int64_t* out, int64_t cap, int64_t* count);
+}
+namespace {
+struct OwnColumns {
+  plfem::ColumnLists lists;
+  plfem::FrontRec* d = nullptr;
+  ~OwnColumns() { if (d) (void)hipFree(d); }
+};
+}
+
+extern "C" int plfem_debug_column_lists(plfem_ctx* c, int64_t* out, int64_t cap, int64_t* count) try {
+  if (!c || !count) return PLFEM_EINVAL;
+  const int rc = plfem::debug_column_records(*c->plan, *c->cols, out, cap, count);
+  if (rc != PLFEM_OK) c->err = "debug column lists: cap too small";
+  return rc;
+} catch (...) { return host_failure(c); }
+
+extern "C" int plfem_debug_set_column_budget(plfem_ctx* c, int64_t budget) try {
+  if (!c || budget < 0) return PLFEM_EINVAL;
+  HIP_TRY(c, hipSetDevice(c->device));
+  TRY(wait_for_upload(c));
+  HIP_TRY(c, hipStreamSynchronize(c->stream));
+  auto own = std::make_shared<OwnColumns>();
+  plfem::build_column_lists(*c->S, *c->plan, budget, own->lists);
+  const size_t bytes = sizeof(plfem::FrontRec) * std::max<size_t>(own->lists.jobs.size(), 1);
+  HIP_TRY(c, hipMalloc((void**)&own->d, bytes));
+  if (!own->lists.jobs.empty())
+    HIP_TRY(c, hipMemcpy(own->d, own->lists.jobs.data(), sizeof(plfem::FrontRec) * own->lists.jobs.size(), hipMemcpyHostToDevice));
+  c->cols = &own->lists;
+  c->d_cols = own->d;
+  c->test_owned = std::move(own);
+  c->factored = false;
+  return PLFEM_OK;
+} catch (...) { return host_failure(c); }
+
 namespace {
 int lanczos_hook_done(plfem_ctx* c, const char* what) {
   HIP_TRY(c, hipStreamSynchronize(c->stream));
diff --git a/pl_fem_vectoriel_amd/csrc/api_debug_host.cpp b/pl_fem_vectoriel_amd/csrc/api_debug_host.cpp
--- a/pl_fem_vectoriel_amd/csrc/api_debug_host.cpp
+++ b/pl_fem_vectoriel_amd/csrc/api_debug_host.cpp
@@ -7,6 +7,46 @@
 #include "../../include/plfem.h"
 #include "host_eig.h"
 #include "internal.h"
+
+namespace plfem {
+int debug_column_records(const LaunchPlan& P, const ColumnLists& C, int64_t* out, int64_t cap, int64_t* count) {
+  *count = (int64_t)C.jobs.size();
+  if (!out) return PLFEM_OK;
+  if (cap < (int64_t)PLFEM_DEBUG_COLUMN_FIELDS * *count) return PLFEM_EINVAL;
+  auto put = [&](int lev, int kb, int nact, int listed, int64_t off, int n) {
+    for (int64_t q = off; q < off + n; ++q) {
+      const FrontRec& R = C.jobs[q];
+      const int64_t rec[PLFEM_DEBUG_COLUMN_FIELDS] = {lev, kb, nact, listed, R.f, R.m, R.s2, column_job_bx(R.reserved),
+                                                      column_job_n_pan(R.reserved)};
+      std::copy(rec, rec + PLFEM_DEBUG_COLUMN_FIELDS, out + (int64_t)PLFEM_DEBUG_COLUMN_FIELDS * q);
+    }
+  };
+  const int nl = (int)P.levels.size();
+  for (int lev = 0; lev < nl; ++lev) {
+    const int s0 = P.levels[lev].step0, s1 = lev + 1 < nl ? P.levels[lev + 1].step0 : (int)P.upd_n.size();
+    if (s1 > s0) put(lev, -1, C.nact[s0], C.nact[s0], C.first_off[lev], C.first_n[lev]);
+    for (int s = s0; s < s1; ++s) put(lev, s - s0, C.nact[s], C.n_look[s], C.col_off[s], C.col_n[s]);
+  }
+  return PLFEM_OK;
+}
+}
+
+extern "C" int plfem_debug_column_policy(const int32_t* chunks, int32_t n, int64_t budget, int32_t* w) try {
+  if (n < 0 || budget < 0 || (n > 0 && (!chunks || !w))) return PLFEM_EINVAL;
+  for (int q = 0; q < n; ++q)
+    if (chunks[q] < 1) return PLFEM_EINVAL;
+  plfem::column_workgroups(chunks, n, budget, w);
+  return PLFEM_OK;
+} catch (...) { return host_failure(nullptr, 0); }
+
+extern "C" int plfem_debug_symbolic_column_lists(const plfem_symbolic* sym, int64_t budget, int64_t* out, int64_t cap,
+                                                 int64_t* count) try {
+  if (!sym || !count || !sym->S.plan.built) return PLFEM_EINVAL;
+  if (budget < 0) return plfem::debug_column_records(sym->S.plan, sym->S.plan.cols, out, cap, count);
+  plfem::ColumnLists C;
+  plfem::build_column_lists(sym->S, sym->S.plan, budget, C);
+  return plfem::debug_column_records(sym->S.plan, C, out, cap, count);
+} catch (...) { return host_failure(nullptr, 0); }
 
 extern "C" int plfem_debug_symeig(int32_t n, const double* a_host, int32_t last_rows, double* w_out, double* v_out) try {
   if (n < 1 || n > 4096 || !a_host || !w_out || !v_out || last_rows > n) return PLFEM_EINVAL;
diff --git a/pl_fem_vectoriel_amd/csrc/api_device.hip b/pl_fem_vectoriel_amd/csrc/api_device.hip
--- a/pl_fem_vectoriel_amd/csrc/api_device.hip
+++ b/pl_fem_vectoriel_amd/csrc/api_device.hip
@@ -240,7 +240,7 @@
   TRY(upload(c, items, &c->d_blk, P.jobs));
   TRY(upload(c, items, reinterpret_cast<plfem::Tile**>(&c->d_tiles), P.tiles));
   TRY(upload(c, items, &c->d_forder, P.forder));
-  TRY(upload(c, items, &c->d_frec, P.frec));
+  TRY(upload(c, items, &c->d_cols, P.cols.jobs));
   TRY(upload(c, items, &c->d_fs2, P.fs2));
   TRY(upload(c, items, &c->d_fm, P.fm));
   TRY(upload(c, items, &c->d_fnode_ptr, S.fnode_ptr));
@@ -324,6 +324,7 @@
   c->L = S.L; c->nfronts = S.nfronts; c->dpn = S.dpn; c->sh = S.dpn - 1; c->n2 = S.dpn * (int64_t)S.N; c->max_ncv = max_ncv;
   if (!S.plan.built) { c->err = "plfem_create: the analysis carries no launch plan"; return PLFEM_ESTATE; }
   c->plan = &S.plan;
+  c->cols = &S.plan.cols;
   if (!size_only) {
     int lim = 0;
     HIP_TRY(c, hipDeviceGetAttribute(&lim, hipDeviceAttributeMaxSharedMemoryPerBlock, device));
diff --git a/pl_fem_vectoriel_amd/csrc/device.h b/pl_fem_vectoriel_amd/csrc/device.h
--- a/pl_fem_vectoriel_amd/csrc/device.h
+++ b/pl_fem_vectoriel_amd/csrc/device.h
@@ -75,7 +75,8 @@
   int64_t fnodes_total = 0;
   int64_t n2 = 0;
   int32_t* d_forder = nullptr;
-  plfem::FrontRec* d_frec = nullptr;
+  const plfem::ColumnLists* cols = nullptr;
+  plfem::FrontRec* d_cols = nullptr;
   int2* d_tiles = nullptr;
   plfem::SweepJob* d_blk = nullptr;
   int32_t *d_tsorted = nullptr, *d_edof = nullptr, *d_rowptr = nullptr, *d_colind = nullptr;
@@ -142,6 +143,7 @@
   int refine_steps = 0;
   void (*test_post_factor)(plfem_ctx*) = nullptr;
   double test_perturb = 0.0;
+  std::shared_ptr<void> test_owned;
   int max_block_p = plfem::BLOCK_P;
   double sigma = 0.0;
   hipEvent_t ev[plfem::PH_COUNT][2] = {};
diff --git a/pl_fem_vectoriel_amd/csrc/kernels_front.hip b/pl_fem_vectoriel_amd/csrc/kernels_front.hip
--- a/pl_fem_vectoriel_amd/csrc/kernels_front.hip
+++ b/pl_fem_vectoriel_amd/csrc/kernels_front.hip
@@ -313,19 +313,19 @@
   }
 };
 
-__global__ __launch_bounds__(256) void k_ldl_first_panel(const FrontRec* __restrict__ frec, double* __restrict__ front,
+__global__ __launch_bounds__(256) void k_ldl_first_panel(const FrontRec* __restrict__ cols, double* __restrict__ front,
                                                          double* __restrict__ dinv, double* __restrict__ delta,
                                                          double* __restrict__ wbuf, double* __restrict__ rbuf,
                                                          int32_t* __restrict__ counters) {
-  const FrontRec R = frec[blockIdx.x];
+  const FrontRec R = cols[blockIdx.x];
   const int f = R.f;
   const int s2 = R.s2;
   const int nbk = min(NB, s2);
   const int m = R.m;
   double* F = front + R.foff;
   const int wave = threadIdx.x >> 6, lane = threadIdx.x & 63;
-  const int bx = blockIdx.y;
-  const int n_pan = gridDim.y;
+  const int bx = column_job_bx(R.reserved);
+  const int n_pan = column_job_n_pan(R.reserved);
   const int t0 = nbk;
   if (bx > 0 && t0 + bx * 64 >= m) return;
   __shared__ __attribute__((aligned(16))) PivotLds piv;
@@ -609,8 +609,8 @@
 
 template <int MODE>
 __global__ __launch_bounds__(256) __attribute__((amdgpu_waves_per_eu(3, 3))) void k_ldl_update(
-    int un, int n_inv, int n_look, int n_pan, const int2* __restrict__ tiles, const int32_t* __restrict__ forder,
-    const FrontRec* __restrict__ frec, int kb,
+    int un, int n_inv, int n_col, const int2* __restrict__ tiles, const int32_t* __restrict__ forder,
+    const FrontRec* __restrict__ cols, int kb,
     const int32_t* __restrict__ fs2, const int32_t* __restrict__ fm, const int64_t* __restrict__ foff,
     const int64_t* __restrict__ soff, const int64_t* __restrict__ fnode_ptr, double* __restrict__ front,
     double* __restrict__ schur, int64_t arena, const double* __restrict__ dinv, double* __restrict__ dinv_next,
@@ -618,13 +618,13 @@
     const double* __restrict__ wbuf_prev, const double* __restrict__ rbuf_prev, double* __restrict__ wbuf_next,
     double* __restrict__ rbuf_next, int32_t* __restrict__ counters) {
   int bid = blockIdx.x;
-  if (bid < n_look * n_pan) {
-    const FrontRec R = frec[bid / n_pan];
-    ldl_column_block<MODE>(R, bid % n_pan, n_pan, kb, front, dinv_next, delta, wbuf, rbuf, wbuf_prev, rbuf_prev, wbuf_next,
-                           rbuf_next, counters);
+  if (bid < n_col) {
+    const FrontRec R = cols[bid];
+    ldl_column_block<MODE>(R, column_job_bx(R.reserved), column_job_n_pan(R.reserved), kb, front, dinv_next, delta, wbuf, rbuf,
+                           wbuf_prev, rbuf_prev, wbuf_next, rbuf_next, counters);
     return;
   }
-  bid -= n_look * n_pan;
+  bid -= n_col;
   if (bid < un) {
     ldl_update_tile<MODE>(tiles[bid], kb, fs2, fm, foff, soff, fnode_ptr, front, schur, arena, wbuf, rbuf, wbuf_prev, rbuf_prev);
     return;
@@ -739,6 +739,7 @@
 void launch_factor(plfem_ctx* c, double sigma, int stop_level, int stop_step, int stop_stage) {
   hipStream_t st = c->stream;
   const LaunchPlan& plan = *c->plan;
+  const ColumnLists& cols = *c->cols;
   (void)hipMemsetAsync(c->d_counters, 0, 4 * sizeof(int32_t), st);
   for (int lev = c->L; lev >= 0; --lev) {
     const LevelInfo& li = plan.levels[lev];
@@ -766,19 +767,10 @@
     if (lev == stop_level && stop_stage == 0) return;
     const int steps = (li.max_s2 + NB - 1) / NB;
     const int32_t* ford = c->d_forder + li.first;
-    const FrontRec* frec = c->d_frec + li.first;
-    const int* hs2 = plan.forder_s2.data() + li.first;
-    const int* hpm = plan.forder_maxm.data() + li.first;
     for (int kb = 0; kb < steps; ++kb) {
       const bool stop_here = (lev == stop_level && kb == stop_step);
       const int k0 = kb * NB;
-      int nact = 0;
-      {
-        int lo = 0, hi = li.count;
-        while (lo < hi) { int mid = (lo + hi) / 2; if (hs2[mid] > k0) lo = mid + 1; else hi = mid; }
-        nact = lo;
-      }
-      if (nact == 0) break;
+      const int nact = cols.nact[li.step0 + kb];
       const size_t third = (size_t)2 * plan.level_nodes_max * NB;
       const int64_t base = 2 * c->S->fnode_ptr[li.first] * NB;
       double* wb0 = c->d_wbuf - base;
@@ -791,31 +783,20 @@
       double* rb_next = rb0 + ((kb + 1) % 3) * third;
       double* dinv_cur = c->d_dinv + (size_t)(kb & 1) * c->nfronts * NB * NB;
       double* dinv_nxt = c->d_dinv + (size_t)((kb + 1) & 1) * c->nfronts * NB * NB;
-      auto panel_wgs = [&](int rows_below, int cap) {
-        int n = std::max(1, rows_below > 0 ? (rows_below + 63) / 64 : 0);
-        return li.count > 64 ? std::min(n, cap) : n;
-      };
       if (kb == 0) {
-        const int n_pan0 = panel_wgs(hpm[nact - 1] - 16, 2);
-        hipLaunchKernelGGL(k_ldl_first_panel, dim3(nact, n_pan0), dim3(256), 0, st, frec, c->d_front, dinv_cur, c->d_delta, wb, rb,
-                           c->d_counters);
+        hipLaunchKernelGGL(k_ldl_first_panel, dim3(cols.first_n[lev]), dim3(256), 0, st, c->d_cols + cols.first_off[lev], c->d_front,
+                           dinv_cur, c->d_delta, wb, rb, c->d_counters);
       }
       if (stop_here && stop_stage >= 1 && stop_stage <= 2) return;
       const int un = plan.upd_n[li.step0 + kb];
       const int n_inv = kb > 0 ? (k0 + 15) / 16 : 0;
       const int2* ut = c->d_tiles + plan.upd_off[li.step0 + kb];
-      int n_look = 0;
-      {
-        int lo = 0, hi = nact;
-        while (lo < hi) { int mid = (lo + hi) / 2; if (hs2[mid] > k0 + NB) lo = mid + 1; else hi = mid; }
-        n_look = lo;
-      }
-      const int cap = li.count >= 1024 ? 1 : 4;
-      const int n_pan = n_look > 0 ? panel_wgs(hpm[n_look - 1] - (k0 + NB) - 16, cap) : 1;
-      const unsigned gridB = (unsigned)(n_look * n_pan + un + nact * (n_inv + 1));
+      const int n_col = cols.col_n[li.step0 + kb];
+      const FrontRec* dcol = c->d_cols + cols.col_off[li.step0 + kb];
+      const unsigned gridB = (unsigned)(n_col + un + nact * (n_inv + 1));
       with_constant<0, 1>(kb & 1, [&](auto mode) {
-        hipLaunchKernelGGL(k_ldl_update<decltype(mode)::value>, dim3(gridB), dim3(256), 0, st, un, n_inv, n_look, n_pan, ut, ford,
-                           frec, kb, c->d_fs2, c->d_fm, c->d_foff, c->d_soff, c->d_fnode_ptr, c->d_front, c->d_schur, c->arena_doubles,
+        hipLaunchKernelGGL(k_ldl_update<decltype(mode)::value>, dim3(gridB), dim3(256), 0, st, un, n_inv, n_col, ut, ford,
+                           dcol, kb, c->d_fs2, c->d_fm, c->d_foff, c->d_soff, c->d_fnode_ptr, c->d_front, c->d_schur, c->arena_doubles,
                            dinv_cur, dinv_nxt, c->d_delta, wb, rb, mode ? wb_prev : wb, mode ? rb_prev : rb, wb_next, rb_next,
                            c->d_counters);
       });
diff --git a/pl_fem_vectoriel_amd/csrc/plan.cpp b/pl_fem_vectoriel_amd/csrc/plan.cpp
--- a/pl_fem_vectoriel_amd/csrc/plan.cpp
+++ b/pl_fem_vectoriel_amd/csrc/plan.cpp
@@ -6,6 +6,85 @@
 #include "symbolic.h"
 
 namespace plfem {
+
+void column_workgroups(const int32_t* chunks, int n, int64_t budget, int32_t* w) {
+  if (n <= 0) return;
+  const int64_t cap = std::max<int64_t>(budget, n);
+  auto need = [&](int trips) {
+    int64_t s = 0;
+    for (int q = 0; q < n; ++q) s += (chunks[q] + trips - 1) / trips;
+    return s;
+  };
+  int lo = 1, hi = *std::max_element(chunks, chunks + n);
+  while (lo < hi) {
+    const int mid = (lo + hi) / 2;
+    if (need(mid) <= cap) hi = mid; else lo = mid + 1;
+  }
+  for (int q = 0; q < n; ++q) w[q] = (chunks[q] + lo - 1) / lo;
+}
+
+namespace {
+int active_fronts(const LaunchPlan& P, int lev, int k0) {
+  const int32_t* hs2 = P.forder_s2.data() + P.levels[lev].first;
+  return (int)(std::partition_point(hs2, hs2 + P.levels[lev].count, [&](int32_t s2) { return s2 > k0; }) - hs2);
+}
+int64_t gen_columns(const Symbolic& S, const LaunchPlan& P, int lev, int kb, int64_t un, int64_t budget, FrontRec* out) {
+  if (budget < 0)
+    budget = column_budget(kb < 0 ? 0 : un + (int64_t)active_fronts(P, lev, kb * NB) * ((kb * NB + 15) / 16 + 1));
+  const int32_t* o = P.forder.data() + P.levels[lev].first;
+  const int n = active_fronts(P, lev, (kb + 1) * NB);
+  std::vector<int32_t> chunks(n), w(n);
+  for (int q = 0; q < n; ++q) chunks[q] = column_chunks(P.fm[o[q]], kb + 1);
+  column_workgroups(chunks.data(), n, budget, w.data());
+  int64_t pos = 0;
+  for (int q = 0; q < n; ++q) {
+    const int f = o[q];
+    if (out)
+      for (int bx = 0; bx < w[q]; ++bx)
+        out[pos + bx] = FrontRec{f, P.fm[f], P.fs2[f], column_job_word(bx, w[q]), S.foff[f], S.fnode_ptr[f]};
+    pos += w[q];
+  }
+  return pos;
+}
+std::vector<int64_t> count_columns(const Symbolic& S, const LaunchPlan& P, int lev, const std::vector<int64_t>& un, int64_t budget) {
+  const int steps = (int)un.size();
+  std::vector<int64_t> n(steps + 1);
+  for (int kb = -1; kb < steps; ++kb) n[kb + 1] = gen_columns(S, P, lev, kb, kb < 0 ? 0 : un[kb], budget, nullptr);
+  return n;
+}
+void place_columns(const LaunchPlan& P, int lev, const std::vector<int64_t>& n, ColumnLists& C, int64_t& pos) {
+  C.first_off.push_back(pos);
+  C.first_n.push_back((int32_t)n[0]);
+  pos += n[0];
+  for (int kb = 0; kb + 1 < (int)n.size(); ++kb) {
+    C.col_off.push_back(pos);
+    C.col_n.push_back((int32_t)n[kb + 1]);
+    C.nact.push_back(active_fronts(P, lev, kb * NB));
+    C.n_look.push_back(active_fronts(P, lev, (kb + 1) * NB));
+    pos += n[kb + 1];
+  }
+}
+
+void fill_columns(const Symbolic& S, const LaunchPlan& P, int lev, int64_t budget, ColumnLists& C) {
+  gen_columns(S, P, lev, -1, 0, budget, C.jobs.data() + C.first_off[lev]);
+  const int s0 = P.levels[lev].step0, s1 = lev + 1 < (int)P.levels.size() ? P.levels[lev + 1].step0 : (int)P.upd_n.size();
+  for (int s = s0; s < s1; ++s) gen_columns(S, P, lev, s - s0, P.upd_n[s], budget, C.jobs.data() + C.col_off[s]);
+}
+}
+
+void build_column_lists(const Symbolic& S, const LaunchPlan& P, int64_t budget, ColumnLists& C) {
+  C = ColumnLists();
+  C.budget = budget;
+  const int nl = (int)P.levels.size();
+  auto un = [&](int lev) {
+    const int s1 = lev + 1 < nl ? P.levels[lev + 1].step0 : (int)P.upd_n.size();
+    return std::vector<int64_t>(P.upd_n.begin() + P.levels[lev].step0, P.upd_n.begin() + s1);
+  };
+  int64_t pos = 0;
+  for (int lev = 0; lev < nl; ++lev) place_columns(P, lev, count_columns(S, P, lev, un(lev), budget), C, pos);
+  C.jobs.resize((size_t)pos);
+  for (int lev = 0; lev < nl; ++lev) fill_columns(S, P, lev, budget, C);
+}
 
 void build_launch_plan(const Symbolic& S, LaunchPlan& P, const PlanTasks& par) {
   auto run = [&](int ntasks, const std::function<void(int)>& f) {
@@ -21,7 +100,6 @@
   P.forder.resize(nf);
   std::vector<int32_t>& forder = P.forder;
   P.forder_s2.assign(nf, 0);
-  P.forder_maxm.assign(nf, 0);
   auto cdiv = [](int a, int b) { return (a + b - 1) / b; };
   auto gen_jobs = [&](int lev, bool fwd, SweepJob* out) -> int64_t {
     const LevelInfo& li = P.levels[lev];
@@ -97,7 +175,7 @@
       }
     return pos;
   };
-  struct Counts { int64_t fwd = 0, bwd = 0, gather = 0, formz = 0, mirrorx = 0; std::vector<int64_t> upd; };
+  struct Counts { int64_t fwd = 0, bwd = 0, gather = 0, formz = 0, mirrorx = 0; std::vector<int64_t> upd, cols; };
   std::vector<Counts> cnt(L + 1);
   run(L + 1, [&](int lev) {
     LevelInfo& li = P.levels[lev];
@@ -118,12 +196,7 @@
     for (int f = li.first; f < li.first + li.count; ++f) bucket[nb - 2 - fs2[f] / 16 + 1]++;
     for (int b = 1; b < nb; ++b) bucket[b] += bucket[b - 1];
     for (int f = li.first; f < li.first + li.count; ++f) o[bucket[nb - 2 - fs2[f] / 16]++] = f;
-    int mx = 0;
-    for (int q = 0; q < li.count; ++q) {
-      mx = std::max(mx, fm[o[q]]);
-      P.forder_s2[li.first + q] = fs2[o[q]];
-      P.forder_maxm[li.first + q] = mx;
-    }
+    for (int q = 0; q < li.count; ++q) P.forder_s2[li.first + q] = fs2[o[q]];
     li.fwd_rows = fwd_block_rows(li.count);
     li.bwd_rows = bwd_block_rows(li.count, lev == L);
     for (int q = 0; q < li.count; ++q)
@@ -137,13 +210,15 @@
     for (int kb = 0; kb < steps; ++kb) c.upd[kb] = gen_update(lev, kb, nullptr);
     c.formz = gen_formz(lev, nullptr);
     c.mirrorx = gen_mirrorx(lev, nullptr);
+    c.cols = count_columns(S, P, lev, c.upd, -1);
   });
   P.worst_m = 0;
   struct Fill { int kind, lev, kb; int64_t off; };
   std::vector<Fill> fills;
-  int64_t njobs = 0, pos = 0;
+  int64_t njobs = 0, pos = 0, ncols = 0;
   P.upd_off.clear();
   P.upd_n.clear();
+  P.cols = ColumnLists();
   for (int lev = 0; lev <= L; ++lev) {
     LevelInfo& li = P.levels[lev];
     const Counts& c = cnt[lev];
@@ -164,6 +239,8 @@
       if (c.upd[kb]) fills.push_back({3, lev, kb, pos});
       pos += c.upd[kb];
     }
+    place_columns(P, lev, c.cols, P.cols, ncols);
+    if (c.cols[0]) fills.push_back({8, lev, 0, 0});
     li.formz_off = pos; li.formz_n = (int)c.formz;
     if (c.formz) fills.push_back({4, lev, 0, pos});
     pos += c.formz;
@@ -183,10 +260,9 @@
     pos += cnt[lev].mirrorx;
   }
   P.mirrorx_all_n = (int)(pos - P.mirrorx_all_off);
-  for (int lev = 0; lev <= L; ++lev) fills.push_back({8, lev, 0, 0});
   P.jobs.resize((size_t)njobs);
   P.tiles.resize((size_t)pos);
-  P.frec.resize(nf);
+  P.cols.jobs.resize((size_t)ncols);
   std::stable_sort(fills.begin(), fills.end(), [&](const Fill& a, const Fill& b) { return a.lev > b.lev; });
   run((int)fills.size(), [&](int t) {
     const Fill& F = fills[t];
@@ -197,13 +273,7 @@
       case 3: gen_update(F.lev, F.kb, P.tiles.data() + F.off); break;
       case 4: case 6: gen_formz(F.lev, P.tiles.data() + F.off); break;
       case 5: case 7: gen_mirrorx(F.lev, P.tiles.data() + F.off); break;
-      default: {
-        const LevelInfo& li = P.levels[F.lev];
-        for (int q = li.first; q < li.first + li.count; ++q) {
-          const int f = forder[q];
-          P.frec[q] = FrontRec{f, fm[f], fs2[f], 0, S.foff[f], S.fnode_ptr[f]};
-        }
-      }
+      default: fill_columns(S, P, F.lev, -1, P.cols);
     }
   });
   int64_t level_nodes = 0;
diff --git a/pl_fem_vectoriel_amd/csrc/plan.h b/pl_fem_vectoriel_amd/csrc/plan.h
--- a/pl_fem_vectoriel_amd/csrc/plan.h
+++ b/pl_fem_vectoriel_amd/csrc/plan.h
@@ -43,6 +43,17 @@
   int64_t foff, np;
 };
 static_assert(sizeof(FrontRec) == 32, "FrontRec layout");
+constexpr int COLUMN_BX_BITS = 16;
+constexpr int32_t column_job_word(int bx, int n_pan) { return bx | (n_pan << COLUMN_BX_BITS); }
+constexpr int column_job_bx(int32_t word) { return word & ((1 << COLUMN_BX_BITS) - 1); }
+constexpr int column_job_n_pan(int32_t word) { return word >> COLUMN_BX_BITS; }
+inline int column_chunks(int m, int kb_next) {
+  const int rows = m - kb_next * NB - 16;
+  return rows > 64 ? (rows + 63) / 64 : 1;
+}
+constexpr int64_t COLUMN_BUDGET = 768;
+constexpr int64_t COLUMN_OTHERS_MAX = 3 * COLUMN_BUDGET;
+constexpr int64_t column_budget(int64_t others) { return others > COLUMN_OTHERS_MAX ? COLUMN_BUDGET / 2 : COLUMN_BUDGET; }
 inline int fwd_block_rows(int count) { return count <= 8 ? 8 : count <= ROW_FORM_MAX_FRONTS ? 16 : 64; }
 inline int bwd_block_rows(int count, bool leaf) { return leaf ? 64 : count <= ROW_FORM_MAX_FRONTS ? 8 : 16; }
 constexpr int BLOCK_P = 4;
@@ -74,18 +85,28 @@
 struct Tile { int32_t x, y; };
 static_assert(sizeof(Tile) == 8, "Tile layout");
 
+struct ColumnLists {
+  int64_t budget = -1;
+  std::vector<FrontRec, default_init_allocator<FrontRec>> jobs;
+  std::vector<int64_t> col_off;
+  std::vector<int32_t> col_n, nact, n_look;
+  std::vector<int64_t> first_off;
+  std::vector<int32_t> first_n;
+};
+void column_workgroups(const int32_t* chunks, int n, int64_t budget, int32_t* w);
+
 struct Symbolic;
 struct LaunchPlan {
   bool built = false;
   std::vector<int32_t> fs2, fm;
   std::vector<int32_t> forder;
-  std::vector<int32_t> forder_s2, forder_maxm;
-  std::vector<FrontRec, default_init_allocator<FrontRec>> frec;
+  std::vector<int32_t> forder_s2;
   std::vector<LevelInfo> levels;
   std::vector<SweepJob, default_init_allocator<SweepJob>> jobs;
   std::vector<Tile, default_init_allocator<Tile>> tiles;
   std::vector<int64_t> upd_off;
   std::vector<int32_t> upd_n;
+  ColumnLists cols;
   int64_t formz_all_off = 0, mirrorx_all_off = 0;
   int32_t formz_all_n = 0, mirrorx_all_n = 0;
   int64_t level_nodes_max = 0;
@@ -93,5 +114,6 @@
 };
 using PlanTasks = std::function<void(int ntasks, const std::function<void(int)>& f)>;
 void build_launch_plan(const Symbolic& S, LaunchPlan& P, const PlanTasks& par = {});
+void build_column_lists(const Symbolic& S, const LaunchPlan& P, int64_t budget, ColumnLists& C);
 
 }
```

Result: no change. 516.7 (-0.1%).
